# CFGpp-diffusion/CFGpp

Hardware: AMD Instinct MI355X
Metric: images/sec (higher is better)
Workload: dtype fp16; 1 GPU; SD1.5 512x512 ddim_cfg++ 50 NFE lambda=0.6 batch=8/GPU; per_gpu_batch=8, global_batch=8, nfe=50, unet_batch_rows=16, weights=seeded synthetic, exact diffusers shapes, build_id=cfgpp-build:650f45cb6498717d:nogit

## Files before the change

### cfgpp_amd/_lib.py

```python
from __future__ import annotations

import ctypes as C
import os

HERE = os.path.dirname(os.path.abspath(__file__))
LIB_PATH = os.environ.get("CFGPP_LIB") or os.path.join(HERE, "libcfgpp_hip.so")


class CfgppError(RuntimeError):
    pass


class UNetConfigC(C.Structure):
    _fields_ = [
        ("in_channels", C.c_int), ("out_channels", C.c_int),
        ("num_levels", C.c_int),
        ("block_out_channels", C.c_int * 4),
        ("layers_per_block", C.c_int),
        ("level_has_attn", C.c_int * 4),
        ("transformer_depth", C.c_int * 4),
        ("num_heads", C.c_int * 4),
        ("cross_attention_dim", C.c_int),
        ("addition_embed", C.c_int),
        ("addition_time_embed_dim", C.c_int),
# ... 15 lines not shown
    "cfgpp_kdiff_input": (_I, [_P, _P, _F, _I, _L, _P]),
    "cfgpp_step_kdiff": (_I, [_P, _P, _P, _P, _P, C.POINTER(C.c_float), _I, _I, _I, _I, _L, _P]),
    "cfgpp_kdiff_denoise": (_I, [_P, _P, _P, _F, _F, _P, _P, _L, _P]),
    "cfgpp_lincomb": (_I, [_P, _P, _P, _P, _F, _F, _I, _L, _P]),
    "cfgpp_unet_create": (_P, [C.POINTER(UNetConfigC), _I]),
    "cfgpp_unet_destroy": (None, [_P]),
    "cfgpp_unet_load_tensor": (_I, [_P, C.c_char_p, _P, _I, C.POINTER(C.c_long), _I]),
    "cfgpp_unet_missing": (_I, [_P]),
    "cfgpp_unet_finalize": (_I, [_P]),
    "cfgpp_unet_set_context": (_I, [_P, _P, _I, _I, _P, _P, _I, _P]),
    "cfgpp_unet_image_condition": (_I, [_P, _P, _I, _P]),
    "cfgpp_unet_forward": (_I, [_P, _P, _I, _I, _F, _P, _I, _P]),
    "cfgpp_sample_graph_ddim": (_I, [_P, _P, _P, _I, _I, _P, _P, _P, _I, C.POINTER(C.c_float), _I, _F, _I, _I, _P]),
    "cfgpp_unet_profile": (_I, [_P, _P, _I, _I, _F, _P, _I, _P, C.POINTER(C.c_double), C.POINTER(C.c_double), C.POINTER(C.c_int), C.c_char_p, _L]),
    "cfgpp_unet_tuning": (_I, [_P, _I, C.POINTER(C.c_int), _I, _I]),
    "cfgpp_unet_attach_control": (_I, [_P, _P, _F]),
    "cfgpp_unet_lora": (_I, [_P, C.c_char_p, _P, _P, _I, _P]),
    "cfgpp_unet_flops": (C.c_double, [_P, _I]),
    "cfgpp_unet_device_bytes": (C.c_double, [_P]),
    "cfgpp_vae_create": (_P, [_I, _I, _I, _F, _I]),
    "cfgpp_vae_destroy": (None, [_P]),
    "cfgpp_vae_load_tensor": (_I, [_P, C.c_char_p, _P, _I, C.POINTER(C.c_long), _I]),
    "cfgpp_vae_finalize": (_I, [_P]),
    "cfgpp_vae_decode": (_I, [_P, _P, _P, _I, _P]),
    "cfgpp_vae_decode_image": (_I, [_P, _P, _P, _I, _P]),
    "cfgpp_vae_encode": (_I, [_P, _P, _P, _P, _P, _I, _P]),
    "cfgpp_vae_flops": (C.c_double, [_P, _I]),
    "cfgpp_text_create": (_P, [_I, _I, _I, _I, _I, _I, _I, _I, _I]),
    "cfgpp_text_destroy": (None, [_P]),
    "cfgpp_text_load_tensor": (_I, [_P, C.c_char_p, _P, _I, C.POINTER(C.c_long), _I]),
    "cfgpp_text_finalize": (_I, [_P]),
    "cfgpp_text_encode": (_I, [_P, C.POINTER(C.c_int), C.POINTER(C.c_int), _I, _I, _P, _P, _P]),
    "cfgpp_text_device_bytes": (C.c_double, [_P]),
    "cfgpp_vae_encode_flops": (C.c_double, [_P, _I]),
    "cfgpp_vae_device_bytes": (C.c_double, [_P]),
}

IP_ADAPTER_PROTOTYPES = {
    "cfgpp_unet_ip_load": (_I, [_P, C.c_char_p, _P, _I, C.POINTER(C.c_long), _I]),
    "cfgpp_unet_image_context": (_I, [_P, _P, _I, _I, _F, _P]),
}

LONG_PROMPT_PROTOTYPES = {
    "cfgpp_unet_set_max_tokens": (_I, [_P, _I]),
}

DEBUG_PROTOTYPES = {
    "cfgpp_op_softmax_rows": (_I, [_P, _L, _I, _P]),
    "cfgpp_op_conv_in_ex": (_I, [_P, _I, _P, _P, _P, _I, _I, _I, _I, _I, _I, _P, _P, _F, _P]),
    "cfgpp_op_groupnorm": (_I, [_P, _P, _P, _P, _P, _P, _I, _I, _I, _I, _I, _I, _F, _I, _I, _P]),
    "cfgpp_op_groupnorm_pre": (_I, [_P, _P, _P, _P, _P, _P, _P, _P, _I, _I, _I, _I, _I, _I, _F, _I, _I, _P]),
    "cfgpp_op_igemm_set_gstat": (None, [_P]),
    "cfgpp_op_igemm_gstat_written": (_I, []),
    "cfgpp_groupnorm_set_prestats": (None, [_I]),
    "cfgpp_groupnorm_prestats_enabled": (_I, []),
    "cfgpp_unet_set_share_prefix": (None, [_I]),
    "cfgpp_unet_share_prefix_enabled": (_I, []),
    "cfgpp_unet_shared_prefix_ops": (_I, [_P, _I, _I]),
    "cfgpp_op_layernorm": (_I, [_P, _P, _P, _P, _L, _I, _F, _P]),
    "cfgpp_op_attention_prepare_vt": (_I, [_P, _I, _I, _I, _P]),
    "cfgpp_op_attention": (_I, [_P, _P, _P, _P, _I, _I, _I, _I, _I, _I, _I, _P]),
    "cfgpp_op_attention_cross": (_I, [_P, _P, _P, _P, _I, _I, _I, _I, _I, _I, _I, _P]),
    "cfgpp_attention_set_cross_long": (None, [_I]),
    "cfgpp_op_attention_clear_slots": (_I, [_P, _P, _I, _I, _I, _I, _I, _P]),
    "cfgpp_op_attention_ip": (_I, [_P, _P, _P, _P, _I, _I, _I, _I, _I, _I, _F, _I, _I, _P]),
    "cfgpp_op_conv_in": (_I, [_P, _I, _P, _P, _P, _I, _I, _I, _I, _I, _I, _P]),
    "cfgpp_op_conv_in_cond": (_I, [_P, _I, _P, _I, _I, _P, _P, _P, _I, _I, _I, _I, _I, _I, _P]),
    "cfgpp_op_conv_in_add": (_I, [_P, _I, _P, _I, _I, _P, _I, _P, _P, _P, _I, _I, _I, _I, _I, _I, _P]),
    "cfgpp_op_cn_conv3x3": (_I, [_P, _I, _P, _I, _P, _P, _I, _I, _I, _I, _I, _I, _I, _P]),
    "cfgpp_op_residual_add": (_I, [C.POINTER(C.c_void_p), C.POINTER(C.c_void_p), C.POINTER(C.c_int), _I, _I, _F, _P]),
    "cfgpp_op_residual_nchw": (_I, [_P, _P, _I, _I, _I, _I, _F, _P]),
    "cfgpp_controlnet_residual": (_I, [_P, _I, _F, _P, _I, C.POINTER(C.c_int), _P]),
    "cfgpp_vae_profile": (_I, [_P, _P, _P, _I, _P, C.c_char_p, C.c_long]),
    "cfgpp_unet_read_weight": (_I, [_P, C.c_char_p, _P]),
    "cfgpp_op_vae_posterior": (_I, [_P, _P, _P, _P, _P, _P, _I, _I, _F, _P]),
    "cfgpp_op_conv_out": (_I, [_P, _P, _I, _P, _P, _I, _I, _I, _I, _I, _P]),
    "cfgpp_op_conv_out_ex": (_I, [_P, _P, _I, _P, _P, _I, _I, _I, _I, _I, _F, _F, _I, _P]),
    "cfgpp_conv_out_set_tiled": (None, [_I]),
    "cfgpp_op_sinusoid": (_I, [_P, _F, _P, _I, _I, _I, _I, _P]),
    "cfgpp_op_skinny_gemm": (_I, [_P, _I, _P, _P, _P, _I, _P, _I, _I, _I, _I, _I, _I, _P]),
    "cfgpp_op_f16_to_f32_rows": (_I, [_P, _P, _I, _I, _I, _I, _P]),
    "cfgpp_op_igemm": (_I, [_P, _P, _I, _I, _I, _I, _I, _I, _P, _I, _I, _P, _P, _I, _P, _I, _I, _P, _I, _I, _I, _P]),
    "cfgpp_op_igemm_heads": (_I, [_P, _I, _P, _I, _I, _P, _I, _P, _P, _P, _I, _I, _I, _I, _I, _I, _P]),
    "cfgpp_igemm_force_config": (None, [_I]),
    "cfgpp_igemm_set_staging": (None, [_I]),
    "cfgpp_igemm_set_staged_epilogue": (None, [_I]),
    "cfgpp_igemm_set_big_tiles": (None, [_I]),
    "cfgpp_igemm_set_tail_split": (None, [_I]),
    "cfgpp_igemm_set_autotune": (None, [_I]),
    "cfgpp_igemm_set_blocked_walk": (None, [_I]),
    "cfgpp_igemm_walk_plan_probe": (None, [_I, _I, _I, _I, _I, _I, _I, C.POINTER(C.c_int)]),
    "cfgpp_igemm_set_n_major": (None, [_I]),
    "cfgpp_igemm_force_split": (None, [_I]),
    "cfgpp_igemm_set_split_tile": (None, [_I]),
    "cfgpp_igemm_set_mf16": (None, [_I]),
    "cfgpp_igemm_set_mf16_rounds": (None, [_I]),
    "cfgpp_igemm_set_mf16_heads": (None, [_I]),
    "cfgpp_igemm_set_mf16_linear": (None, [_I]),
    "cfgpp_igemm_set_big_split": (None, [_I]),
    "cfgpp_igemm_set_tune_mask": (None, [C.c_uint]),
    "cfgpp_igemm_tuner_state": (C.c_uint, []),
    "cfgpp_igemm_timeline": (None, [_P, _L, _I]),
    "cfgpp_igemm_timeline_info": (None, [C.POINTER(C.c_int)]),
    "cfgpp_groupnorm_set_mode": (None, [_I]),
    "cfgpp_layernorm_set_rows_per_wave": (None, [_I]),
    "cfgpp_attention_set_dma": (None, [_I]),
    "cfgpp_attention_set_stagger": (None, [_I]),
    "cfgpp_attention_set_cross": (None, [_I]),
    "cfgpp_attention_last_launch": (None, [C.POINTER(C.c_int)]),
    "cfgpp_groupnorm_last_launch": (None, [C.POINTER(C.c_int)]),
    "cfgpp_layernorm_last_launch": (None, [C.POINTER(C.c_int)]),
    "cfgpp_softmax_last_launch": (None, [C.POINTER(C.c_int)]),
}

_lib = None


def load():
    global _lib
    if _lib is not None:
        return _lib
    if not os.path.exists(LIB_PATH):
        raise CfgppError(
            f"{LIB_PATH} not found: build it with `python -m cfgpp_amd.build` "
            "(__graft_entry__.build()).  The HIP path has no CPU fallback.")
    import torch
    try:
        lib = C.CDLL(LIB_PATH)
    except OSError as e:
        raise CfgppError(f"cannot load {LIB_PATH}: {e}") from e
    for name, (res, args) in list(PROTOTYPES.items()) + list(IP_ADAPTER_PROTOTYPES.items()) + list(LONG_PROMPT_PROTOTYPES.items()) + list(DEBUG_PROTOTYPES.items()):
        try:
            fn = getattr(lib, name)
        except AttributeError as e:
            raise CfgppError(f"{LIB_PATH} does not export {name}") from e
        fn.restype = res
        fn.argtypes = args
    if os.environ.get("CFGPP_AUTOTUNE", "1") == "0":
        lib.cfgpp_igemm_set_autotune(0)
    _lib = lib
    return lib


def build_id() -> str:
    return load().cfgpp_build_id().decode("utf-8", "replace")


def last_error() -> str:
    return load().cfgpp_last_error().decode("utf-8", "replace")


def check(rc: int, what: str):
    if rc != 0:
        raise CfgppError(f"{what} failed (rc={rc}): {last_error()}")
```

### cfgpp_amd/csrc/big4.h

```cpp
#pragma once
#include "igemm.h"

inline void big4_tile(int cfg, int* BM, int* BN) {
    *BM = cfg == 24 ? 256 : 128;
    *BN = cfg == 25 ? 320 : 256;
}
inline bool big4_supports(int cfg, const IGemmArgs& a, bool staged_epi) {
    if (cfg < 24 || cfg > 26 || !staged_epi || a.K < 64) return false;
    const long rows = a.amode == 0 ? (long)a.M : a.amode == 2 ? (long)(a.M / a.rows_per_batch) * (2 * a.H + 2) * (2 * a.W + 2)
                                                : (long)(a.M / a.rows_per_batch) * (a.H + 2) * (a.W + 2);
    const long cmax = a.C0 > a.C1 ? a.C0 : a.C1;
    if (rows >= (1L << 24) || rows * cmax * 2 >= (1L << 32) || (long)a.N * a.K * 2 >= (1L << 32) || a.N >= (1 << 24)) return false;
    if (a.epi == EPI_STORE) return (a.N & 7) == 0;
    if (a.epi == EPI_GEGLU) return cfg != 25 && (a.N & 127) == 0 && a.omode == 0;
    return a.epi == EPI_HEADS && (a.rows_per_batch & 31) == 0 && (a.part_width & 31) == 0 && (a.head_dim & 7) == 0 && (a.N & 31) == 0 &&
           (a.M & 31) == 0;
}
int big4_par_bytes(int BN, int nb);
int big4_run(int cfg, const IGemmArgs& a, int grid, int smem, hipStream_t stream);

inline bool big4p_supports(const IGemmArgs& a, bool staged_epi) {
    return a.amode == 0 && a.C1 == 0 && a.taps == 1 && a.temb == nullptr && big4_supports(24, a, staged_epi) && (long)a.K * 2 < (1L << 24);
}
int big4p_smem(int par_bytes_one);
int big4p_run(const IGemmArgs& a, int grid, int smem, int par_bytes_one, hipStream_t stream);
```

### cfgpp_amd/csrc/cfgpp_debug.h

```cpp
#ifndef CFGPP_DEBUG_H
#define CFGPP_DEBUG_H
#ifdef __cplusplus
extern "C" {
#endif

int cfgpp_op_softmax_rows(void* s, long rows, int ncols, void* stream);
int cfgpp_op_conv_in_ex(const void* z, int z_is_half, void* out, const float* w, const float* bias,
                        int R, int zB, int Cin, int H, int W, int Cout, const float* pre_w, const float* pre_b,
                        float in_scale, void* stream);
int cfgpp_op_groupnorm(const void* src0, const void* src1, void* dst, const float* gamma, const float* beta,
                       float* stats, int N, int H, int W, int C0, int C1, int G, float eps, int silu,
                       int dst_padded, void* stream);
int cfgpp_op_groupnorm_pre(const void* src0, const void* src1, void* dst, const float* gamma, const float* beta,
                           const float* gst0, const float* gst1, float* stats, int N, int H, int W, int C0, int C1, int G,
                           float eps, int silu, int dst_padded, void* stream);
void cfgpp_op_igemm_set_gstat(void* buf);
int cfgpp_op_igemm_gstat_written(void);
void cfgpp_groupnorm_set_prestats(int on);
int cfgpp_groupnorm_prestats_enabled(void);
void cfgpp_unet_set_share_prefix(int on);
int cfgpp_unet_share_prefix_enabled(void);
int cfgpp_unet_shared_prefix_ops(cfgpp_unet* u, int rows, int z_rows);
void cfgpp_groupnorm_set_mode(int mode);
int cfgpp_op_layernorm(const void* x, void* y, const float* gamma, const float* beta, long rows, int C,
                       float eps, void* stream);
void cfgpp_layernorm_set_rows_per_wave(int rpw);
void cfgpp_groupnorm_last_launch(int* out8);
void cfgpp_layernorm_last_launch(int* out2);
void cfgpp_softmax_last_launch(int* out1);
int cfgpp_op_attention_prepare_vt(void* vt, int BH, int d, int tok_pad, void* stream);
int cfgpp_op_attention(const void* q, const void* k, const void* vt, void* o, int B, int heads, int d,
                       int nq, int nk, int q_tok_pad, int k_tok_pad, void* stream);
void cfgpp_attention_set_dma(int mode);
void cfgpp_attention_set_stagger(int sleeps);
void cfgpp_attention_set_cross(int on);
int cfgpp_op_attention_cross(const void* q, const void* k, const void* vt, void* o, int B, int heads, int d,
                             int nq, int nk, int q_tok_pad, int k_tok_pad, void* stream);
void cfgpp_attention_set_cross_long(int mode);
void cfgpp_attention_last_launch(int* out4);
int cfgpp_op_attention_clear_slots(void* k, void* vt, int BH, int d, int tok_pad, int slot0, int n, void* stream);
int cfgpp_op_attention_ip(const void* q, const void* k, const void* vt, void* o, int B, int heads, int d, int nq, int nk_text,
                          int n_img, float ip_scale, int q_tok_pad, int k_tok_pad, void* stream);
int cfgpp_op_conv_in(const void* z, int z_is_half, void* out, const float* w, const float* bias,
                     int R, int zB, int Cin, int H, int W, int Cout, void* stream);
int cfgpp_op_conv_in_cond(const void* z, int z_is_half, const void* cond, int cond_rows, int Cc, void* out, const float* w,
                          const float* bias, int R, int zB, int Cz, int H, int W, int Cout, void* stream);
int cfgpp_op_conv_in_add(const void* z, int z_is_half, const void* cond, int cond_rows, int Cc, const void* addend, int add_rows,
                         void* out, const float* w, const float* bias, int R, int zB, int Cz, int H, int W, int Cout, void* stream);
int cfgpp_op_cn_conv3x3(const void* in, int in_kind, void* out, int out_pad, const float* w, const float* bias, int R, int Ci, int Co,
                        int Hi, int Wi, int stride, int silu, void* stream);
int cfgpp_op_residual_add(void* const* dst, const void* const* src, const int* hwc, int n, int rows, float scale, void* stream);
int cfgpp_op_residual_nchw(const void* src, float* out, int rows, int H, int W, int C, float scale, void* stream);
int cfgpp_controlnet_residual(cfgpp_unet* cn, int i, float scale, float* out, int rows, int* hwc_out, void* stream);

int cfgpp_unet_read_weight(cfgpp_unet* u, const char* key, void* host_fp16_out);

int cfgpp_vae_profile(cfgpp_vae* v, const void* z, void* img, int B, void* stream, char* detail, long detail_cap);

int cfgpp_op_vae_posterior(const float* conv_out, const float* qw, const float* qb, const float* noise, float* z,
                           float* moments, int B, int HW, float scale, void* stream);
int cfgpp_op_conv_out(const void* x, void* out, int out_is_half, const void* w, const float* bias,
                      int R, int H, int W, int C, int Cout, void* stream);
int cfgpp_op_conv_out_ex(const void* x, void* out, int out_is_half, const void* w, const float* bias,
                         int R, int H, int W, int C, int Cout, float post_scale, float post_shift, int clamp01, void* stream);
void cfgpp_conv_out_set_tiled(int on);
int cfgpp_op_sinusoid(const float* vals, float scalar, float* out, int count, int dim, int out_ld, int out_off,
                      void* stream);
int cfgpp_op_skinny_gemm(const float* x, int ldx, const void* w, const float* bias, const float* addend, int add_ld,
                         float* out, int ldo, int M, int N, int K, int silu_in, int silu_out, void* stream);
int cfgpp_op_f16_to_f32_rows(const void* in, float* out, int rows, int cols, int out_ld, int out_off, void* stream);

int cfgpp_op_igemm(const void* a0, const void* a1, int C0, int C1, int taps, int amode, int H, int W,
                   const void* w, int M, int N, const float* bias, const float* temb, int temb_ld,
                   const void* resid, int rmode, int rld, void* out, int omode, int old_, int epi,
                   void* stream);
int cfgpp_op_igemm_heads(const void* a, int K, const void* w, int M, int N, const float* bias, int rows_per_batch,
                         void* hq, void* hk, void* hvt, int part0, int part_width, int head_dim, int heads,
                         int q_tok_pad, int tok_pad, void* stream);
void cfgpp_igemm_force_config(int cfg);
void cfgpp_igemm_set_tail_split(int on);
void cfgpp_igemm_set_mf16(int mode);
void cfgpp_igemm_set_mf16_linear(int on);
void cfgpp_igemm_set_mf16_heads(int on);
void cfgpp_igemm_set_mf16_rounds(int n);
void cfgpp_igemm_set_split_tile(int cfg);
void cfgpp_igemm_force_split(int s);
void cfgpp_igemm_set_big_split(int min_kt);
void cfgpp_igemm_set_n_major(int mode);
void cfgpp_igemm_set_blocked_walk(int on);
void cfgpp_igemm_walk_plan_probe(int M, int N, int K, int BM, int BN, int smem, int n_major, int* out5);
void cfgpp_igemm_set_tune_mask(unsigned mask);
unsigned cfgpp_igemm_tuner_state(void);
void cfgpp_igemm_set_autotune(int on);
void cfgpp_igemm_set_big_tiles(int on);
void cfgpp_igemm_set_staged_epilogue(int on);
void cfgpp_igemm_set_staging(int glds);
void cfgpp_igemm_timeline(void* buf, long cap_blocks, int target);
void cfgpp_igemm_timeline_info(int* out12);

#ifdef __cplusplus
}
#endif
#endif
```

### cfgpp_amd/csrc/engine_base.h

```cpp
#pragma once
#include <algorithm>
#include <cmath>
#include <cstring>
#include <deque>
#include <functional>
#include <map>
#include <string>
#include <utility>
#include <vector>

#include "../../include/cfgpp.h"
#include "../../include/cfgpp_ip_adapter.h"
#include "../../include/cfgpp_long_prompt.h"
#include "cfgpp_debug.h"
#include "igemm.h"

namespace {


struct HostParam {
    std::vector<long> shape;
    std::vector<half_t> h;
    std::vector<float> f;
    bool is_matrix = false;
// ... 69 lines not shown
        static const int cands[] = {0, 1, 4, 5, 6, 7, 8, 9, 10, 11, 12, 13, 14, 15, 16, 17, 20, 24, 25, 26, 27, 28};
        const size_t n = plan.size();
        plan_hint.resize(n, nullptr);
        hipStreamCaptureStatus cap = hipStreamCaptureStatusNone;
        if (hipStreamIsCapturing(s, &cap) != hipSuccess || cap != hipStreamCaptureStatusNone) return 0;
        std::vector<hipEvent_t> ev(n + 1, nullptr);
        for (auto& e : ev) if (hipEventCreate(&e) != hipSuccess) return -1;
        std::vector<float> base(n, 1e30f), best(n, 1e30f), t(n);
        std::vector<char> applied(n, 1);
        std::vector<int> bestc(n, 0);
        int rc = 0;
        auto timed_passes = [&]() {
            std::fill(t.begin(), t.end(), 1e30f);
            for (int rep = 0; rep < 2 && rc == 0; ++rep) {
                if (hipEventRecord(ev[0], s) != hipSuccess) rc = -1;
                for (size_t i = 0; i < n && rc == 0; ++i) {
                    rc = plan[i](s, rows_for(i, rows, shared));
                    if (plan_hint[i]) applied[i] = (char)igemm_last_hint_applied();
                    if (rc == 0 && hipEventRecord(ev[i + 1], s) != hipSuccess) rc = -1;
                }
                if (rc == 0 && hipEventSynchronize(ev[n]) != hipSuccess) rc = -1;
                for (size_t i = 0; i < n && rc == 0; ++i) {
                    if (!plan_hint[i]) continue;
                    float ms = 0.f;
                    if (hipEventElapsedTime(&ms, ev[i], ev[i + 1]) == hipSuccess && ms < t[i]) t[i] = ms;
                }
            }
        };
        const unsigned mask = igemm_tune_mask();
        for (int c : cands) {
            if (c != 0 && !((mask >> c) & 1u)) continue;
            for (int& h : cfg_hints) h = c;
            timed_passes();
            for (size_t i = 0; i < n; ++i) {
                if (c == 0) base[i] = t[i];
                if (t[i] < best[i] && (c == 0 || applied[i])) { best[i] = t[i]; bestc[i] = c; }
            }
        }
        for (size_t i = 0; i < n; ++i)
            if (plan_hint[i] && !(bestc[i] != 0 && best[i] < 0.97f * base[i])) { bestc[i] = 0; best[i] = base[i]; }
        for (int walk = 1; walk <= 2 && rc == 0 && (mask >> 31); ++walk) {
            for (size_t i = 0; i < n; ++i) if (plan_hint[i]) *plan_hint[i] = (bestc[i] & 63) | (walk << 6);
            timed_passes();
            for (size_t i = 0; i < n; ++i)
                if (plan_hint[i] && t[i] < 0.97f * best[i]) { best[i] = t[i]; bestc[i] = (bestc[i] & 63) | (walk << 6); }
        }
        for (int& h : cfg_hints) h = 0;
        for (size_t i = 0; i < n; ++i) if (plan_hint[i]) *plan_hint[i] = bestc[i];
        for (auto& e : ev) hipEventDestroy(e);
        if (rc == 0) tuned_by_rows[key] = std::vector<int>(cfg_hints.begin(), cfg_hints.end());
        tuned_rows = rows; tuned_shared = shared;
        return rc;
    }
    std::map<std::tuple<int, int, int>, std::vector<std::pair<half_t*, float*>>> pool;
    std::deque<int> gst_flags;
    float* d_gn_stats = nullptr;
    static constexpr long KSPLIT_WS_BYTES = 128L << 20;
    float* d_ksplit_ws = nullptr;
    float* ksplit_ws() {
        if (!d_ksplit_ws) d_ksplit_ws = (float*)dmalloc((size_t)KSPLIT_WS_BYTES, false);
        return d_ksplit_ws;
    }

    void* dmalloc(size_t bytes, bool zero = true) {
        void* p = nullptr;
        if (hipMalloc(&p, bytes) != hipSuccess) return nullptr;
        if (zero) hipMemset(p, 0, bytes);
        allocs.push_back(p);
        dev_bytes += (double)bytes;
        return p;
    }
    Tensor acq(int H, int W, int C) {
        auto key = std::make_tuple(H, W, C);
        auto& fl = pool[key];
        Tensor t; t.H = H; t.W = W; t.C = C;
        gst_flags.push_back(0);
        t.gst_ok = &gst_flags.back();
        if (!fl.empty()) { t.p = fl.back().first; t.gst = fl.back().second; fl.pop_back(); return t; }
        t.p = (half_t*)dmalloc((size_t)max_rows * (H + 2) * (W + 2) * C * sizeof(half_t));
        if (H * W >= 1024 && (H * W) % 32 == 0 && C % 8 == 0)
            t.gst = (float*)dmalloc((size_t)max_rows * (H * W / 32) * C * 2 * sizeof(float), false);
        return t;
    }
    void rel(const Tensor& t) { if (t.p) pool[std::make_tuple(t.H, t.W, t.C)].push_back(std::make_pair(t.p, t.gst)); }
    ~EngineBase() { for (void* p : allocs) hipFree(p); }
};

void expect(EngineBase* u, const std::string& key, std::vector<long> shape, bool matrix) {
    HostParam hp; hp.shape = std::move(shape); hp.is_matrix = matrix;
    u->params[key] = std::move(hp);
}
void expect_linear(EngineBase* u, const std::string& p, long out, long in, bool bias = true) {
    expect(u, p + ".weight", {out, in}, true);
    if (bias) expect(u, p + ".bias", {out}, false);
}
void expect_conv(EngineBase* u, const std::string& p, long out, long in, int k) {
    expect(u, p + ".weight", {out, in, k, k}, true);
    expect(u, p + ".bias", {out}, false);
}
void expect_norm(EngineBase* u, const std::string& p, long c) {
    expect(u, p + ".weight", {c}, false);
    expect(u, p + ".bias", {c}, false);
}
void expect_resnet(EngineBase* u, const std::string& p, long cin, long cout, long temb) {
    expect_norm(u, p + ".norm1", cin);
    expect_conv(u, p + ".conv1", cout, cin, 3);
    expect_linear(u, p + ".time_emb_proj", cout, temb);
    expect_norm(u, p + ".norm2", cout);
    expect_conv(u, p + ".conv2", cout, cout, 3);
    if (cin != cout) expect_conv(u, p + ".conv_shortcut", cout, cin, 1);
}
void expect_transformer(EngineBase* u, const std::string& p, long c, int depth, long cross) {
    expect_norm(u, p + ".norm", c);
    expect(u, p + ".proj_in.weight", {c, c}, true);  expect(u, p + ".proj_in.bias", {c}, false);
    expect(u, p + ".proj_out.weight", {c, c}, true); expect(u, p + ".proj_out.bias", {c}, false);
    for (int k = 0; k < depth; ++k) {
        const std::string b = p + ".transformer_blocks." + std::to_string(k);
        expect_norm(u, b + ".norm1", c); expect_norm(u, b + ".norm2", c); expect_norm(u, b + ".norm3", c);
        expect_linear(u, b + ".attn1.to_q", c, c, false); expect_linear(u, b + ".attn1.to_k", c, c, false);
        expect_linear(u, b + ".attn1.to_v", c, c, false); expect_linear(u, b + ".attn1.to_out.0", c, c, true);
        expect_linear(u, b + ".attn2.to_q", c, c, false); expect_linear(u, b + ".attn2.to_k", c, cross, false);
        expect_linear(u, b + ".attn2.to_v", c, cross, false); expect_linear(u, b + ".attn2.to_out.0", c, c, true);
        expect_linear(u, b + ".ff.net.0.proj", 8 * c, c, true);
        expect_linear(u, b + ".ff.net.2", c, 4 * c, true);
    }
}

struct Builder {
    EngineBase* u;
    bool ok = true;
    std::string err;

    HostParam* get(const std::string& key) {
        auto it = u->params.find(key);
        if (it == u->params.end() || !it->second.loaded) { ok = false; err = "missing parameter " + key; return nullptr; }
        return &it->second;
    }
    template <typename T>
    T* upload(const std::vector<T>& v) {
        T* d = (T*)u->dmalloc(v.size() * sizeof(T), false);
        if (!d) { ok = false; err = "hipMalloc failed"; return nullptr; }
        if (hipMemcpy(d, v.data(), v.size() * sizeof(T), hipMemcpyHostToDevice) != hipSuccess) { ok = false; err = "hipMemcpy failed"; }
        return d;
    }
    void slot(const std::string& key, half_t* d, int kind, long row_off = 0) {
        const HostParam& p = u->params[key];
        WeightSlot w; w.ptr = d; w.kind = kind; w.row_off = row_off; w.O = p.shape[0];
        w.taps = kind == SLOT_CONV3 ? 9 : 1; w.I = p.numel() / (w.O * w.taps);
        u->slots[key] = w;
    }
    void drop(const std::string& key) { auto& p = u->params[key]; std::vector<half_t>().swap(p.h); std::vector<float>().swap(p.f); }

    float* f32(const std::string& key) {
        HostParam* p = get(key); if (!p) return nullptr;
        float* d = upload(p->f); drop(key); return d;
    }
    half_t* linear(const std::string& key) {
        HostParam* p = get(key); if (!p) return nullptr;
        half_t* d = upload(p->h); drop(key); slot(key, d, SLOT_PLAIN); return d;
    }
    half_t* conv3(const std::string& key) {
        HostParam* p = get(key); if (!p) return nullptr;
        const long O = p->shape[0], I = p->shape[1];
        std::vector<half_t> r((size_t)O * 9 * I);
        for (long o = 0; o < O; ++o)
            for (long i = 0; i < I; ++i)
                for (int t = 0; t < 9; ++t) r[(size_t)o * 9 * I + ((i >> 6) * 9 + t) * 64 + (i & 63)] = p->h[((size_t)o * I + i) * 9 + t];
        half_t* d = upload(r); drop(key); slot(key, d, SLOT_CONV3); return d;
    }
    std::vector<half_t> concat_host(const std::vector<std::string>& keys) {
        std::vector<half_t> r;
        for (auto& k : keys) { HostParam* p = get(k); if (!p) return {}; r.insert(r.end(), p->h.begin(), p->h.end()); }
        for (auto& k : keys) drop(k);
        return r;
    }
    half_t* concat(const std::vector<std::string>& keys) {
        std::vector<half_t> r = concat_host(keys);
        if (!ok) return nullptr;
        half_t* d = upload(r);
        long row = 0;
        for (auto& k : keys) { slot(k, d, SLOT_MEMBER, row); row += u->params[k].shape[0]; }
        return d;
    }
    bool geglu_host(const std::string& pfx, long C, std::vector<half_t>& rw, std::vector<float>& rb) {
        HostParam* pw = get(pfx + ".weight"); HostParam* pb = get(pfx + ".bias");
        if (!pw || !pb) return false;
        const long F = 4 * C;
        rw.resize((size_t)2 * F * C); rb.resize((size_t)2 * F);
        for (long f = 0; f < F; ++f) {
            const long pv = (f / 32) * 64 + (f % 32), pg = pv + 32;
            std::memcpy(&rw[(size_t)pv * C], &pw->h[(size_t)f * C], C * sizeof(half_t));
            std::memcpy(&rw[(size_t)pg * C], &pw->h[(size_t)(F + f) * C], C * sizeof(half_t));
            rb[pv] = pb->f[f]; rb[pg] = pb->f[F + f];
        }
        drop(pfx + ".weight"); drop(pfx + ".bias");
        return true;
    }
    void geglu(const std::string& pfx, long C, half_t** w, float** b) {
        std::vector<half_t> rw; std::vector<float> rb;
        if (!geglu_host(pfx, C, rw, rb)) return;
        *w = upload(rw); *b = upload(rb);
        slot(pfx + ".weight", *w, SLOT_GEGLU);
    }
};

inline int round_up(int a, int b) { return (a + b - 1) / b * b; }

IGemmArgs base_args(EngineBase* u = nullptr) {
    IGemmArgs a; std::memset(&a, 0, sizeof(a)); a.out_scale = 1.0f; a.taps = 1;
    if (u) { a.ws_buf = u->ksplit_ws(); a.ws_bytes = a.ws_buf ? EngineBase::KSPLIT_WS_BYTES : 0; }
    return a;
}

struct Plan {
    EngineBase* u;
    Builder* B;
    std::vector<Op>* ops;

    void conv3x3(const Tensor& src, const Tensor& dst, const half_t* w, const float* bias, int amode,
                 const float* temb, int temb_ld, const Tensor* resid, int ashift = 0) {
        IGemmArgs a = base_args(u);
        a.a0 = src.p; a.C0 = src.C; a.taps = 9; a.amode = amode; a.ashift = ashift; a.H = dst.H; a.W = dst.W;
        a.w = w; a.N = dst.C; a.K = 9 * src.C; a.bias = bias; a.temb = temb; a.temb_ld = temb_ld;
        a.rows_per_batch = dst.H * dst.W;
        if (resid) { a.resid = resid->p; a.rmode = 1; a.rld = resid->C; }
        a.out = dst.p; a.omode = 1; a.old = dst.C; a.epi = EPI_STORE;
        a.gstat = dst.gst; a.stat_flag = dst.gst ? dst.gst_ok : nullptr;
        const int HW = dst.H * dst.W;
        u->macs_per_row += (double)HW * dst.C * 9.0 * src.C;
        int* hint = u->new_hint(ops == &u->plan);
        ops->push_back([a, HW, hint](hipStream_t s, int rows) mutable { IGemmArgs b = a; b.M = rows * HW; b.cfg_hint = *hint; return igemm_launch(b, s); });
        if (ops == &u->plan) u->tag(0, (double)HW * dst.C * 9.0 * src.C, "conv3x3 amode=" + std::to_string(amode) + " HW=" + std::to_string(HW) + " N=" + std::to_string(dst.C) + " K=" + std::to_string(9 * src.C) + (resid ? " +res" : "") + (temb ? " +temb" : ""));
    }
    void conv1x1(const Tensor& s0, const Tensor* s1, const Tensor& dst, const half_t* w, const float* bias) {
        IGemmArgs a = base_args(u);
        a.a0 = s0.p; a.C0 = s0.C; if (s1) { a.a1 = s1->p; a.C1 = s1->C; }
        a.amode = 1; a.H = dst.H; a.W = dst.W; a.w = w; a.N = dst.C; a.K = a.C0 + a.C1; a.bias = bias;
        a.rows_per_batch = dst.H * dst.W; a.out = dst.p; a.omode = 1; a.old = dst.C; a.epi = EPI_STORE;
        const int HW = dst.H * dst.W;
        u->macs_per_row += (double)HW * dst.C * a.K;
        int* hint = u->new_hint(ops == &u->plan);
        ops->push_back([a, HW, hint](hipStream_t s, int rows) mutable { IGemmArgs b = a; b.M = rows * HW; b.cfg_hint = *hint; return igemm_launch(b, s); });
        if (ops == &u->plan) u->tag(0, (double)HW * dst.C * a.K, "conv1x1 HW=" + std::to_string(HW) + " N=" + std::to_string(dst.C) + " K=" + std::to_string(a.K));
    }
    void linear(const half_t* A, int K, half_t* out, int N, const half_t* w, const float* bias, const half_t* resid,
                int tokens, int epi = EPI_STORE) {
        IGemmArgs a = base_args(u);
        a.a0 = A; a.C0 = K; a.amode = 0; a.w = w; a.N = N; a.K = K; a.bias = bias;
        a.resid = resid; a.rmode = 0; a.rld = N; a.out = out; a.omode = 0;
        a.old = (epi == EPI_GEGLU) ? N / 2 : N; a.epi = epi; a.rows_per_batch = tokens;
        u->macs_per_row += (double)tokens * N * K;
        int* hint = u->new_hint(ops == &u->plan);
        ops->push_back([a, tokens, hint](hipStream_t s, int rows) mutable { IGemmArgs b = a; b.M = rows * tokens; b.cfg_hint = *hint; return igemm_launch(b, s); });
        if (ops == &u->plan) u->tag(0, (double)tokens * N * K, std::string(epi == EPI_GEGLU ? "geglu" : "linear") + " HW=" + std::to_string(tokens) + " N=" + std::to_string(N) + " K=" + std::to_string(K) + (resid ? " +res" : ""));
    }
    void linear_to_padded(const half_t* A, int K, const Tensor& dst, const half_t* w, const float* bias, const Tensor& resid) {
        IGemmArgs a = base_args(u);
        a.a0 = A; a.C0 = K; a.amode = 0; a.H = dst.H; a.W = dst.W; a.w = w; a.N = dst.C; a.K = K; a.bias = bias;
        a.resid = resid.p; a.rmode = 1; a.rld = resid.C; a.out = dst.p; a.omode = 1; a.old = dst.C;
        a.epi = EPI_STORE; a.rows_per_batch = dst.H * dst.W;
        a.gstat = dst.gst; a.stat_flag = dst.gst ? dst.gst_ok : nullptr;
        const int HW = dst.H * dst.W;
        u->macs_per_row += (double)HW * dst.C * K;
        int* hint = u->new_hint(ops == &u->plan);
        ops->push_back([a, HW, hint](hipStream_t s, int rows) mutable { IGemmArgs b = a; b.M = rows * HW; b.cfg_hint = *hint; return igemm_launch(b, s); });
        if (ops == &u->plan) u->tag(0, (double)HW * dst.C * K, "proj_out HW=" + std::to_string(HW) + " N=" + std::to_string(dst.C) + " K=" + std::to_string(K));
    }
    void heads(const half_t* A, int K, const half_t* w, int N, int tokens, int part0, int C, int nheads,
               half_t* q, half_t* k, half_t* vt, int q_tok_pad, int tok_pad, bool count = true,
               const float* bias = nullptr) {
        IGemmArgs a = base_args(u);
        const int d = C / nheads;
        a.a0 = A; a.C0 = K; a.amode = 0; a.w = w; a.N = N; a.K = K; a.epi = EPI_HEADS;
        a.bias = bias;
        a.rows_per_batch = tokens; a.hq = q; a.hk = k; a.hvt = vt; a.part0 = part0; a.part_width = C;
        a.head_dim = d; a.head_dim_pad = round_up(d, 32); a.heads = nheads; a.tok_pad = tok_pad; a.q_tok_pad = q_tok_pad;
        if (count) u->macs_per_row += (double)tokens * N * K;
        int* hint = u->new_hint(ops == &u->plan);
        ops->push_back([a, tokens, hint](hipStream_t s, int rows) mutable { IGemmArgs b = a; b.M = rows * tokens; b.cfg_hint = *hint; return igemm_launch(b, s); });
        if (ops == &u->plan) u->tag(0, count ? (double)tokens * N * K : 0.0, "heads HW=" + std::to_string(tokens) + " N=" + std::to_string(N) + " K=" + std::to_string(K));
    }
    void groupnorm(const Tensor& s0, const Tensor* s1, half_t* dst, bool dst_padded, const float* g, const float* b,
                   float eps, bool silu) {
        EngineBase* uu = u;
        const half_t* p0 = s0.p; const half_t* p1 = s1 ? s1->p : nullptr;
        const int H = s0.H, W = s0.W, C0 = s0.C, C1 = s1 ? s1->C : 0, G = u->norm_groups;
        const float* gst0 = s0.gst; const float* gst1 = s1 ? s1->gst : nullptr;
        const int* ok0 = s0.gst_ok; const int* ok1 = s1 ? s1->gst_ok : nullptr;
        ops->push_back([=](hipStream_t s, int rows) {
            if (cfgpp_groupnorm_prestats_enabled() && gst0 && ok0 && *ok0 && (!p1 || (gst1 && ok1 && *ok1)))
                return cfgpp_op_groupnorm_pre(p0, p1, dst, g, b, gst0, gst1, uu->d_gn_stats, rows, H, W, C0, C1, G, eps, silu ? 1 : 0,
                                              dst_padded ? 1 : 0, s);
            return cfgpp_op_groupnorm(p0, p1, dst, g, b, uu->d_gn_stats, rows, H, W, C0, C1, G, eps, silu ? 1 : 0,
                                      dst_padded ? 1 : 0, s);
        });
        if (ops == &u->plan) u->tag(2, 0.0, "groupnorm HW=" + std::to_string(H * W) + " C=" + std::to_string(C0 + C1));
    }
    void layernorm(const half_t* x, half_t* y, const float* g, const float* b, int tokens, int C) {
        ops->push_back([=](hipStream_t s, int rows) { return cfgpp_op_layernorm(x, y, g, b, (long)rows * tokens, C, 1e-5f, s); });
        if (ops == &u->plan) u->tag(2, 0.0, "layernorm HW=" + std::to_string(tokens) + " C=" + std::to_string(C));
    }
    void attention(const half_t* q, const half_t* k, const half_t* vt, half_t* o, int nheads, int d, int nq, int nk,
                   int q_tok_pad, int k_tok_pad) {
        u->attn_macs_per_row += 2.0 * (double)nheads * nq * nk * d;
        ops->push_back([=](hipStream_t s, int rows) {
            return cfgpp_op_attention(q, k, vt, o, rows, nheads, d, nq, nk, q_tok_pad, k_tok_pad, s);
        });
        if (ops == &u->plan) u->tag(1, 2.0 * (double)nheads * nq * nk * d, "self_attn heads=" + std::to_string(nheads) + " N=" + std::to_string(nq) + " d=" + std::to_string(d));
    }
};

}
```

### cfgpp_amd/csrc/igemm.h

```cpp
#pragma once
#include "common.h"

enum IGemmEpi : int {
    EPI_STORE = 0,
    EPI_GEGLU = 1,
    EPI_HEADS = 2,
};

struct IGemmArgs {
    const half_t* a0;
    const half_t* a1;
    int C0, C1;
    int taps;
    int amode;
    int H, W;
    int ashift;
    const half_t* w;
    int M, N, K;
    int epi;
    const float* bias;
    const float* temb;
    int temb_ld;
    int rows_per_batch;
    const half_t* resid;
    int rmode, rld;
    half_t* out;
    int omode, old;
    float out_scale;
    float* gstat;
    int* stat_flag;
    half_t* hq; half_t* hk; half_t* hvt;
    int part0;
    int part_width;
    int head_dim, head_dim_pad, heads;
    int vt_linear;
    int tok_pad;
    int q_tok_pad;
    int n_main;
    int ksplit;
    float* ws;
    float* ws_buf;
    long ws_bytes;
    int cfg_hint;
    int allow_split;
    int staged_epi;
    int n_major;
    int walk_div;
    int walk_hint;
    int walk_bn, walk_per, walk_tmb, walk_tnb;
    int split;
    int par_nb;
    unsigned long long* tl;
};

int igemm_launch(const IGemmArgs& a, hipStream_t stream);
int igemm_autotune_enabled();
int igemm_last_hint_applied();
unsigned igemm_tune_mask();
```

### cfgpp_amd/csrc/igemm_device.h

```cpp
#pragma once
#include "igemm.h"

namespace {


__device__ __forceinline__ void tl_stamp(unsigned long long* tl, int slot) {
    if (tl != nullptr && threadIdx.x == 0) tl[(long)blockIdx.x * 16 + slot] = __builtin_amdgcn_s_memtime();
}
__device__ __forceinline__ void tl_begin(unsigned long long* tl) {
    if (tl != nullptr && threadIdx.x == 0) {
        unsigned long long* r = tl + (long)blockIdx.x * 16;
        r[0] = __builtin_amdgcn_s_memtime();
        r[4] = __builtin_amdgcn_s_memrealtime();
        const unsigned hw = __builtin_amdgcn_s_getreg((31 << 11) | 4), xcc = __builtin_amdgcn_s_getreg((31 << 11) | 20);
        r[6] = (unsigned long long)hw | ((unsigned long long)xcc << 32);
    }
}
__device__ __forceinline__ void tl_end(unsigned long long* tl) {
    if (tl != nullptr) {
        asm volatile("s_waitcnt vmcnt(0)" ::: "memory");
        if (threadIdx.x == 0) {
            unsigned long long* r = tl + (long)blockIdx.x * 16;
            r[3] = __builtin_amdgcn_s_memtime();
            r[5] = __builtin_amdgcn_s_memrealtime();
        }
    }
}

__device__ __forceinline__ int qdiv(int m, int d) {
    int dv = d;
    asm volatile("" : "+v"(dv));
    const float inv = __builtin_amdgcn_rcpf((float)dv);
    int q = (int)((float)m * inv);
    const int r = m - q * d;
    q += (r >= d ? 1 : 0) - (r < 0 ? 1 : 0);
    return q;
}

__device__ __forceinline__ int padded_pix(int m, int HW, int W, int H) {
    const int b = qdiv(m, HW), p = m - b * HW;
    const int y = qdiv(p, W), x = p - y * W;
    return (b * (H + 2) + y + 1) * (W + 2) + x + 1;
}


__device__ __forceinline__ int qdiv_u(int a, int d) { return __builtin_amdgcn_readfirstlane(qdiv(a, d)); }
__device__ __forceinline__ void tile_of(const IGemmArgs& p, int wg, int& tile_m, int& tile_n) {
    if (p.walk_bn > 0) {
        const int x = qdiv_u(wg, p.walk_per), i = wg - x * p.walk_per;
        const int bmi = qdiv_u(x, p.walk_bn), bni = x - bmi * p.walk_bn;
        int im, in;
        if (p.n_major) { in = qdiv_u(i, p.walk_tmb); im = i - in * p.walk_tmb; }
        else { im = qdiv_u(i, p.walk_tnb); in = i - im * p.walk_tnb; }
        tile_m = bmi * p.walk_tmb + im; tile_n = bni * p.walk_tnb + in;
    } else {
        const int wq = qdiv(wg, p.walk_div), wr = wg - wq * p.walk_div;
        tile_m = p.n_major ? wr : wq; tile_n = p.n_major ? wq : wr;
    }
}

constexpr int PAR_NB = 5;
__host__ __device__ constexpr int par_bnp(int BN) { return (BN + 63) / 64 * 64; }
__host__ __device__ constexpr int par_bytes(int BN, int nb = PAR_NB) { return par_bnp(BN) * 4 * (1 + nb); }
struct Par {
    const char* lds;
    int n0, b0, bnp;
};
template <int BN, int NW>
__device__ __forceinline__ void par_stage(const IGemmArgs& p, char* par, int n0, int m0, int wid, int lane) {
    constexpr int BNP = par_bnp(BN), NPC = BNP / 64;
    int nn = n0 + lane;
    const int HW = p.rows_per_batch;
    const int b0 = HW > 0 ? qdiv(m0, HW) : 0;
    const int nb = HW > 0 ? (p.M + HW - 1) / HW : 1;
    int pi = 0;
    auto arr = [&](const float* src, int slot) {
#pragma unroll
        for (int q = 0; q < NPC; ++q, ++pi) {
            if (wid == pi % NW) {
                int n = nn + 64 * q;
                n = n < p.N ? n : p.N - 1;
                __builtin_amdgcn_global_load_lds((const __attribute__((address_space(1))) void*)(src + n),
                                                 (__attribute__((address_space(3))) void*)(par + (slot * BNP + q * 64) * 4), 4, 0, 0);
            }
        }
    };
    if (p.bias) arr(p.bias, 0);
    if (p.temb) {
        for (int k = 0; k < p.par_nb; ++k) {
            int b = b0 + k;
            b = b < nb ? b : nb - 1;
            arr(p.temb + (long)b * p.temb_ld, 1 + k);
        }
    }
}
template <bool L>
__device__ __forceinline__ float4 par_bias4(const IGemmArgs& p, const Par& q, int n) {
    if constexpr (L) return *reinterpret_cast<const float4*>(q.lds + (n - q.n0) * 4);
    else return *reinterpret_cast<const float4*>(p.bias + n);
}
template <bool L>
__device__ __forceinline__ float4 par_temb4(const IGemmArgs& p, const Par& q, int b, int n) {
    if constexpr (L) {
        int k = b - q.b0;
        k = k < p.par_nb ? k : p.par_nb - 1;
        k = k < 0 ? 0 : k;
        return *reinterpret_cast<const float4*>(q.lds + ((1 + k) * q.bnp + n - q.n0) * 4);
    } else {
        return *reinterpret_cast<const float4*>(p.temb + (long)b * p.temb_ld + n);
    }
}
template <bool PIN, int NT>
__device__ __forceinline__ void acc_row_pin(f32x16 (&row)[NT]) {
    if constexpr (PIN) {
#pragma unroll
        for (int j = 0; j < NT; ++j) asm volatile("" : "+a"(row[j]));
    }
}
template <int MT, int NT, bool L>
__device__ __forceinline__ void igemm_epilogue(const IGemmArgs& p, f32x16 (&acc)[MT][NT], int mw0, int nw0, int lane, const Par& par) {
    const int frow = lane & 31, fhi = lane >> 5;
    const int HW = p.rows_per_batch;
#pragma unroll
    for (int i = 0; i < MT; ++i) {
        const int m = mw0 + i * 32 + frow;
        if (m >= p.M) continue;
        const int b = (HW > 0) ? qdiv(m, HW) : 0;
        const int tok = m - b * HW;
        long orow = m, rrow = m;
        if (p.omode == 1 || p.rmode == 1) {
            const long pp = padded_pix(m, HW, p.W, p.H);
            if (p.omode == 1) orow = pp;
            if (p.rmode == 1) rrow = pp;
        }
        if (p.epi == EPI_STORE) {
#pragma unroll
            for (int j = 0; j < NT; ++j)
#pragma unroll
                for (int g = 0; g < 4; ++g) {
                    int n = nw0 + j * 32 + 8 * g + 4 * fhi;
                    asm volatile("" : "+v"(n));
                    if (n >= p.N) continue;
                    float v[4];
#pragma unroll
                    for (int k = 0; k < 4; ++k) v[k] = acc[i][j][4 * g + k] * p.out_scale;
                    if (p.bias) {
                        const float4 bb = par_bias4<L>(p, par, n);
                        v[0] += bb.x; v[1] += bb.y; v[2] += bb.z; v[3] += bb.w;
                    }
                    if (p.temb) {
                        const float4 tt = par_temb4<L>(p, par, b, n);
                        v[0] += tt.x; v[1] += tt.y; v[2] += tt.z; v[3] += tt.w;
                    }
                    if (p.resid) {
                        const half4_t rr = *reinterpret_cast<const half4_t*>(p.resid + rrow * p.rld + n);
#pragma unroll
                        for (int k = 0; k < 4; ++k) v[k] += (float)rr[k];
                    }
                    half4_t o;
#pragma unroll
                    for (int k = 0; k < 4; ++k) o[k] = (half_t)v[k];
                    *reinterpret_cast<half4_t*>(p.out + orow * p.old + n) = o;
                }
        } else if (p.epi == EPI_GEGLU) {
            if constexpr (NT % 2 == 0) {
#pragma unroll
                for (int j = 0; j < NT; j += 2)
#pragma unroll
                    for (int g = 0; g < 4; ++g) {
                        const int pc = nw0 + j * 32 + 8 * g + 4 * fhi;
                        if (pc >= p.N) continue;
                        const int f = (pc >> 6) * 32 + (pc & 31);
                        float v[4], gt[4];
#pragma unroll
                        for (int k = 0; k < 4; ++k) { v[k] = acc[i][j][4 * g + k]; gt[k] = acc[i][j + 1][4 * g + k]; }
                        if (p.bias) {
                            const float4 bv = par_bias4<L>(p, par, pc);
                            const float4 bg = par_bias4<L>(p, par, pc + 32);
                            v[0] += bv.x; v[1] += bv.y; v[2] += bv.z; v[3] += bv.w;
                            gt[0] += bg.x; gt[1] += bg.y; gt[2] += bg.z; gt[3] += bg.w;
                        }
                        half4_t o;
                        const f32x2 g01 = gelu_erf_pk((f32x2){gt[0], gt[1]}), g23 = gelu_erf_pk((f32x2){gt[2], gt[3]});
                        o[0] = (half_t)(v[0] * g01.x); o[1] = (half_t)(v[1] * g01.y);
                        o[2] = (half_t)(v[2] * g23.x); o[3] = (half_t)(v[3] * g23.y);
                        *reinterpret_cast<half4_t*>(p.out + orow * p.old + f) = o;
                    }
            }
        } else {
#pragma unroll
            for (int j = 0; j < NT; ++j)
#pragma unroll
                for (int g = 0; g < 4; ++g) {
                    int n = nw0 + j * 32 + 8 * g + 4 * fhi;
                    asm volatile("" : "+v"(n));
                    if (n >= p.N) continue;
                    const int part = n / p.part_width + p.part0;
                    const int cn = n % p.part_width;
                    const int head = cn / p.head_dim, dd = cn - head * p.head_dim;
                    float v[4];
#pragma unroll
                    for (int k = 0; k < 4; ++k) v[k] = acc[i][j][4 * g + k];
                    if (p.bias) {
                        const float4 bb = par_bias4<L>(p, par, n);
                        v[0] += bb.x; v[1] += bb.y; v[2] += bb.z; v[3] += bb.w;
                    }
                    const long bh = (long)b * p.heads + head;
                    if (part == 2) {
                        half_t* dst = p.hvt + (bh * p.head_dim_pad + dd) * p.tok_pad + (p.vt_linear ? tok : cfgpp_vt_pos(tok));
#pragma unroll
                        for (int k = 0; k < 4; ++k) dst[(long)k * p.tok_pad] = (half_t)v[k];
                    } else {
                        half4_t o;
#pragma unroll
                        for (int k = 0; k < 4; ++k) o[k] = (half_t)v[k];
                        half_t* base = part == 0 ? p.hq : p.hk;
                        const int tp = part == 0 ? p.q_tok_pad : p.tok_pad;
                        *reinterpret_cast<half4_t*>(base + (bh * tp + tok) * p.head_dim_pad + dd) = o;
                    }
                }
        }
    }
}

template <int WTN, int PITCH>
__device__ __forceinline__ void gstat_block(const IGemmArgs& p, const char* stg, int m_blk0, int nw0, int lane) {
    if (m_blk0 >= p.M) return;
    float* dst = p.gstat + ((long)(m_blk0 >> 5) * p.N + nw0) * 2;
#pragma unroll 1
    for (int cp = lane; cp < WTN / 2; cp += 64) {
        const half2_t x0 = *reinterpret_cast<const half2_t*>(stg + cp * 4);
        const float pv0 = (float)x0[0], pv1 = (float)x0[1];
        float s0 = 0.f, s1 = 0.f, q0 = 0.f, q1 = 0.f;
#pragma unroll 4
        for (int r = 1; r < 32; ++r) {
            const half2_t x = *reinterpret_cast<const half2_t*>(stg + r * PITCH + cp * 4);
            const float d0 = (float)x[0] - pv0, d1 = (float)x[1] - pv1;
            s0 += d0; q0 += d0 * d0; s1 += d1; q1 += d1 * d1;
        }
        if (nw0 + 2 * cp < p.N)
            *reinterpret_cast<float4*>(dst + 4 * cp) = make_float4(pv0 + s0 * (1.0f / 32.0f), q0 - s0 * s0 * (1.0f / 32.0f),
                                                                   pv1 + s1 * (1.0f / 32.0f), q1 - s1 * s1 * (1.0f / 32.0f));
    }
}

template <int MT, int NT, bool L, bool PIN = false>
__device__ __forceinline__ void igemm_epilogue_staged(const IGemmArgs& p, f32x16 (&acc)[MT][NT], int mw0, int nw0, int lane,
                                                      char* stg , const Par& par) {
    constexpr int WTN = NT * 32;
    constexpr int PITCH = WTN * 2 + 16;
    constexpr int CPR = WTN / 8;
    constexpr int NQ = (32 * CPR + 63) / 64;
    constexpr bool EARLY = false;
    const int frow = lane & 31, fhi = lane >> 5;
    const int HW = p.rows_per_batch;
#pragma unroll
    for (int i = 0; i < MT; ++i) {
        acc_row_pin<PIN, NT>(acc[i]);
        const int m = mw0 + i * 32 + frow;
        const int mc = m < p.M ? m : p.M - 1;
        const int b = (HW > 0) ? qdiv(mc, HW) : 0;
        int opix = mc, rpix = mc;
        if (p.omode == 1 || p.rmode == 1) {
            const int pp = padded_pix(mc, HW, p.W, p.H);
            if (p.omode == 1) opix = pp;
            if (p.rmode == 1) rpix = pp;
        }
        half8_t rres[NQ];
        auto request_residual = [&]() {
#pragma unroll
            for (int q = 0; q < NQ; ++q) {
                const int c = lane + 64 * q;
                const int r = c / CPR, cc = c - r * CPR;
                const int rp = __shfl(rpix, r);
                int n = nw0 + cc * 8;
                n = n < p.N ? n : p.N - 8;
                rres[q] = *reinterpret_cast<const half8_t*>(p.resid + (long)rp * p.rld + n);
            }
        };
        if constexpr (EARLY) { if (p.resid) request_residual(); }
#pragma unroll
        for (int j = 0; j < NT; ++j)
#pragma unroll
            for (int g = 0; g < 4; ++g) {
                const int nl = j * 32 + 8 * g + 4 * fhi;
                int n = nw0 + nl;
                n = n < p.N ? n : p.N - 4;
                float v[4];
#pragma unroll
                for (int k = 0; k < 4; ++k) v[k] = acc[i][j][4 * g + k] * p.out_scale;
                if (p.bias) {
                    const float4 bb = par_bias4<L>(p, par, n);
                    v[0] += bb.x; v[1] += bb.y; v[2] += bb.z; v[3] += bb.w;
                }
                if (p.temb) {
                    const float4 tt = par_temb4<L>(p, par, b, n);
                    v[0] += tt.x; v[1] += tt.y; v[2] += tt.z; v[3] += tt.w;
                }
                half4_t o;
#pragma unroll
                for (int k = 0; k < 4; ++k) o[k] = (half_t)v[k];
                *reinterpret_cast<half4_t*>(stg + frow * PITCH + nl * 2) = o;
            }
        if constexpr (!EARLY) { if (p.resid) request_residual(); }
#pragma unroll
        for (int q = 0; q < NQ; ++q) {
            const int c = lane + 64 * q;
            const int r = c / CPR, cc = c - r * CPR;
            const int op = __shfl(opix, r);
            const int mm = mw0 + i * 32 + r, n = nw0 + cc * 8;
            half8_t v = *reinterpret_cast<const half8_t*>(stg + (r & 31) * PITCH + cc * 16);
            if (p.resid) {
#pragma unroll
                for (int k = 0; k < 8; ++k) v[k] = (half_t)((float)v[k] + (float)rres[q][k]);
                if (p.gstat && c < 32 * CPR) *reinterpret_cast<half8_t*>(stg + (r & 31) * PITCH + cc * 16) = v;
            }
            if (c < 32 * CPR && mm < p.M && n < p.N) *reinterpret_cast<half8_t*>(p.out + (long)op * p.old + n) = v;
        }
        if (p.gstat) gstat_block<WTN, PITCH>(p, stg, mw0 + i * 32, nw0, lane);
    }
}

template <int MT, int NT, bool L, bool PIN = false>
__device__ __forceinline__ void igemm_epilogue_geglu_staged(const IGemmArgs& p, f32x16 (&acc)[MT][NT], int mw0, int nw0, int lane,
                                                            char* stg, const Par& par) {
    constexpr int WTF = (NT / 2) * 32;
    constexpr int PITCH = WTF * 2 + 16;
    constexpr int CPR = WTF / 8;
    constexpr int NQ = (32 * CPR + 63) / 64;
    const int frow = lane & 31, fhi = lane >> 5;
    const int f0 = (nw0 >> 6) * 32;
    const int NF = p.N >> 1;
#pragma unroll
    for (int i = 0; i < MT; ++i) {
        acc_row_pin<PIN, NT>(acc[i]);
#pragma unroll
        for (int j = 0; j < NT; j += 2)
#pragma unroll
            for (int g = 0; g < 4; ++g) {
                int pc = nw0 + j * 32 + 8 * g + 4 * fhi;
                pc = pc < p.N ? pc : p.N - 64;
                float v[4], gt[4];
#pragma unroll
                for (int k = 0; k < 4; ++k) { v[k] = acc[i][j][4 * g + k]; gt[k] = acc[i][j + 1][4 * g + k]; }
                if (p.bias) {
                    const float4 bv = par_bias4<L>(p, par, pc);
                    const float4 bg = par_bias4<L>(p, par, pc + 32);
                    v[0] += bv.x; v[1] += bv.y; v[2] += bv.z; v[3] += bv.w;
                    gt[0] += bg.x; gt[1] += bg.y; gt[2] += bg.z; gt[3] += bg.w;
                }
                half4_t o;
                const f32x2 g01 = gelu_erf_pk((f32x2){gt[0], gt[1]}), g23 = gelu_erf_pk((f32x2){gt[2], gt[3]});
                o[0] = (half_t)(v[0] * g01.x); o[1] = (half_t)(v[1] * g01.y);
                o[2] = (half_t)(v[2] * g23.x); o[3] = (half_t)(v[3] * g23.y);
                *reinterpret_cast<half4_t*>(stg + frow * PITCH + ((j >> 1) * 32 + 8 * g + 4 * fhi) * 2) = o;
            }
#pragma unroll
        for (int q = 0; q < NQ; ++q) {
            const int c = lane + 64 * q;
            const int r = c / CPR, cc = c - r * CPR;
            const int mm = mw0 + i * 32 + r, f = f0 + cc * 8;
            if (c < 32 * CPR && mm < p.M && f < NF)
                *reinterpret_cast<half8_t*>(p.out + (long)mm * p.old + f) = *reinterpret_cast<const half8_t*>(stg + r * PITCH + cc * 16);
        }
    }
}

struct HeadCol { int part, head, dd; };
__device__ __forceinline__ HeadCol head_col(const IGemmArgs& p, int ng_uniform) {
    const int ng = __builtin_amdgcn_readfirstlane(ng_uniform);
    const int pr = ng / p.part_width, cn0 = ng - pr * p.part_width;
    const int h = cn0 / p.head_dim;
    HeadCol c; c.part = pr + p.part0; c.head = h; c.dd = cn0 - h * p.head_dim;
    return c;
}
__device__ __forceinline__ void head_step(const IGemmArgs& p, const HeadCol& c, int off, int& head, int& dd) {
    dd = c.dd + off; head = c.head;
    if (p.head_dim >= 32) {
        if (dd >= p.head_dim) { dd -= p.head_dim; ++head; }
    } else {
        const int q = dd / p.head_dim;
        head += q; dd -= q * p.head_dim;
    }
}

template <int MT, int NT, bool L, bool PIN = false>
__device__ __forceinline__ void igemm_epilogue_heads_staged(const IGemmArgs& p, f32x16 (&acc)[MT][NT], int mw0, int nw0, int lane,
                                                            char* stg , const Par& par) {
    constexpr int PITCH = 80, BLK = 32 * PITCH;
    const int frow = lane & 31, fhi = lane >> 5;
    const int HW = p.rows_per_batch;
    const int ppos = cfgpp_vt_pos(frow);
    HeadCol hc[NT];
#pragma unroll
    for (int j = 0; j < NT; ++j) { const int ng = nw0 + j * 32; hc[j] = head_col(p, ng < p.N ? ng : p.N - 32); }
#pragma unroll
    for (int i = 0; i < MT; ++i) {
        acc_row_pin<PIN, NT>(acc[i]);
        const int m0s = __builtin_amdgcn_readfirstlane(mw0 + i * 32);
        if (m0s >= p.M) continue;
        const int b = qdiv(m0s, HW), tok0 = m0s - b * HW;
#pragma unroll
// ... 63 lines not shown
```

### cfgpp_amd/csrc/igemm_kernel.hip

```cpp
#include <cstring>
#include <map>
#include <tuple>
#include <type_traits>
#include "igemm.h"

#include "igemm_device.h"
#include "big4.h"

namespace {

template <int WM, int WN, int WTM, int WTN, bool GLDS, int AMODE, int NST = 2>
__global__ void __launch_bounds__(64 * WM * WN)
igemm_kernel(const IGemmArgs p) {
    constexpr int NTHR = 64 * WM * WN;
    constexpr int BM = WM * WTM, BN = WN * WTN;
    constexpr int MT = WTM / 32, NT = WTN / 32;
    constexpr int RSTEP = NTHR / 8;
    constexpr int A_CH = BM / RSTEP, B_CH = BN / RSTEP;
    static_assert(BM % RSTEP == 0 && BN % RSTEP == 0, "tile/loader mismatch");
    constexpr int STAGE_BYTES = (BM + BN) * 128;

    extern __shared__ __attribute__((aligned(16))) char smem[];
    tl_begin(p.tl);
    constexpr int PAR_OFF = NST * (WM * WTM + WN * WTN) * 128;

    const int ntn = (p.N + BN - 1) / BN;
    const int bid = blockIdx.x;
    int wg, ksl = 0;
    const bool is_tail = bid >= p.n_main;
    if (!is_tail) {
        const int nwg = p.n_main;
        const int q = nwg >> 3, r = nwg & 7;
        const int xcd = bid & 7, idx = bid >> 3;
        wg = (xcd < r ? xcd * (q + 1) : r * (q + 1) + (xcd - r) * q) + idx;
    } else {
        const int b1 = bid - p.n_main, nb = (int)gridDim.x - p.n_main;
        const int q = nb >> 3, r = nb & 7;
        const int xcd = b1 & 7, idx = b1 >> 3;
        const int b2 = (xcd < r ? xcd * (q + 1) : r * (q + 1) + (xcd - r) * q) + idx;
        wg = p.n_main + b2 / p.ksplit;
        ksl = b2 - (b2 / p.ksplit) * p.ksplit;
    }
    int tile_m, tile_n;
    tile_of(p, wg, tile_m, tile_n);
    const int m0 = tile_m * BM, n0 = tile_n * BN;

    const int tid = threadIdx.x, lane = tid & 63, wid = tid >> 6;
    const int wm = wid / WN, wn = wid - wm * WN;

    const int lrow = tid >> 3, lchunk = tid & 7;
    const int HW = p.rows_per_batch;
    const int Cin = p.C0 + p.C1;
    int a_pix[A_CH];
#pragma unroll
    for (int j = 0; j < A_CH; ++j) {
        int m = m0 + lrow + j * RSTEP;
        m = m < p.M ? m : p.M - 1;
        if constexpr (AMODE == 0) a_pix[j] = m;
        else if constexpr (AMODE == 1) a_pix[j] = padded_pix(m, HW, p.W, p.H);
        else if constexpr (AMODE == 2) {
            const int b = qdiv(m, HW), q = m - b * HW, y = qdiv(q, p.W), x = q - y * p.W;
            a_pix[j] = (b * (2 * p.H + 2) + 2 * y + 1 + p.ashift) * (2 * p.W + 2) + 2 * x + 1 + p.ashift;
        } else {
            const int b = qdiv(m, HW), q = m - b * HW, y = qdiv(q, p.W), x = q - y * p.W;
            a_pix[j] = (b << 22) | (y << 11) | x;
        }
    }
    const int schunk = GLDS ? (lchunk ^ ((lrow >> 1) & 7)) : lchunk;
    const half_t* b_ptr[B_CH];
#pragma unroll
    for (int j = 0; j < B_CH; ++j) {
        int n = n0 + lrow + j * RSTEP;
        n = n < p.N ? n : p.N - 1;
        b_ptr[j] = p.w + (long)n * p.K + schunk * 8;
    }
    int st_off[(A_CH > B_CH ? A_CH : B_CH)];
#pragma unroll
    for (int j = 0; j < (A_CH > B_CH ? A_CH : B_CH); ++j) {
        const int r = lrow + j * RSTEP;
        st_off[j] = r * 128 + ((lchunk ^ ((r >> 1) & 7)) << 4);
    }

    half8_t ra[A_CH], rb[B_CH];
    const int KT_all = p.K >> 6;
    const int kt_begin = is_tail ? (int)(((long)ksl * KT_all) / p.ksplit) : 0;
    const int kt_end = is_tail ? (int)(((long)(ksl + 1) * KT_all) / p.ksplit) : KT_all;

    auto load_tile = [&](int kt) {
        int tap = 0, cc = kt << 6;
        if (p.taps == 9) { const int cb = kt / 9; tap = kt - cb * 9; cc = cb << 6; }
        const bool s0 = cc < p.C0;
        const half_t* src = s0 ? p.a0 : p.a1;
        const int cs = s0 ? cc : cc - p.C0, Cs = s0 ? p.C0 : p.C1;
        int dy = 0, dx = 0;
        if (p.taps == 9) { dy = tap / 3 - 1; dx = tap - (tap / 3) * 3 - 1; }
        int dpix = 0;
        if constexpr (AMODE == 1) dpix = dy * (p.W + 2) + dx;
        else if constexpr (AMODE == 2) dpix = dy * (2 * p.W + 2) + dx;
#pragma unroll
        for (int j = 0; j < A_CH; ++j) {
            int pix;
            if constexpr (AMODE == 3) {
                const int b = a_pix[j] >> 22, y = (a_pix[j] >> 11) & 2047, x = a_pix[j] & 2047;
                const int Hs = p.H >> 1, Ws = p.W >> 1;
                pix = (b * (Hs + 2) + ((y + dy) >> 1) + 1) * (Ws + 2) + ((x + dx) >> 1) + 1;
            } else {
                pix = a_pix[j] + dpix;
            }
            ra[j] = *reinterpret_cast<const half8_t*>(src + (long)pix * Cs + cs + lchunk * 8);
        }
#pragma unroll
        for (int j = 0; j < B_CH; ++j) rb[j] = *reinterpret_cast<const half8_t*>(b_ptr[j] + ((long)kt << 6));
    };
    const int wave_row0 = __builtin_amdgcn_readfirstlane(wid) * 8;
    auto dma_tile = [&](int kt, int stage) {
        int tap = 0, cc = kt << 6;
        if (p.taps == 9) { const int cb = kt / 9; tap = kt - cb * 9; cc = cb << 6; }
        const bool s0 = cc < p.C0;
        const half_t* src = s0 ? p.a0 : p.a1;
        const int cs = s0 ? cc : cc - p.C0, Cs = s0 ? p.C0 : p.C1;
        int dy = 0, dx = 0;
        if (p.taps == 9) { dy = tap / 3 - 1; dx = tap - (tap / 3) * 3 - 1; }
        int dpix = 0;
        if constexpr (AMODE == 1) dpix = dy * (p.W + 2) + dx;
        else if constexpr (AMODE == 2) dpix = dy * (2 * p.W + 2) + dx;
        char* As = smem + stage * STAGE_BYTES;
        char* Bs = As + BM * 128;
#pragma unroll
        for (int j = 0; j < A_CH; ++j) {
            int pix;
            if constexpr (AMODE == 3) {
                const int b = a_pix[j] >> 22, y = (a_pix[j] >> 11) & 2047, x = a_pix[j] & 2047;
                const int Hs = p.H >> 1, Ws = p.W >> 1;
                pix = (b * (Hs + 2) + ((y + dy) >> 1) + 1) * (Ws + 2) + ((x + dx) >> 1) + 1;
            } else {
                pix = a_pix[j] + dpix;
            }
            const half_t* g = src + (long)pix * Cs + cs + schunk * 8;
            __builtin_amdgcn_global_load_lds((const __attribute__((address_space(1))) void*)g,
                                             (__attribute__((address_space(3))) void*)(As + (wave_row0 + j * RSTEP) * 128), 16, 0, 0);
        }
#pragma unroll
        for (int j = 0; j < B_CH; ++j) {
            const half_t* g = b_ptr[j] + ((long)kt << 6);
            __builtin_amdgcn_global_load_lds((const __attribute__((address_space(1))) void*)g,
                                             (__attribute__((address_space(3))) void*)(Bs + (wave_row0 + j * RSTEP) * 128), 16, 0, 0);
        }
    };
    auto store_tile = [&](int stage) {
        char* As = smem + stage * STAGE_BYTES;
        char* Bs = As + BM * 128;
#pragma unroll
        for (int j = 0; j < A_CH; ++j) *reinterpret_cast<half8_t*>(As + st_off[j]) = ra[j];
#pragma unroll
        for (int j = 0; j < B_CH; ++j) *reinterpret_cast<half8_t*>(Bs + st_off[j]) = rb[j];
    };

    f32x16 acc[MT][NT];
#pragma unroll
    for (int i = 0; i < MT; ++i)
#pragma unroll
        for (int j = 0; j < NT; ++j)
#pragma unroll
            for (int k = 0; k < 16; ++k) acc[i][j][k] = 0.f;

    const int frow = lane & 31, fhi = lane >> 5;
    const int fsw = (frow >> 1) & 7;
    const int a_rd = (wm * WTM + frow) * 128;
    const int b_rd = (wn * WTN + frow) * 128;

    if constexpr (GLDS) {
        constexpr int NP = A_CH + B_CH;
        constexpr int NM = 4 * MT * NT;
        constexpr bool ILV = (WM * WN >= 8);
        constexpr int SPAN = ILV ? (NM * 5) / 8 : 0;
        const int nk = kt_end - kt_begin;
        tl_stamp(p.tl, 8);
        if (!is_tail) par_stage<BN, WM * WN>(p, smem + PAR_OFF, n0, m0, __builtin_amdgcn_readfirstlane(wid), lane);
#pragma unroll
        for (int s_ = 0; s_ < NST - 1; ++s_) if (s_ < nk) dma_tile(kt_begin + s_, s_);
        tl_stamp(p.tl, 9);
        if (NST > 2 && nk >= NST - 1) asm volatile("s_waitcnt vmcnt(%0)" :: "n"((NST > 2 ? (NST - 2) * NP : 0)) : "memory");
        else asm volatile("s_waitcnt vmcnt(0)" ::: "memory");
        __syncthreads();
        tl_stamp(p.tl, 1);
        auto tile_body = [&](int kt, int cur, int ktn, int nxt, auto with_dma) {
            constexpr bool DMA = decltype(with_dma)::value;
            const char* As = smem + cur * STAGE_BYTES;
            const char* Bs = As + BM * 128;
            const half_t* src = p.a0; int cs = 0, Cs = p.C0, dpix = 0, dy = 0, dx = 0;
            char* Asn = smem + nxt * STAGE_BYTES;
            char* Bsn = Asn + BM * 128;
            if constexpr (DMA) {
                int tap = 0, cc = ktn << 6;
                if (p.taps == 9) { const int cb = ktn / 9; tap = ktn - cb * 9; cc = cb << 6; }
                const bool s0 = cc < p.C0;
                src = s0 ? p.a0 : p.a1;
                cs = s0 ? cc : cc - p.C0; Cs = s0 ? p.C0 : p.C1;
                if (p.taps == 9) { dy = tap / 3 - 1; dx = tap - (tap / 3) * 3 - 1; }
                if constexpr (AMODE == 1) dpix = dy * (p.W + 2) + dx;
                else if constexpr (AMODE == 2) dpix = dy * (2 * p.W + 2) + dx;
            }
            auto piece = [&](int q) {
                if (q < A_CH) {
                    const int j = q;
                    int pix;
                    if constexpr (AMODE == 3) {
                        const int b = a_pix[j] >> 22, y = (a_pix[j] >> 11) & 2047, x = a_pix[j] & 2047;
                        const int Hs = p.H >> 1, Ws = p.W >> 1;
                        pix = (b * (Hs + 2) + ((y + dy) >> 1) + 1) * (Ws + 2) + ((x + dx) >> 1) + 1;
                    } else {
                        pix = a_pix[j] + dpix;
                    }
                    const half_t* g = src + (long)pix * Cs + cs + schunk * 8;
                            __builtin_amdgcn_global_load_lds((const __attribute__((address_space(1))) void*)g,
                                                     (__attribute__((address_space(3))) void*)(Asn + (wave_row0 + j * RSTEP) * 128), 16, 0, 0);
                } else {
                    const int j = q - A_CH;
                    const half_t* g = b_ptr[j] + ((long)ktn << 6);
                            __builtin_amdgcn_global_load_lds((const __attribute__((address_space(1))) void*)g,
                                                     (__attribute__((address_space(3))) void*)(Bsn + (wave_row0 + j * RSTEP) * 128), 16, 0, 0);
                }
            };
            int issued = 0, done = 0;
            if constexpr (DMA && !ILV) {
#pragma unroll
                for (int q = 0; q < NP; ++q) piece(q);
                issued = NP;
            }
            auto after_mfma = [&]() {
                ++done;
                if constexpr (DMA && ILV) {
                    if (issued < NP && done * NP >= (issued + 1) * SPAN) {
                        __builtin_amdgcn_sched_barrier(0);
                        piece(issued); ++issued;
                        __builtin_amdgcn_sched_barrier(0);
                    }
                }
            };
            if constexpr (MT * NT <= 8) {
                half8_t xa[2][MT], wb[2][NT];
                {
                    const int coff = ((0 | fhi) ^ fsw) << 4;
#pragma unroll
                    for (int i = 0; i < MT; ++i) xa[0][i] = *reinterpret_cast<const half8_t*>(As + a_rd + i * 32 * 128 + coff);
#pragma unroll
                    for (int j = 0; j < NT; ++j) wb[0][j] = *reinterpret_cast<const half8_t*>(Bs + b_rd + j * 32 * 128 + coff);
                }
#pragma unroll
                for (int ks = 0; ks < 4; ++ks) {
                    if (ks < 3) {
                        const int coff = ((((ks + 1) << 1) | fhi) ^ fsw) << 4;
#pragma unroll
                        for (int i = 0; i < MT; ++i) xa[(ks + 1) & 1][i] = *reinterpret_cast<const half8_t*>(As + a_rd + i * 32 * 128 + coff);
#pragma unroll
                        for (int j = 0; j < NT; ++j) wb[(ks + 1) & 1][j] = *reinterpret_cast<const half8_t*>(Bs + b_rd + j * 32 * 128 + coff);
                    }
#pragma unroll
                    for (int i = 0; i < MT; ++i) {
#pragma unroll
                        for (int j = 0; j < NT; ++j) {
                            acc[i][j] = __builtin_amdgcn_mfma_f32_32x32x16_f16(wb[ks & 1][j], xa[ks & 1][i], acc[i][j], 0, 0, 0);
                            after_mfma();
                        }
                    }
                }
            } else {
#pragma unroll
                for (int ks = 0; ks < 4; ++ks) {
                    const int coff = (((ks << 1) | fhi) ^ fsw) << 4;
                    half8_t xa[MT], wb[NT];
#pragma unroll
                    for (int i = 0; i < MT; ++i) xa[i] = *reinterpret_cast<const half8_t*>(As + a_rd + i * 32 * 128 + coff);
#pragma unroll
                    for (int j = 0; j < NT; ++j) wb[j] = *reinterpret_cast<const half8_t*>(Bs + b_rd + j * 32 * 128 + coff);
#pragma unroll
                    for (int i = 0; i < MT; ++i) {
#pragma unroll
                        for (int j = 0; j < NT; ++j) {
                            acc[i][j] = __builtin_amdgcn_mfma_f32_32x32x16_f16(wb[j], xa[i], acc[i][j], 0, 0, 0);
                            after_mfma();
                        }
                    }
                    __builtin_amdgcn_sched_barrier(0);
// ... 12 lines not shown
                asm volatile("s_waitcnt lgkmcnt(0)" ::: "memory");
                __builtin_amdgcn_s_barrier();
                asm volatile("" ::: "memory");
            }
        };
        int kt = kt_begin;
        for (; kt + NST - 1 < kt_end; ++kt) {
            tile_body(kt, (kt - kt_begin) % NST, kt + NST - 1, (kt - kt_begin + NST - 1) % NST, std::true_type{});
            if (kt == kt_begin) tl_stamp(p.tl, 7);
        }
        for (; kt < kt_end; ++kt) tile_body(kt, (kt - kt_begin) % NST, 0, 0, std::false_type{});
        tl_stamp(p.tl, 2);
    } else {
        load_tile(kt_begin);
        store_tile(0);
    __syncthreads();
    for (int kt = kt_begin; kt < kt_end; ++kt) {
        const int cur = (kt - kt_begin) & 1;
        if (kt + 1 < kt_end) {
            load_tile(kt + 1);
        }
        const char* As = smem + cur * STAGE_BYTES;
        const char* Bs = As + BM * 128;
        if constexpr (MT * NT <= 8) {
            half8_t xa[2][MT], wb[2][NT];
            {
                const int coff = ((0 | fhi) ^ fsw) << 4;
#pragma unroll
                for (int i = 0; i < MT; ++i) xa[0][i] = *reinterpret_cast<const half8_t*>(As + a_rd + i * 32 * 128 + coff);
#pragma unroll
                for (int j = 0; j < NT; ++j) wb[0][j] = *reinterpret_cast<const half8_t*>(Bs + b_rd + j * 32 * 128 + coff);
            }
#pragma unroll
            for (int ks = 0; ks < 4; ++ks) {
                if (ks < 3) {
                    const int coff = ((((ks + 1) << 1) | fhi) ^ fsw) << 4;
#pragma unroll
                    for (int i = 0; i < MT; ++i) xa[(ks + 1) & 1][i] = *reinterpret_cast<const half8_t*>(As + a_rd + i * 32 * 128 + coff);
#pragma unroll
                    for (int j = 0; j < NT; ++j) wb[(ks + 1) & 1][j] = *reinterpret_cast<const half8_t*>(Bs + b_rd + j * 32 * 128 + coff);
                }
#pragma unroll
                for (int i = 0; i < MT; ++i)
#pragma unroll
                    for (int j = 0; j < NT; ++j)
                        acc[i][j] = __builtin_amdgcn_mfma_f32_32x32x16_f16(wb[ks & 1][j], xa[ks & 1][i], acc[i][j], 0, 0, 0);
            }
        } else {
#pragma unroll
            for (int ks = 0; ks < 4; ++ks) {
                const int coff = (((ks << 1) | fhi) ^ fsw) << 4;
                half8_t xa[MT], wb[NT];
#pragma unroll
                for (int i = 0; i < MT; ++i) xa[i] = *reinterpret_cast<const half8_t*>(As + a_rd + i * 32 * 128 + coff);
#pragma unroll
                for (int j = 0; j < NT; ++j) wb[j] = *reinterpret_cast<const half8_t*>(Bs + b_rd + j * 32 * 128 + coff);
#pragma unroll
                for (int i = 0; i < MT; ++i)
#pragma unroll
                    for (int j = 0; j < NT; ++j)
                        acc[i][j] = __builtin_amdgcn_mfma_f32_32x32x16_f16(wb[j], xa[i], acc[i][j], 0, 0, 0);
                __builtin_amdgcn_sched_barrier(0);
            }
        }
        if (kt + 1 < kt_end) store_tile(cur ^ 1);
        __syncthreads();
    }

    }

    const int mw0 = m0 + wm * WTM, nw0 = n0 + wn * WTN;
    if (is_tail) {
        float* ws = p.ws + ((long)(wg - p.n_main) * p.ksplit + ksl) * (MT * NT * 16) * NTHR + tid;
#pragma unroll
        for (int i = 0; i < MT; ++i)
#pragma unroll
            for (int j = 0; j < NT; ++j)
#pragma unroll
                for (int r = 0; r < 16; ++r) ws[(long)((i * NT + j) * 16 + r) * NTHR] = acc[i][j][r];
        tl_end(p.tl);
        return;
    }
    Par par;
    par.lds = GLDS ? smem + PAR_OFF : nullptr; par.n0 = n0; par.b0 = HW > 0 ? qdiv(m0, HW) : 0; par.bnp = par_bnp(BN);
    constexpr bool STAGED_FITS = WM * WN * 32 * (WTN * 2 + 16) <= NST * STAGE_BYTES;
    if (STAGED_FITS && p.epi == EPI_STORE && (p.N & 7) == 0 && p.staged_epi) {
        igemm_epilogue_staged<MT, NT, GLDS>(p, acc, mw0, nw0, lane, smem + wid * (32 * (WTN * 2 + 16)), par);
        tl_end(p.tl);
        return;
    }
    if constexpr (NT % 2 == 0) {
        if (p.epi == EPI_GEGLU && (p.N & 127) == 0 && p.staged_epi && p.omode == 0) {
            igemm_epilogue_geglu_staged<MT, NT, GLDS>(p, acc, mw0, nw0, lane, smem + wid * (32 * ((NT / 2) * 64 + 16)), par);
            tl_end(p.tl);
            return;
        }
    }
    constexpr bool HEADS_FITS = WM * WN * NT * 2560 <= NST * STAGE_BYTES && MT * NT <= 8;
    if constexpr (HEADS_FITS) if (p.epi == EPI_HEADS && p.staged_epi && (p.rows_per_batch & 31) == 0 && (p.part_width & 31) == 0 &&
        (p.head_dim & 7) == 0 && (p.N & 31) == 0 && (p.M & 31) == 0) {
        igemm_epilogue_heads_staged<MT, NT, GLDS>(p, acc, mw0, nw0, lane, smem + wid * (NT * 2560), par);
        tl_end(p.tl);
        return;
    }
    igemm_epilogue<MT, NT, GLDS>(p, acc, mw0, nw0, lane, par);
    tl_end(p.tl);
}

template <int WM, int WN, int WTM, int WTN>
__global__ void __launch_bounds__(64 * WM * WN)
igemm_reduce_kernel(const IGemmArgs p) {
    constexpr int NTHR = 64 * WM * WN;
    constexpr int BM = WM * WTM, BN = WN * WTN;
    constexpr int MT = WTM / 32, NT = WTN / 32;
    const int ntn = (p.N + BN - 1) / BN;
    const int wg = p.n_main + blockIdx.x;
    const int ij = blockIdx.y, i = ij / NT, j = ij - i * NT;
    const int tile_m = wg / ntn, tile_n = wg - tile_m * ntn;
    const int tid = threadIdx.x, lane = tid & 63, wid = tid >> 6;
    const int wm = wid / WN, wn = wid - wm * WN;
    const float* base = p.ws + ((long)blockIdx.x * p.ksplit * (MT * NT * 16) + (long)ij * 16) * NTHR + tid;
    const long sstride = (long)(MT * NT * 16) * NTHR;
    f32x16 acc[1][1];
#pragma unroll
    for (int r = 0; r < 16; ++r) acc[0][0][r] = 0.f;
    int sidx = 0;
    for (; sidx + 2 <= p.ksplit; sidx += 2) {
        float v0[16], v1[16];
#pragma unroll
        for (int r = 0; r < 16; ++r) { v0[r] = base[sidx * sstride + (long)r * NTHR]; v1[r] = base[(sidx + 1) * sstride + (long)r * NTHR]; }
#pragma unroll
        for (int r = 0; r < 16; ++r) acc[0][0][r] += v0[r] + v1[r];
    }
    if (sidx < p.ksplit) {
#pragma unroll
        for (int r = 0; r < 16; ++r) acc[0][0][r] += base[sidx * sstride + (long)r * NTHR];
    }
    Par par; par.lds = nullptr; par.n0 = 0; par.b0 = 0; par.bnp = 0;
    igemm_epilogue<1, 1, false>(p, acc, tile_m * BM + wm * WTM + i * 32, tile_n * BN + wn * WTN + j * 32, lane, par);
}

template <int WM, int WN, int WTM, int WTN, int NST, int WPE, int AMODE>
__global__ void __launch_bounds__(64 * WM * WN) __attribute__((amdgpu_waves_per_eu(WPE, WPE)))
tile32_kernel(const IGemmArgs p) {
    constexpr int NW = WM * WN;
    constexpr int BM = WM * WTM, BN = WN * WTN;
    constexpr int MT = WTM / 32, NT = WTN / 32;
    constexpr int A_P = BM / 16, B_P = BN / 16, TOT = A_P + B_P;
    constexpr int FULL = TOT / NW, REM = TOT % NW, PPW = FULL + (REM ? 1 : 0);
    constexpr int NM = 2 * MT * NT;
    constexpr int STAGE_BYTES = (BM + BN) * 64;
    constexpr int PAR_OFF = NST * STAGE_BYTES;
    extern __shared__ __attribute__((aligned(16))) char smem[];
    tl_begin(p.tl);

    const int bid = blockIdx.x;
    int wg;
    {
        const int nwg = gridDim.x;
        const int q = nwg >> 3, r = nwg & 7;
        const int xcd = bid & 7, idx = bid >> 3;
        wg = (xcd < r ? xcd * (q + 1) : r * (q + 1) + (xcd - r) * q) + idx;
    }
    int tile_m, tile_n;
    tile_of(p, wg, tile_m, tile_n);
    const int m0 = tile_m * BM, n0 = tile_n * BN;

    const int tid = threadIdx.x, lane = tid & 63;
    const int wid = __builtin_amdgcn_readfirstlane(tid >> 6);
    const int wm = wid / WN, wn = wid - wm * WN;
    const bool extra = REM != 0 && wid < REM;
    const int HW = p.rows_per_batch;

    const int prow = lane >> 2, pchunk = lane & 3;
    const int schunk = pchunk ^ ((prow >> 2) & 3);
    int a_pix[PPW];
    const half_t* b_ptr[PPW];
    int dst[PPW];
#pragma unroll
    for (int q = 0; q < PPW; ++q) {
        const int g = wid + NW * q;
        a_pix[q] = 0; b_ptr[q] = p.w;
        if (g < A_P) {
            int m = m0 + g * 16 + prow;
            m = m < p.M ? m : p.M - 1;
            if constexpr (AMODE == 0) a_pix[q] = m;
            else if constexpr (AMODE == 1) a_pix[q] = padded_pix(m, HW, p.W, p.H);
            else if constexpr (AMODE == 2) {
                const int b = qdiv(m, HW), r2 = m - b * HW, y = qdiv(r2, p.W), x = r2 - y * p.W;
                a_pix[q] = (b * (2 * p.H + 2) + 2 * y + 1 + p.ashift) * (2 * p.W + 2) + 2 * x + 1 + p.ashift;
            } else {
                const int b = qdiv(m, HW), r2 = m - b * HW, y = qdiv(r2, p.W), x = r2 - y * p.W;
                a_pix[q] = (b << 22) | (y << 11) | x;
            }
            dst[q] = g * 16 * 64;
        } else {
            int n = n0 + (g - A_P) * 16 + prow;
            n = n < p.N ? n : p.N - 1;
            b_ptr[q] = p.w + (long)n * p.K + schunk * 8;
            dst[q] = BM * 64 + (g - A_P) * 16 * 64;
        }
    }
    struct Gather { const half_t* src; int cs, Cs, dpix, dy, dx; };
    auto gather_of = [&](int kt) {
        Gather g;
        const int k64 = kt >> 1;
        int tap = 0, cc = k64 << 6;
        if (p.taps == 9) { const int cb = k64 / 9; tap = k64 - cb * 9; cc = cb << 6; }
        const bool s0 = cc < p.C0;
        g.src = s0 ? p.a0 : p.a1;
        g.cs = (s0 ? cc : cc - p.C0) + ((kt & 1) << 5); g.Cs = s0 ? p.C0 : p.C1;
        g.dy = 0; g.dx = 0;
        if (p.taps == 9) { g.dy = tap / 3 - 1; g.dx = tap - (tap / 3) * 3 - 1; }
        g.dpix = 0;
        if constexpr (AMODE == 1) g.dpix = g.dy * (p.W + 2) + g.dx;
        else if constexpr (AMODE == 2) g.dpix = g.dy * (2 * p.W + 2) + g.dx;
        return g;
    };
    auto piece = [&](int q, int kt, int stage, const Gather& g) {
        char* base = smem + stage * STAGE_BYTES;
        const int gi = wid + NW * q;
        if (gi < A_P) {
            int pix;
            if constexpr (AMODE == 3) {
                const int b = a_pix[q] >> 22, y = (a_pix[q] >> 11) & 2047, x = a_pix[q] & 2047;
                const int Hs = p.H >> 1, Ws = p.W >> 1;
                pix = (b * (Hs + 2) + ((y + g.dy) >> 1) + 1) * (Ws + 2) + ((x + g.dx) >> 1) + 1;
            } else {
                pix = a_pix[q] + g.dpix;
            }
            const half_t* gp = g.src + (long)pix * g.Cs + g.cs + schunk * 8;
            __builtin_amdgcn_global_load_lds((const __attribute__((address_space(1))) void*)gp,
                                             (__attribute__((address_space(3))) void*)(base + dst[q]), 16, 0, 0);
        } else {
            __builtin_amdgcn_global_load_lds((const __attribute__((address_space(1))) void*)(b_ptr[q] + ((long)kt << 5)),
                                             (__attribute__((address_space(3))) void*)(base + dst[q]), 16, 0, 0);
        }
    };
    auto dma_tile = [&](int kt, int stage) {
        const Gather g = gather_of(kt);
#pragma unroll
        for (int q = 0; q < PPW; ++q) if (q < FULL || extra) piece(q, kt, stage, g);
    };
#define CFGPP_T32_WAIT(n) do { if (REM != 0 && extra) asm volatile("s_waitcnt vmcnt(%0)" :: "n"((n) * PPW) : "memory");          \
                               else asm volatile("s_waitcnt vmcnt(%0)" :: "n"((n) * FULL) : "memory"); } while (0)

    f32x16 acc[MT][NT];
#pragma unroll
    for (int i = 0; i < MT; ++i)
#pragma unroll
        for (int j = 0; j < NT; ++j)
#pragma unroll
            for (int k = 0; k < 16; ++k) acc[i][j][k] = 0.f;

    const int frow = lane & 31, fhi = lane >> 5;
    const int fsw = (frow >> 2) & 3;
    const int a_rd = (wm * WTM + frow) * 64;
    const int b_rd = BM * 64 + (wn * WTN + frow) * 64;

    const int nk = p.K >> 5;
    tl_stamp(p.tl, 8);
    par_stage<BN, NW>(p, smem + PAR_OFF, n0, m0, wid, lane);
#pragma unroll
    for (int s_ = 0; s_ < NST - 1; ++s_) if (s_ < nk) dma_tile(s_, s_);
    tl_stamp(p.tl, 9);

    auto tile_body = [&](int stage, int ktn, int nxt, auto with_dma) {
        constexpr bool DMA = decltype(with_dma)::value;
        const char* S = smem + stage * STAGE_BYTES;
        Gather gn = {p.a0, 0, p.C0, 0, 0, 0};
        if constexpr (DMA) gn = gather_of(ktn);
        int issued = 0, done = 0;
        auto after_mfma = [&]() {
            ++done;
            if constexpr (DMA) {
                if (issued < PPW && done >= 2 * issued + 1) {
                    __builtin_amdgcn_sched_barrier(0);
                    if (issued < FULL || extra) piece(issued, ktn, nxt, gn);
                    ++issued;
                    __builtin_amdgcn_sched_barrier(0);
                }
            }
        };
        if constexpr (MT * NT <= 8) {
            half8_t xa[2][MT], wb[2][NT];
#pragma unroll
            for (int ks = 0; ks < 2; ++ks) {
                const int coff = (((ks << 1) | fhi) ^ fsw) << 4;
#pragma unroll
                for (int i = 0; i < MT; ++i) xa[ks][i] = *reinterpret_cast<const half8_t*>(S + a_rd + i * 32 * 64 + coff);
#pragma unroll
                for (int j = 0; j < NT; ++j) wb[ks][j] = *reinterpret_cast<const half8_t*>(S + b_rd + j * 32 * 64 + coff);
            }
#pragma unroll
            for (int ks = 0; ks < 2; ++ks)
#pragma unroll
                for (int i = 0; i < MT; ++i)
#pragma unroll
                    for (int j = 0; j < NT; ++j) {
                        acc[i][j] = __builtin_amdgcn_mfma_f32_32x32x16_f16(wb[ks][j], xa[ks][i], acc[i][j], 0, 0, 0);
                        after_mfma();
                    }
        } else {
#pragma unroll
            for (int ks = 0; ks < 2; ++ks) {
                const int coff = (((ks << 1) | fhi) ^ fsw) << 4;
                half8_t xa[MT], wb[NT];
#pragma unroll
                for (int i = 0; i < MT; ++i) xa[i] = *reinterpret_cast<const half8_t*>(S + a_rd + i * 32 * 64 + coff);
#pragma unroll
                for (int j = 0; j < NT; ++j) wb[j] = *reinterpret_cast<const half8_t*>(S + b_rd + j * 32 * 64 + coff);
#pragma unroll
                for (int i = 0; i < MT; ++i)
#pragma unroll
                    for (int j = 0; j < NT; ++j) {
                        acc[i][j] = __builtin_amdgcn_mfma_f32_32x32x16_f16(wb[j], xa[i], acc[i][j], 0, 0, 0);
                        after_mfma();
                    }
                __builtin_amdgcn_sched_barrier(0);
            }
        }
        if constexpr (DMA) {
#pragma unroll
            for (int q = 0; q < PPW; ++q) if (q >= issued && (q < FULL || extra)) piece(q, ktn, nxt, gn);
        }
    };
    int kt = 0, cur = 0, nxt = NST - 1;
    for (; kt + NST - 1 < nk; ++kt) {
        CFGPP_T32_WAIT(NST - 2);
        __builtin_amdgcn_s_barrier();
        asm volatile("" ::: "memory");
        if (kt == 0) tl_stamp(p.tl, 1);
        tile_body(cur, kt + NST - 1, nxt, std::true_type{});
        if (kt == 0) tl_stamp(p.tl, 7);
        cur = cur + 1 == NST ? 0 : cur + 1;
        nxt = nxt + 1 == NST ? 0 : nxt + 1;
    }
    for (; kt < nk; ++kt) {
        asm volatile("s_waitcnt vmcnt(0)" ::: "memory");
        __builtin_amdgcn_s_barrier();
        asm volatile("" ::: "memory");
        tile_body(cur, 0, 0, std::false_type{});
        cur = cur + 1 == NST ? 0 : cur + 1;
    }
#undef CFGPP_T32_WAIT
    asm volatile("s_waitcnt vmcnt(0)" ::: "memory");
    __syncthreads();
    tl_stamp(p.tl, 2);

    const int mw0 = m0 + wm * WTM, nw0 = n0 + wn * WTN;
    Par par;
    par.lds = smem + PAR_OFF; par.n0 = n0; par.b0 = HW > 0 ? qdiv(m0, HW) : 0; par.bnp = par_bnp(BN);
    constexpr bool STAGED_FITS = NW * 32 * (WTN * 2 + 16) <= NST * STAGE_BYTES;
    if (STAGED_FITS && p.epi == EPI_STORE && (p.N & 7) == 0 && p.staged_epi) {
        igemm_epilogue_staged<MT, NT, true>(p, acc, mw0, nw0, lane, smem + wid * (32 * (WTN * 2 + 16)), par);
        tl_end(p.tl);
        return;
    }
    if constexpr (NT % 2 == 0) {
        if (p.epi == EPI_GEGLU && (p.N & 127) == 0 && p.staged_epi && p.omode == 0) {
            igemm_epilogue_geglu_staged<MT, NT, true>(p, acc, mw0, nw0, lane, smem + wid * (32 * ((NT / 2) * 64 + 16)), par);
            tl_end(p.tl);
            return;
        }
    }
    constexpr bool HEADS_FITS = NW * NT * 2560 <= NST * STAGE_BYTES && MT * NT <= 8;
    if constexpr (HEADS_FITS) if (p.epi == EPI_HEADS && p.staged_epi && (p.rows_per_batch & 31) == 0 && (p.part_width & 31) == 0 &&
        (p.head_dim & 7) == 0 && (p.N & 31) == 0 && (p.M & 31) == 0) {
        igemm_epilogue_heads_staged<MT, NT, true>(p, acc, mw0, nw0, lane, smem + wid * (NT * 2560), par);
        tl_end(p.tl);
        return;
    }
    igemm_epilogue<MT, NT, true>(p, acc, mw0, nw0, lane, par);
    tl_end(p.tl);
}

template <bool L = true>
__device__ __forceinline__ void igemm_epilogue_staged16(const IGemmArgs& p, f32x4 (&acc)[2][5], int mw0, int nw0, int lane,
                                                        char* stg , const Par& par) {
    constexpr int WTN = 80, PITCH = WTN * 2 + 16, CPR = WTN / 8, NQ = (32 * CPR + 63) / 64;
    const int c16 = lane & 15, fq = lane >> 4;
    const int HW = p.rows_per_batch;
    const int frow = lane & 31;
    const int mr = mw0 + frow;
    const int mrc = mr < p.M ? mr : p.M - 1;
    int opix = mrc, rpix = mrc;
    if (p.omode == 1 || p.rmode == 1) {
        const int pp = padded_pix(mrc, HW, p.W, p.H);
        if (p.omode == 1) opix = pp;
        if (p.rmode == 1) rpix = pp;
    }
    float4 add[2][5];
#pragma unroll
    for (int i = 0; i < 2; ++i) {
        const int m = mw0 + i * 16 + c16;
        const int mc = m < p.M ? m : p.M - 1;
        const int b = (HW > 0) ? qdiv(mc, HW) : 0;
#pragma unroll
        for (int j = 0; j < 5; ++j) {
            int n = nw0 + j * 16 + 4 * fq;
            n = n < p.N ? n : p.N - 4;
            add[i][j] = make_float4(0.f, 0.f, 0.f, 0.f);
            if (p.bias) add[i][j] = par_bias4<L>(p, par, n);
            if (p.temb) {
                const float4 tt = par_temb4<L>(p, par, b, n);
                add[i][j].x += tt.x; add[i][j].y += tt.y; add[i][j].z += tt.z; add[i][j].w += tt.w;
            }
        }
    }
    half8_t rres[NQ];
    if (p.resid) {
#pragma unroll
        for (int q = 0; q < NQ; ++q) {
            const int c = lane + 64 * q;
            const int r = c / CPR, cc = c - r * CPR;
            const int rp = __shfl(rpix, r);
            int n = nw0 + cc * 8;
            n = n < p.N ? n : p.N - 8;
            rres[q] = *reinterpret_cast<const half8_t*>(p.resid + (long)rp * p.rld + n);
        }
    }
#pragma unroll
    for (int i = 0; i < 2; ++i)
#pragma unroll
        for (int j = 0; j < 5; ++j) {
            const int nl = j * 16 + 4 * fq;
            half4_t o;
            o[0] = (half_t)(acc[i][j][0] * p.out_scale + add[i][j].x);
            o[1] = (half_t)(acc[i][j][1] * p.out_scale + add[i][j].y);
            o[2] = (half_t)(acc[i][j][2] * p.out_scale + add[i][j].z);
            o[3] = (half_t)(acc[i][j][3] * p.out_scale + add[i][j].w);
            *reinterpret_cast<half4_t*>(stg + (i * 16 + c16) * PITCH + nl * 2) = o;
        }
#pragma unroll
    for (int q = 0; q < NQ; ++q) {
        const int c = lane + 64 * q;
        const int r = c / CPR, cc = c - r * CPR;
        const int op = __shfl(opix, r);
        const int mm = mw0 + r, n = nw0 + cc * 8;
        half8_t v = *reinterpret_cast<const half8_t*>(stg + (r & 31) * PITCH + cc * 16);
        if (p.resid) {
#pragma unroll
            for (int k = 0; k < 8; ++k) v[k] = (half_t)((float)v[k] + (float)rres[q][k]);
            if (p.gstat && c < 32 * CPR) *reinterpret_cast<half8_t*>(stg + (r & 31) * PITCH + cc * 16) = v;
        }
        if (c < 32 * CPR && mm < p.M && n < p.N) *reinterpret_cast<half8_t*>(p.out + (long)op * p.old + n) = v;
    }
    if (p.gstat) gstat_block<WTN, PITCH>(p, stg, mw0, nw0, lane);
}

template <bool L = true>
__device__ __forceinline__ void igemm_epilogue_heads_staged16(const IGemmArgs& p, f32x4 (&acc)[2][5], int mw0, int nw0, int lane,
                                                              char* stg , const Par& par) {
    constexpr int BLK = 1536, QK_PITCH = 48, VT_PITCH = 80;
    if (mw0 >= p.M) return;
    const int c16 = lane & 15, fq = lane >> 4;
    const int HW = p.rows_per_batch;
    const int mw0u = __builtin_amdgcn_readfirstlane(mw0);
    const int b = qdiv(mw0u, HW), tok0 = mw0u - b * HW;
    HeadCol hc[5];
#pragma unroll
    for (int j = 0; j < 5; ++j) hc[j] = head_col(p, nw0 + j * 16);
#pragma unroll
    for (int j = 0; j < 5; ++j) {
        const int ng = nw0 + j * 16;
        const int part = hc[j].part;
        char* blk = stg + j * BLK;
        const int n = ng + 4 * fq;
#pragma unroll
        for (int i = 0; i < 2; ++i) {
            const int r = i * 16 + c16;
            float v[4];
#pragma unroll
            for (int k = 0; k < 4; ++k) v[k] = acc[i][j][k];
            if (p.bias) {
                const float4 bb = par_bias4<L>(p, par, n);
                v[0] += bb.x; v[1] += bb.y; v[2] += bb.z; v[3] += bb.w;
            }
            if (part == 2) {
                const int pos = p.vt_linear ? r : cfgpp_vt_pos(r);
#pragma unroll
                for (int k = 0; k < 4; ++k) *reinterpret_cast<half_t*>(blk + (4 * fq + k) * VT_PITCH + pos * 2) = (half_t)v[k];
            } else {
                half4_t o;
#pragma unroll
                for (int k = 0; k < 4; ++k) o[k] = (half_t)v[k];
                *reinterpret_cast<half4_t*>(blk + r * QK_PITCH + (4 * fq) * 2) = o;
            }
        }
    }
#pragma unroll
    for (int j = 0; j < 5; ++j) {
        const int part = hc[j].part;
        const char* blk = stg + j * BLK;
        if (part == 2) {
            const int r = lane >> 2, c4 = lane & 3;
            const half8_t v = *reinterpret_cast<const half8_t*>(blk + r * VT_PITCH + c4 * 16);
            int head, dd;
            head_step(p, hc[j], r, head, dd);
            const long bh = (long)b * p.heads + head;
            *reinterpret_cast<half8_t*>(p.hvt + (bh * p.head_dim_pad + dd) * p.tok_pad + tok0 + 8 * c4) = v;
        } else {
            const int r = lane >> 1, c2 = lane & 1;
            const half8_t v = *reinterpret_cast<const half8_t*>(blk + r * QK_PITCH + c2 * 16);
            int head, dd;
            head_step(p, hc[j], 8 * c2, head, dd);
            const long bh = (long)b * p.heads + head;
            half_t* base = part == 0 ? p.hq : p.hk;
            const int tp = part == 0 ? p.q_tok_pad : p.tok_pad;
            *reinterpret_cast<half8_t*>(base + (bh * tp + tok0 + r) * p.head_dim_pad + dd) = v;
        }
    }
}

template <int AMODE, int NST>
__global__ void __launch_bounds__(512)
igemm16_kernel(const IGemmArgs p) {
    constexpr int BM = 128, BN = 160, RSTEP = 64;
    constexpr int A_CH = BM / RSTEP;
    constexpr int STAGE_BYTES = (BM + BN) * 128;
    constexpr int NM = 20;
    static_assert(NST >= 3 && NST <= 4, "ring depth");
    extern __shared__ __attribute__((aligned(16))) char smem[];
    tl_begin(p.tl);

    const int bid = blockIdx.x;
    int wg;
    {
        const int nwg = gridDim.x;
        const int q = nwg >> 3, r = nwg & 7;
        const int xcd = bid & 7, idx = bid >> 3;
        wg = (xcd < r ? xcd * (q + 1) : r * (q + 1) + (xcd - r) * q) + idx;
    }
    int tile_m, tile_n;
    tile_of(p, wg, tile_m, tile_n);
    const int m0 = tile_m * BM, n0 = tile_n * BN;

    const int tid = threadIdx.x, lane = tid & 63;
    const int wid = __builtin_amdgcn_readfirstlane(tid >> 6);
    const int wm = wid >> 1, wn = wid & 1;
    const bool b3 = wid < 4;

    const int lrow = tid >> 3, lchunk = tid & 7;
    const int HW = p.rows_per_batch;
    int a_pix[A_CH];
#pragma unroll
    for (int j = 0; j < A_CH; ++j) {
        int m = m0 + lrow + j * RSTEP;
        m = m < p.M ? m : p.M - 1;
        if constexpr (AMODE == 0) a_pix[j] = m;
        else if constexpr (AMODE == 1) a_pix[j] = padded_pix(m, HW, p.W, p.H);
        else if constexpr (AMODE == 2) {
            const int b = qdiv(m, HW), q = m - b * HW, y = qdiv(q, p.W), x = q - y * p.W;
            a_pix[j] = (b * (2 * p.H + 2) + 2 * y + 1 + p.ashift) * (2 * p.W + 2) + 2 * x + 1 + p.ashift;
        } else {
            const int b = qdiv(m, HW), q = m - b * HW, y = qdiv(q, p.W), x = q - y * p.W;
            a_pix[j] = (b << 22) | (y << 11) | x;
        }
    }
    const int schunk = lchunk ^ ((lrow >> 1) & 7);
    const half_t* b_ptr[3];
#pragma unroll
    for (int j = 0; j < 3; ++j) {
        int n = n0 + lrow + j * RSTEP;
        n = n < p.N ? n : p.N - 1;
        b_ptr[j] = p.w + (long)n * p.K + schunk * 8;
    }
    const int wave_row0 = wid * 8;

    struct Gather { const half_t* src; int cs, Cs, dpix, dy, dx; };
    auto gather_of = [&](int kt) {
        Gather g;
        int tap = 0, cc = kt << 6;
        if (p.taps == 9) { const int cb = kt / 9; tap = kt - cb * 9; cc = cb << 6; }
        const bool s0 = cc < p.C0;
        g.src = s0 ? p.a0 : p.a1;
        g.cs = s0 ? cc : cc - p.C0; g.Cs = s0 ? p.C0 : p.C1;
        g.dy = 0; g.dx = 0;
        if (p.taps == 9) { g.dy = tap / 3 - 1; g.dx = tap - (tap / 3) * 3 - 1; }
        g.dpix = 0;
        if constexpr (AMODE == 1) g.dpix = g.dy * (p.W + 2) + g.dx;
        else if constexpr (AMODE == 2) g.dpix = g.dy * (2 * p.W + 2) + g.dx;
        return g;
    };
    auto piece = [&](int q, int kt, int stage, const Gather& g) {
        char* As = smem + stage * STAGE_BYTES;
        char* Bs = As + BM * 128;
        if (q < A_CH) {
            const int j = q;
            int pix;
            if constexpr (AMODE == 3) {
                const int b = a_pix[j] >> 22, y = (a_pix[j] >> 11) & 2047, x = a_pix[j] & 2047;
                const int Hs = p.H >> 1, Ws = p.W >> 1;
                pix = (b * (Hs + 2) + ((y + g.dy) >> 1) + 1) * (Ws + 2) + ((x + g.dx) >> 1) + 1;
            } else {
                pix = a_pix[j] + g.dpix;
            }
            const half_t* gp = g.src + (long)pix * g.Cs + g.cs + schunk * 8;
            __builtin_amdgcn_global_load_lds((const __attribute__((address_space(1))) void*)gp,
                                             (__attribute__((address_space(3))) void*)(As + (wave_row0 + j * RSTEP) * 128), 16, 0, 0);
        } else {
            const int j = q - A_CH;
            const half_t* gp = b_ptr[j] + ((long)kt << 6);
            __builtin_amdgcn_global_load_lds((const __attribute__((address_space(1))) void*)gp,
                                             (__attribute__((address_space(3))) void*)(Bs + (wave_row0 + j * RSTEP) * 128), 16, 0, 0);
        }
    };
#define CFGPP_WAIT_TILES(n) do { if (b3) asm volatile("s_waitcnt vmcnt(%0)" :: "n"((n) * 5) : "memory");          \
                                 else asm volatile("s_waitcnt vmcnt(%0)" :: "n"((n) * 4) : "memory"); } while (0)

    f32x4 acc[2][5];
#pragma unroll
    for (int i = 0; i < 2; ++i)
#pragma unroll
        for (int j = 0; j < 5; ++j)
#pragma unroll
            for (int k = 0; k < 4; ++k) acc[i][j][k] = 0.f;

    const int c16 = lane & 15, fq = lane >> 4;
    const int fsw = c16 >> 1;
    const int a_rd = (wm * 32 + c16) * 128;
    const int b_rd = (wn * 80 + c16) * 128;

    const int nk = p.K >> 6;
    tl_stamp(p.tl, 8);
    constexpr int PAR_OFF = NST * STAGE_BYTES;
    par_stage<BN, 8>(p, smem + PAR_OFF, n0, m0, wid, lane);
#pragma unroll
    for (int s_ = 0; s_ < NST - 1; ++s_)
        if (s_ < nk) {
            const Gather g = gather_of(s_);
#pragma unroll
            for (int q = 0; q < 4; ++q) piece(q, s_, s_, g);
            if (b3) piece(4, s_, s_, g);
        }
    tl_stamp(p.tl, 9);
    if (nk >= NST - 1) CFGPP_WAIT_TILES(NST - 2);
    else asm volatile("s_waitcnt vmcnt(0)" ::: "memory");
    __builtin_amdgcn_s_barrier();
    asm volatile("" ::: "memory");
    tl_stamp(p.tl, 1);

    half8_t xa[2][2], wb[2][5];
    auto rd_frags = [&](int s, int stage) {
        const char* As = smem + stage * STAGE_BYTES;
        const char* Bs = As + BM * 128;
        const int coff = (((s << 2) | fq) ^ fsw) << 4;
#pragma unroll
        for (int i = 0; i < 2; ++i) xa[s][i] = *reinterpret_cast<const half8_t*>(As + a_rd + i * 16 * 128 + coff);
#pragma unroll
        for (int j = 0; j < 5; ++j) wb[s][j] = *reinterpret_cast<const half8_t*>(Bs + b_rd + j * 16 * 128 + coff);
    };
    rd_frags(0, 0);

    auto tile_body = [&](int kt, int cur, int ktn, int nxt, auto with_dma) {
        constexpr bool DMA = decltype(with_dma)::value;
        Gather gn = {p.a0, 0, p.C0, 0, 0, 0};
        if constexpr (DMA) gn = gather_of(ktn);
        auto phase = [&](auto s_tag) {
            constexpr int s = decltype(s_tag)::value;
            const bool mine = (s == 0) == b3;
#pragma unroll
            for (int m = 0; m < 10; ++m) {
                const int i = m / 5, j = m - 5 * (m / 5);
                acc[i][j] = __builtin_amdgcn_mfma_f32_16x16x32_f16(wb[s][j], xa[s][i], acc[i][j], 0, 0, 0);
                if (m == 0) {
                    __builtin_amdgcn_sched_barrier(0);
                    if (s == 0) rd_frags(1, cur);
                    else if (kt + 1 < nk) rd_frags(0, (kt + 1) % NST);
                    __builtin_amdgcn_sched_barrier(0);
                }
                if constexpr (DMA) {
                    if ((m & 1) == 1) {
                        const int q = m >> 1;
                        __builtin_amdgcn_sched_barrier(0);
                        if (mine && (q < 4 || b3)) piece(q, ktn, nxt, gn);
                        __builtin_amdgcn_sched_barrier(0);
                    }
                }
            }
        };
        phase(std::integral_constant<int, 0>{});
        if constexpr (DMA) {
            if (b3) asm volatile("s_waitcnt vmcnt(%0)" :: "n"((NST - 2) * 5) : "memory");
            else asm volatile("s_waitcnt vmcnt(%0)" :: "n"((NST - 3) * 4) : "memory");
        } else {
            asm volatile("s_waitcnt vmcnt(0)" ::: "memory");
        }
        asm volatile("s_waitcnt lgkmcnt(0)" ::: "memory");
        __builtin_amdgcn_s_barrier();
        asm volatile("" ::: "memory");
        phase(std::integral_constant<int, 1>{});
    };
    int kt = 0;
    for (; kt + NST - 1 < nk; ++kt) {
        tile_body(kt, kt % NST, kt + NST - 1, (kt + NST - 1) % NST, std::true_type{});
        if (kt == 0) tl_stamp(p.tl, 7);
    }
    for (; kt < nk; ++kt) tile_body(kt, kt % NST, 0, 0, std::false_type{});
    tl_stamp(p.tl, 2);
#undef CFGPP_WAIT_TILES

    Par par;
    par.lds = smem + PAR_OFF; par.n0 = n0; par.b0 = HW > 0 ? qdiv(m0, HW) : 0; par.bnp = par_bnp(BN);
    if (p.epi == EPI_HEADS) igemm_epilogue_heads_staged16(p, acc, m0 + wm * 32, n0 + wn * 80, lane, smem + wid * (5 * 1536), par);
    else igemm_epilogue_staged16(p, acc, m0 + wm * 32, n0 + wn * 80, lane, smem + wid * (32 * 176), par);
    tl_end(p.tl);
}

static unsigned long long* g_tl = nullptr; static long g_tl_cap = 0; static int g_tl_target = -1, g_tl_count = 0;
static int g_tl_info[12] = {0};
static unsigned long long* tl_take(int cfg, int grid, int threads, int BM, int BN, int NST, const IGemmArgs& a) {
    if (!a.tl || grid > g_tl_cap) return nullptr;
    const int info[12] = {cfg, grid, threads, BM, BN, NST, a.ksplit, a.n_major, a.M, a.N, a.K, a.epi};
    for (int i = 0; i < 12; ++i) g_tl_info[i] = info[i];
    return g_tl;
}
constexpr long WS_BYTES = 128L << 20;
static std::map<hipStream_t, float*> g_ws_by_stream;
static float* ws_for(hipStream_t stream) {
    auto it = g_ws_by_stream.find(stream);
    if (it != g_ws_by_stream.end()) return it->second;
    float* p = nullptr;
    if (hipMalloc((void**)&p, (size_t)WS_BYTES) != hipSuccess) p = nullptr;
    if (p) g_ws_by_stream[stream] = p;
    return p;
}
static int g_staged_epi = 1;
static int g_last_hint_applied = 1;
extern "C" void cfgpp_igemm_set_staged_epilogue(int on) { g_staged_epi = on ? 1 : 0; }
static int g_big_tiles = 1;
extern "C" void cfgpp_igemm_set_big_tiles(int on) { g_big_tiles = on ? 1 : 0; }
static int g_tail_split = 1;
static int g_n_major = -1;
extern "C" void cfgpp_igemm_set_n_major(int mode) { g_n_major = mode; }

static int par_slots(const IGemmArgs& a, int BM) {
    if (a.temb == nullptr || a.rows_per_batch <= 0) return 0;
    const int HW = a.rows_per_batch, nbatch = cdiv(a.M, HW);
    const int span = (BM + HW - 1) / HW + 1;
    return span < nbatch ? span : nbatch;
}

static int g_walk_blocked = 1;
extern "C" void cfgpp_igemm_set_blocked_walk(int on) { g_walk_blocked = on ? 1 : 0; }
static void walk_plan(IGemmArgs& a, int BM, int BN, int ntm, int ntn, int smem) {
    a.walk_bn = 0; a.walk_per = 0; a.walk_tmb = 0; a.walk_tnb = 0;
    const int T = ntm * ntn;
    if (!g_walk_blocked || a.walk_hint || (T & 7) || T < 64 || a.ksplit > 1 || a.n_main != T) return;
    const int per = T >> 3;
    int wpc = smem > 0 ? (160 * 1024) / smem : 1;
    wpc = wpc < 1 ? 1 : wpc > 4 ? 4 : wpc;
    const int R = 32 * wpc;
    const double a_row = 2.0 * BM * (a.C0 + a.C1) * (a.amode == 2 ? 4.0 : a.amode == 3 ? 0.25 : 1.0);
    const double w_col = 2.0 * BN * a.K;
    auto cost = [&](auto tile_at) {
        double tot = 0.0;
        for (int r0 = 0; r0 < per; r0 += R) {
            unsigned long long seen_m[8] = {0}, seen_n[8] = {0};
            int nm = 0, nn = 0;
            for (int i = r0; i < per && i < r0 + R; ++i) {
                int tm, tn; tile_at(i, tm, tn);
                if (tm < 512 && !((seen_m[tm >> 6] >> (tm & 63)) & 1ull)) { seen_m[tm >> 6] |= 1ull << (tm & 63); ++nm; }
                if (tn < 512 && !((seen_n[tn >> 6] >> (tn & 63)) & 1ull)) { seen_n[tn >> 6] |= 1ull << (tn & 63); ++nn; }
            }
            tot += nm * a_row + nn * w_col;
        }
        return tot;
    };
    if (ntm > 512 || ntn > 512) return;
    const int div1 = a.n_major ? ntm : ntn;
    const double now = cost([&](int i, int& tm, int& tn) { const int q = i / div1, r = i - q * div1; tm = a.n_major ? r : q; tn = a.n_major ? q : r; });
    double best = now; int best_bn = 0, best_inner = 0, best_tmb = 0, best_tnb = 0;
    for (int bn : {4, 2}) {
        const int bm = 8 / bn;
        if (ntm % bm || ntn % bn) continue;
        const int tmb = ntm / bm, tnb = ntn / bn;
        for (int inner = 0; inner < 2; ++inner) {
            const double c = cost([&](int i, int& tm, int& tn) {
                if (inner) { tn = i / tmb; tm = i - tn * tmb; } else { tm = i / tnb; tn = i - tm * tnb; } });
            if (c < best) { best = c; best_bn = bn; best_inner = inner; best_tmb = tmb; best_tnb = tnb; }
        }
    }
    if (best_bn && best <= 0.85 * now) {
        a.walk_bn = best_bn; a.walk_per = per; a.walk_tmb = best_tmb; a.walk_tnb = best_tnb; a.n_major = best_inner;
    }
}

extern "C" void cfgpp_igemm_walk_plan_probe(int M, int N, int K, int BM, int BN, int smem, int n_major, int* out5) {
    IGemmArgs a; std::memset(&a, 0, sizeof(a));
    a.M = M; a.N = N; a.K = K; a.C0 = K; a.amode = 0; a.ksplit = 1; a.n_major = n_major;
    const int ntm = cdiv(M, BM), ntn = cdiv(N, BN);
    a.n_main = ntm * ntn;
    walk_plan(a, BM, BN, ntm, ntn, smem);
    out5[0] = a.walk_bn ? 8 / a.walk_bn : 0; out5[1] = a.walk_bn; out5[2] = a.walk_tmb; out5[3] = a.walk_tnb; out5[4] = a.n_major;
}

static void stats_decide(IGemmArgs& a, bool staged_store) {
    const bool on = a.gstat != nullptr && staged_store && a.epi == EPI_STORE && (a.N & 7) == 0 && (a.M & 31) == 0 && a.ksplit <= 1 && a.n_main > 0;
    if (!on) a.gstat = nullptr;
    if (a.stat_flag) *a.stat_flag = on ? 1 : 0;
}

template <int WM, int WN, int WTM, int WTN, bool GLDS, int AMODE, int NST = 2>
int launch_cfg_amode(const IGemmArgs& a_in, hipStream_t stream) {
    constexpr int BM = WM * WTM, BN = WN * WTN, NTHR = 64 * WM * WN;
    constexpr int smem_std = NST * (BM + BN) * 128 + (GLDS ? par_bytes(BN) : 0);
    static_assert(smem_std <= 160 * 1024, "tile does not fit the LDS");
    constexpr int blocks_per_cu = (160 * 1024) / smem_std < 8 ? (160 * 1024) / smem_std : 8;
    constexpr int slots = 256 * blocks_per_cu;
    IGemmArgs a = a_in;
    a.par_nb = par_slots(a, BM);
    const int smem = NST * (BM + BN) * 128 + (GLDS ? par_bytes(BN, a.par_nb > PAR_NB ? a.par_nb : PAR_NB) : 0);
    if (smem > 160 * 1024) {
        if constexpr (WM * WTM > 64 || WN * WTN > 64 || NST != 2) { g_last_hint_applied = 0; return launch_cfg_amode<2, 2, 32, 32, GLDS, AMODE, 2>(a_in, stream); }
        else { cfgpp_set_error("igemm: %d time-embedding rows per tile do not fit the LDS", a.par_nb); return -2; }
    }
    static int attr_smem = 0;
    auto kern = igemm_kernel<WM, WN, WTM, WTN, GLDS, AMODE, NST>;
    if (smem > attr_smem) {
        CFGPP_HIP_CHECK(hipFuncSetAttribute(reinterpret_cast<const void*>(kern),
                                            hipFuncAttributeMaxDynamicSharedMemorySize, smem));
        attr_smem = smem;
    }
    const int T = cdiv(a.M, BM) * cdiv(a.N, BN);
    const int KT = a.K >> 6;
    a.n_main = T; a.ksplit = 1; a.ws = nullptr; a.staged_epi = g_staged_epi;
    {
        const double w_bytes = 2.0 * a.N * a.K, a_bytes = 2.0 * a.M * (a.C0 + a.C1) * (a.amode == 2 ? 4.0 : a.amode == 3 ? 0.25 : 1.0);
        a.n_major = (g_n_major == 1 || (g_n_major < 0 && w_bytes > 1.5 * a_bytes && cdiv(a.N, BN) >= 8)) ? 1 : 0;
        if (g_n_major < 0 && a.walk_hint) a.n_major = a.walk_hint == 2 ? 1 : 0;
    }
    {
        int S = 0;
        if (a_in.split >= 2 && a.epi == EPI_STORE) S = a_in.split < KT ? a_in.split : KT;
        else if (g_tail_split && a_in.allow_split && (WTM == 64 && WTN == 64) && a.epi == EPI_STORE && T * 2 <= slots && KT >= 32) {
            S = g_tail_split == 2 ? (slots + T - 1) / T : slots / T;
            if (KT / S < 12) S = KT / 12;
            if (S > 16) S = 16;
        }
        if (S >= 2 && (long)T * S * BM * BN * 4 <= (a_in.ws_buf ? a_in.ws_bytes : WS_BYTES)) {
            float* const ws = a_in.ws_buf ? a_in.ws_buf : ws_for(stream);
            if (ws) { a.n_main = 0; a.ksplit = S; a.ws = ws; }
        }
    }
    const int n_tail = T - a.n_main;
    stats_decide(a, WM * WN * 32 * (WTN * 2 + 16) <= NST * (BM + BN) * 128 && a.staged_epi && n_tail == 0);
    if (n_tail > 0) a.n_major = 0;
    a.walk_div = a.n_major ? cdiv(a.M, BM) : cdiv(a.N, BN);
    walk_plan(a, BM, BN, cdiv(a.M, BM), cdiv(a.N, BN), smem);
    a.tl = tl_take(WM * 100 + WN * 10 + (GLDS ? 1 : 0), a.n_main + n_tail * a.ksplit, NTHR, BM, BN, NST, a);
    hipLaunchKernelGGL(kern, dim3(a.n_main + n_tail * a.ksplit), dim3(NTHR), smem, stream, a);
    if (n_tail > 0)
        hipLaunchKernelGGL((igemm_reduce_kernel<WM, WN, WTM, WTN>), dim3(n_tail, (WTM / 32) * (WTN / 32)), dim3(NTHR), 0, stream, a);
    CFGPP_HIP_CHECK(hipGetLastError());
    return 0;
}

template <int WM, int WN, int WTM, int WTN, bool GLDS, int NST = 2>
int launch_cfg(const IGemmArgs& a, hipStream_t stream) {
    switch (a.amode) {
        case 0: return launch_cfg_amode<WM, WN, WTM, WTN, GLDS, 0, NST>(a, stream);
        case 1: return launch_cfg_amode<WM, WN, WTM, WTN, GLDS, 1, NST>(a, stream);
        case 2: return launch_cfg_amode<WM, WN, WTM, WTN, GLDS, 2, NST>(a, stream);
        case 3: return launch_cfg_amode<WM, WN, WTM, WTN, GLDS, 3, NST>(a, stream);
        default: cfgpp_set_error("igemm: bad amode %d", a.amode); return -2;
    }
}

template <int WM, int WN, int WTM, int WTN, int NST, int WPE, int AMODE>
int launch_tile32_amode(const IGemmArgs& a_in, hipStream_t stream) {
    constexpr int BM = WM * WTM, BN = WN * WTN, NTHR = 64 * WM * WN;
    constexpr int WGS = WPE * 4 / (WM * WN);
    static_assert((NST * (BM + BN) * 64 + par_bytes(BN)) * WGS <= 160 * 1024, "the workgroups that are meant to share a CU do not fit its LDS");
    IGemmArgs a = a_in;
    a.par_nb = par_slots(a, BM);
    const int nb = a.temb ? (a.par_nb > PAR_NB ? a.par_nb : PAR_NB) : 0;
    const int smem = NST * (BM + BN) * 64 + par_bytes(BN, nb);
    if (smem > 160 * 1024) { g_last_hint_applied = 0; return launch_cfg_amode<2, 2, 32, 32, true, AMODE, 2>(a_in, stream); }
    if (WGS > 1 && smem * WGS > 160 * 1024) {
        g_last_hint_applied = 0;
        return launch_cfg_amode<2, 2, 64, 64, true, AMODE, 2>(a_in, stream);
    }
    static int attr_smem = 0;
    auto kern = tile32_kernel<WM, WN, WTM, WTN, NST, WPE, AMODE>;
    if (smem > attr_smem) {
        CFGPP_HIP_CHECK(hipFuncSetAttribute(reinterpret_cast<const void*>(kern), hipFuncAttributeMaxDynamicSharedMemorySize, smem));
        attr_smem = smem;
    }
    const int ntm = cdiv(a.M, BM), ntn = cdiv(a.N, BN);
    a.n_main = ntm * ntn; a.ksplit = 1; a.ws = nullptr; a.staged_epi = g_staged_epi;
    const double w_bytes = 2.0 * a.N * a.K, a_bytes = 2.0 * a.M * (a.C0 + a.C1) * (a.amode == 2 ? 4.0 : a.amode == 3 ? 0.25 : 1.0);
    a.n_major = (g_n_major == 1 || (g_n_major < 0 && w_bytes > 1.5 * a_bytes && ntn >= 8)) ? 1 : 0;
    if (g_n_major < 0 && a.walk_hint) a.n_major = a.walk_hint == 2 ? 1 : 0;
    a.walk_div = a.n_major ? ntm : ntn;
    walk_plan(a, BM, BN, ntm, ntn, smem);
    stats_decide(a, NTHR / 64 * 32 * (WTN * 2 + 16) <= NST * (BM + BN) * 64 && a.staged_epi);
    a.tl = tl_take(3200 + WM * 100 + WN * 10, a.n_main, NTHR, BM, BN, NST, a);
    hipLaunchKernelGGL(kern, dim3(a.n_main), dim3(NTHR), smem, stream, a);
    CFGPP_HIP_CHECK(hipGetLastError());
    return 0;
}
template <int WM, int WN, int WTM, int WTN, int NST, int WPE>
int launch_tile32(const IGemmArgs& a, hipStream_t stream) {
    switch (a.amode) {
        case 0: return launch_tile32_amode<WM, WN, WTM, WTN, NST, WPE, 0>(a, stream);
        case 1: return launch_tile32_amode<WM, WN, WTM, WTN, NST, WPE, 1>(a, stream);
        case 2: return launch_tile32_amode<WM, WN, WTM, WTN, NST, WPE, 2>(a, stream);
        case 3: return launch_tile32_amode<WM, WN, WTM, WTN, NST, WPE, 3>(a, stream);
        default: cfgpp_set_error("igemm: bad amode %d", a.amode); return -2;
    }
}

}

static int g_mf16_heads = 1;
extern "C" void cfgpp_igemm_set_mf16_heads(int on) { g_mf16_heads = on ? 1 : 0; }
static bool mf16_supports(const IGemmArgs& a) {
    if (a.N % 160 != 0 || !g_staged_epi || a.K < 64) return false;
    if (a.epi == EPI_STORE) return true;
    return a.epi == EPI_HEADS && g_mf16_heads && a.rows_per_batch % 32 == 0 && a.M % 32 == 0 && a.part_width % 16 == 0 &&
           a.head_dim % 8 == 0;
}
template <int AMODE, int NST>
int launch_mf16_amode(const IGemmArgs& a_in, hipStream_t stream) {
    IGemmArgs a = a_in;
    a.par_nb = par_slots(a, 128);
    const int smem = NST * (128 + 160) * 128 + par_bytes(160, a.par_nb > PAR_NB ? a.par_nb : PAR_NB);
    if (smem > 160 * 1024) { g_last_hint_applied = 0; return launch_cfg_amode<4, 1, 32, 160, true, AMODE, 2>(a_in, stream); }
    static int attr_smem = 0;
    auto kern = igemm16_kernel<AMODE, NST>;
    if (smem > attr_smem) {
        CFGPP_HIP_CHECK(hipFuncSetAttribute(reinterpret_cast<const void*>(kern), hipFuncAttributeMaxDynamicSharedMemorySize, smem));
        attr_smem = smem;
    }
    const int ntm = cdiv(a.M, 128), ntn = a.N / 160;
    a.n_main = ntm * ntn; a.ksplit = 1; a.ws = nullptr; a.staged_epi = 1;
    const double w_bytes = 2.0 * a.N * a.K, a_bytes = 2.0 * a.M * (a.C0 + a.C1) * (a.amode == 2 ? 4.0 : a.amode == 3 ? 0.25 : 1.0);
    a.n_major = (g_n_major == 1 || (g_n_major < 0 && w_bytes > 1.5 * a_bytes && ntn >= 8)) ? 1 : 0;
    if (g_n_major < 0 && a.walk_hint) a.n_major = a.walk_hint == 2 ? 1 : 0;
    a.walk_div = a.n_major ? ntm : ntn;
    walk_plan(a, 128, 160, ntm, ntn, smem);
    stats_decide(a, true);
    a.tl = tl_take(16, a.n_main, 512, 128, 160, NST, a);
    hipLaunchKernelGGL(kern, dim3(a.n_main), dim3(512), smem, stream, a);
    CFGPP_HIP_CHECK(hipGetLastError());
    return 0;
}
template <int NST>
int launch_mf16(const IGemmArgs& a, hipStream_t stream) {
    switch (a.amode) {
        case 0: return launch_mf16_amode<0, NST>(a, stream);
        case 1: return launch_mf16_amode<1, NST>(a, stream);
        case 2: return launch_mf16_amode<2, NST>(a, stream);
        case 3: return launch_mf16_amode<3, NST>(a, stream);
        default: cfgpp_set_error("igemm: bad amode %d", a.amode); return -2;
    }
}

static int big4_smem(int cfg, const IGemmArgs& a) {
    int BM, BN; big4_tile(cfg, &BM, &BN);
    const int nb = a.temb ? par_slots(a, BM) : 0;
    return 2 * (BM + BN) * 128 + big4_par_bytes(BN, nb);
}
static bool big4_ok(int cfg, const IGemmArgs& a) { return big4_supports(cfg, a, g_staged_epi != 0) && big4_smem(cfg, a) <= 160 * 1024; }
static int launch_big4(int cfg, const IGemmArgs& a_in, hipStream_t stream) {
    int BM, BN; big4_tile(cfg, &BM, &BN);
    IGemmArgs a = a_in;
    a.par_nb = par_slots(a, BM);
    const int smem = big4_smem(cfg, a);
    const int ntm = cdiv(a.M, BM), ntn = cdiv(a.N, BN);
    a.n_main = ntm * ntn; a.ksplit = 1; a.ws = nullptr; a.staged_epi = 1;
    const double w_bytes = 2.0 * a.N * a.K, a_bytes = 2.0 * a.M * (a.C0 + a.C1) * (a.amode == 2 ? 4.0 : a.amode == 3 ? 0.25 : 1.0);
    a.n_major = (g_n_major == 1 || (g_n_major < 0 && w_bytes > 1.5 * a_bytes && ntn >= 8)) ? 1 : 0;
    if (g_n_major < 0 && a.walk_hint) a.n_major = a.walk_hint == 2 ? 1 : 0;
    a.walk_div = a.n_major ? ntm : ntn;
    walk_plan(a, BM, BN, ntm, ntn, smem);
    stats_decide(a, true);
    a.tl = tl_take(4000 + cfg, a.n_main, 256, BM, BN, 2, a);
    return big4_run(cfg, a, a.n_main, smem, stream);
}

static bool big4p_ok(const IGemmArgs& a) { return big4p_supports(a, g_staged_epi != 0) && big4p_smem(big4_par_bytes(256, 0)) <= 160 * 1024; }
static int launch_big4p(const IGemmArgs& a_in, hipStream_t stream) {
    IGemmArgs a = a_in;
    a.par_nb = 0;
    const int pb = big4_par_bytes(256, 0), smem = big4p_smem(pb);
    const int ntm = cdiv(a.M, 256), ntn = cdiv(a.N, 256);
    a.n_main = ntm * ntn; a.ksplit = 1; a.ws = nullptr; a.staged_epi = 1; a.tl = nullptr;
    const double w_bytes = 2.0 * a.N * a.K, a_bytes = 2.0 * a.M * a.C0;
    a.n_major = (g_n_major == 1 || (g_n_major < 0 && w_bytes > 1.5 * a_bytes && ntn >= 8)) ? 1 : 0;
    if (g_n_major < 0 && a.walk_hint) a.n_major = a.walk_hint == 2 ? 1 : 0;
    a.walk_div = a.n_major ? ntm : ntn;
    walk_plan(a, 256, 256, ntm, ntn, smem);
    stats_decide(a, true);
    return big4p_run(a, a.n_main < 256 ? a.n_main : 256, smem, pb, stream);
}

static int g_force_cfg = 0;
static int g_staging = 1;
extern "C" void cfgpp_igemm_force_config(int cfg) { g_force_cfg = cfg; }
extern "C" void cfgpp_igemm_set_staging(int glds) { g_staging = glds ? 1 : 0; }
extern "C" void cfgpp_igemm_set_tail_split(int on) { g_tail_split = on == 2 ? 2 : on ? 1 : 0; }

static int launch_config(int cfg, const IGemmArgs& a, hipStream_t stream) {
    bool glds = g_staging != 0;
    if (cfg > 20 && cfg < 24) { cfg -= 20; glds = false; }
    switch (cfg) {
        case 1: return glds ? launch_cfg<2, 2, 64, 64, true>(a, stream) : launch_cfg<2, 2, 64, 64, false>(a, stream);
        case 2: return glds ? launch_cfg<4, 1, 64, 64, true>(a, stream) : launch_cfg<4, 1, 64, 64, false>(a, stream);
        case 3: return glds ? launch_cfg<2, 2, 32, 32, true>(a, stream) : launch_cfg<2, 2, 32, 32, false>(a, stream);
        case 4: return launch_cfg<2, 4, 128, 64, true>(a, stream);
        case 5: return launch_cfg<4, 2, 64, 160, true>(a, stream);
        case 6: return launch_cfg<4, 2, 64, 64, true>(a, stream);
        case 7: return launch_cfg<4, 1, 32, 160, true>(a, stream);
        case 8: return launch_cfg<4, 2, 32, 160, true>(a, stream);
        case 9: return launch_cfg<4, 1, 32, 160, true, 3>(a, stream);
        case 11: return launch_cfg<4, 1, 32, 160, true, 4>(a, stream);
        case 12: return launch_cfg<2, 2, 64, 64, true, 3>(a, stream);
        case 14: return launch_cfg<4, 2, 64, 64, true, 3>(a, stream);
        case 10: return launch_cfg<8, 1, 32, 320, true>(a, stream);
        case 15: return launch_tile32<4, 2, 64, 64, 3, 4>(a, stream);
        case 16: return launch_tile32<2, 2, 64, 64, 3, 3>(a, stream);
        case 17: return launch_tile32<4, 1, 64, 64, 3, 2>(a, stream);
        case 13: return launch_tile32<2, 4, 128, 64, 4, 2>(a, stream);
        case 27: if (a.epi != EPI_STORE) return launch_tile32<2, 2, 64, 64, 3, 3>(a, stream);
                 return launch_tile32<2, 2, 64, 160, 2, 2>(a, stream);
        case 20: if (a.epi == EPI_GEGLU) return launch_tile32<2, 4, 128, 64, 4, 2>(a, stream);
                 return launch_tile32<4, 2, 64, 160, 4, 2>(a, stream);
        case 18: return mf16_supports(a) ? launch_mf16<3>(a, stream) : launch_cfg<4, 1, 32, 160, true>(a, stream);
        case 19: return mf16_supports(a) ? launch_mf16<4>(a, stream) : launch_cfg<4, 1, 32, 160, true>(a, stream);
        case 24: case 25: case 26: return big4_ok(cfg, a) ? launch_big4(cfg, a, stream) : launch_cfg<2, 2, 64, 64, true>(a, stream);
        case 28: return big4p_ok(a) ? launch_big4p(a, stream) : launch_cfg<2, 2, 64, 64, true>(a, stream);
        default: cfgpp_set_error("igemm: bad config %d", cfg); return -2;
    }
}

static int g_autotune = 1;
extern "C" void cfgpp_igemm_set_autotune(int on) { g_autotune = on ? 1 : 0; }
static int g_split_cfg = 14;
extern "C" void cfgpp_igemm_set_split_tile(int cfg) { g_split_cfg = (cfg == 1 || cfg == 12) ? cfg : 14; }
static int g_mf16 = 4;
extern "C" void cfgpp_igemm_set_mf16(int mode) { g_mf16 = (mode == 3 || mode == 4) ? mode : 0; }
static int g_mf16_linear = 1;
extern "C" void cfgpp_igemm_set_mf16_linear(int on) { g_mf16_linear = on ? 1 : 0; }
static int g_mf16_rounds = 2;
extern "C" void cfgpp_igemm_set_mf16_rounds(int n) { g_mf16_rounds = n >= 1 ? n : 1; }
static int g_force_split = 0;
extern "C" void cfgpp_igemm_force_split(int s) { g_force_split = s >= 2 ? s : 0; }
static int g_big_split_min_kt = 0;
extern "C" void cfgpp_igemm_set_big_split(int min_kt) { g_big_split_min_kt = min_kt > 0 ? min_kt : 0; }
int igemm_autotune_enabled() { return g_autotune && g_force_cfg == 0 && g_staging != 0; }
static unsigned g_tune_mask = 0xf1ffffffu;
extern "C" void cfgpp_igemm_set_tune_mask(unsigned mask) { g_tune_mask = mask; }
unsigned igemm_tune_mask() { return g_tune_mask; }
extern "C" unsigned cfgpp_igemm_tuner_state(void) {
    return g_tune_mask ^ ((unsigned)g_big_tiles << 1) ^ ((unsigned)g_tail_split << 3) ^ ((unsigned)(g_n_major + 1) << 6) ^ ((unsigned)g_walk_blocked << 9) ^
           ((unsigned)g_staged_epi << 10) ^ ((unsigned)g_force_cfg << 12) ^ ((unsigned)g_staging << 20);
}

extern "C" void cfgpp_igemm_timeline(void* buf, long cap_blocks, int target) {
    g_tl = (unsigned long long*)buf; g_tl_cap = buf ? cap_blocks : 0; g_tl_target = buf ? target : -1; g_tl_count = 0;
}
extern "C" void cfgpp_igemm_timeline_info(int* out12) { for (int i = 0; i < 12; ++i) out12[i] = g_tl_info[i]; }

int igemm_last_hint_applied() { return g_last_hint_applied; }

int igemm_launch(const IGemmArgs& a_in, hipStream_t stream) {
    IGemmArgs a = a_in;
    g_last_hint_applied = (a_in.cfg_hint & 63) == 0 ? 1 : 0;
    a.allow_split = 1;
    a.tl = nullptr;
    if (g_tl) { if (g_tl_count == g_tl_target) a.tl = g_tl; ++g_tl_count; }
    const int Cin = a.C0 + a.C1;
    CFGPP_REQUIRE(a.C0 > 0 && a.C0 % 64 == 0 && a.C1 % 64 == 0, "igemm: C0=%d C1=%d must be multiples of 64", a.C0, a.C1);
    CFGPP_REQUIRE(a.taps == 1 || a.taps == 9, "igemm: taps=%d", a.taps);
    CFGPP_REQUIRE(a.K == a.taps * Cin, "igemm: K=%d != taps*Cin=%d", a.K, a.taps * Cin);
    CFGPP_REQUIRE(a.N % 4 == 0 && a.M > 0 && a.N > 0, "igemm: M=%d N=%d (N must be a multiple of 4)", a.M, a.N);
    CFGPP_REQUIRE(a.amode == 0 || (a.H > 0 && a.W > 0 && a.rows_per_batch == a.H * a.W), "igemm: spatial args");
    CFGPP_REQUIRE(a.amode != 3 || (a.H < 2048 && a.W < 2048 && (a.M / a.rows_per_batch) < 512), "igemm: upsample range");
    CFGPP_REQUIRE(a.epi != EPI_GEGLU || a.N % 64 == 0, "igemm: GEGLU needs N %% 64 == 0");
    CFGPP_REQUIRE(a.epi != EPI_HEADS || (a.head_dim % 4 == 0 && a.part_width % 4 == 0), "igemm: heads args");
    CFGPP_REQUIRE(a.rows_per_batch <= 0 || a.M / a.rows_per_batch < (1 << 20), "igemm: %d rows in batches of %d (batch index must stay below 2^20)", a.M, a.rows_per_batch);
    int cfg = g_force_cfg;
    if (cfg == 0) {
        const long t128 = (long)cdiv(a.M, 128) * cdiv(a.N, 128);
        const long t256x64 = (long)cdiv(a.M, 256) * cdiv(a.N, 64);
        const bool n_odd64 = (a.N % 128) != 0;
        const int KT = a.K >> 6;
        const long t5 = (a.N % 320 == 0) ? (long)cdiv(a.M, 256) * (a.N / 320) : 0;
        const long t4 = (a.N % 256 == 0) ? (long)cdiv(a.M, 256) * (a.N / 256) : 0;
        auto fills = [](long t) { return t >= 224 && (t % 256 == 0 || t % 256 >= 160 || t >= 1024); };
        if (g_big_tiles && a.epi != EPI_GEGLU && a.K >= 1280 && fills(t5)) cfg = 5;
        else if (g_big_tiles && t4 >= 192 && (t4 % 256 == 0 || t4 % 256 >= 128 || t4 >= 512)) cfg = 4;
        else
        if (t128 >= 256 && !n_odd64) cfg = 1;
        else if (t256x64 >= 256 && (n_odd64 || a.N <= 64)) cfg = 2;
        else if (t128 >= 200) cfg = 1;
        else if (g_tail_split && KT >= 32 && t128 >= 8 && a.epi == EPI_STORE) cfg = g_split_cfg;
        else cfg = 3;
        if (a.epi == EPI_GEGLU && cfg == 3) cfg = 1;
    }
    bool big_split = false;
    a.split = 0;
    if (g_force_cfg != 0) a.split = g_force_split;
    else if (g_big_split_min_kt > 0 && g_big_tiles && g_staging != 0 && g_tail_split && a.epi == EPI_STORE && a.N % 320 == 0) {
        const long t8 = (long)cdiv(a.M, 128) * (a.N / 320);
        const int KT = a.K >> 6;
        if (t8 >= 64 && t8 <= 128) {
            int S = (int)(256 / t8);
            while (S >= 2 && KT / S < g_big_split_min_kt) --S;
            if (S >= 2 && t8 * S >= 192) { cfg = 8; a.split = S; big_split = true; }
        }
    }
    if (g_force_cfg == 0 && g_mf16 != 0 && g_staging != 0 && !big_split && mf16_supports(a) && (g_mf16_linear || a.amode != 0)) {
        const long t7 = (long)cdiv(a.M, 128) * (a.N / 160);
        const bool full_rounds = t7 > 256 && t7 % 256 == 0 && t7 / 256 <= g_mf16_rounds;
        if ((t7 >= 200 && t7 <= 256) || full_rounds) return launch_config(g_mf16 == 4 ? 19 : 18, a, stream);
    }
    if (g_force_cfg == 0 && a.cfg_hint > 0 && g_staging != 0 && !big_split) {
        const int KT = a.K >> 6;
        const long t128 = (long)cdiv(a.M, 128) * cdiv(a.N, 128);
        const long t_rule = cfg == 14 ? (long)cdiv(a.M, 256) * cdiv(a.N, 128) : t128;
        const bool rule_splits = (cfg == 1 || cfg == 12 || cfg == 14) && g_tail_split && a.epi == EPI_STORE && KT >= 32 && t_rule * 2 <= (cfg == 1 ? 512 : 256);
        const int h = a.cfg_hint & 63;
        const bool valid = (h == 1 || h == 4 || h == 6 || h == 12 || h == 14 || (h == 10 && a.epi == EPI_GEGLU) ||
                            ((h == 5 || h == 7 || h == 8 || h == 9 || h == 11) && a.epi != EPI_GEGLU) ||
                            h == 13 || h == 15 || h == 16 || h == 17 || (h == 20 && a.epi != EPI_GEGLU) || (h == 27 && a.epi == EPI_STORE) || ((h >= 24 && h <= 26) && big4_ok(h, a)) || (h == 28 && big4p_ok(a))) && (g_big_tiles || h == 1);
        if (!rule_splits && valid) { cfg = h; a.allow_split = 0; g_last_hint_applied = 1; }
    }
    a.walk_hint = (g_force_cfg == 0 && g_staging != 0) ? (a.cfg_hint >> 6) & 3 : 0;
    return launch_config(cfg, a, stream);
}
```

### cfgpp_amd/csrc/lora_kernels.hip

```cpp
#include "common.h"

namespace {

constexpr int LORA_BO = 32, LORA_BK = 128, LORA_RC = 32, LORA_UP_LD = 36;

template <int KIND>
__global__ __launch_bounds__(256) void lora_merge_kernel(const half_t* __restrict__ base, half_t* __restrict__ dst,
                                                         const float* __restrict__ up, const float* __restrict__ down, int rank,
                                                         int O, int Kc, int taps, int vec2) {
    __shared__ __attribute__((aligned(16))) float up_s[LORA_RC][LORA_UP_LD];
    __shared__ __attribute__((aligned(16))) float down_s[LORA_RC][LORA_BK];
    const int tid = threadIdx.x, lane = tid & 63, wave = tid >> 6;
    const int p0 = blockIdx.y * LORA_BO, k0 = blockIdx.x * LORA_BK;

    const int u_r = tid & 31, u_row = tid >> 5;
    const int d_col = tid & 127, d_r = tid >> 7;
    long u_src[4];
#pragma unroll
    for (int i = 0; i < 4; ++i) {
        const int p = p0 + u_row + 8 * i;
        long o = p;
        if (KIND == 2) { const int w = p & 63; o = (long)(p >> 6) * 32 + (w & 31) + (w >= 32 ? O / 2 : 0); }
        u_src[i] = p < O ? o * rank : -1;
    }
    long d_src = -1;
    {
        const int k = k0 + d_col;
        if (k < Kc) {
            d_src = k;
            if (KIND == 1) { const int q = k >> 6; d_src = ((long)(q / taps) * 64 + (k & 63)) * taps + q % taps; }
        }
    }

    float acc[8][2];
#pragma unroll
    for (int i = 0; i < 8; ++i) { acc[i][0] = 0.f; acc[i][1] = 0.f; }

    for (int r0 = 0; r0 < rank; r0 += LORA_RC) {
        const bool u_live = r0 + u_r < rank;
#pragma unroll
        for (int i = 0; i < 4; ++i) up_s[u_r][u_row + 8 * i] = (u_live && u_src[i] >= 0) ? up[u_src[i] + r0 + u_r] : 0.f;
#pragma unroll
        for (int i = 0; i < LORA_RC / 2; ++i) {
            const int r = r0 + d_r + 2 * i;
            down_s[d_r + 2 * i][d_col] = (d_src >= 0 && r < rank) ? down[(long)r * Kc + d_src] : 0.f;
        }
        __syncthreads();
        const int rn = min(LORA_RC, rank - r0);
#pragma unroll 4
        for (int r = 0; r < rn; ++r) {
            const float2 d = *reinterpret_cast<const float2*>(&down_s[r][2 * lane]);
            const float4 a = *reinterpret_cast<const float4*>(&up_s[r][8 * wave]);
            const float4 b = *reinterpret_cast<const float4*>(&up_s[r][8 * wave + 4]);
            const float uu[8] = {a.x, a.y, a.z, a.w, b.x, b.y, b.z, b.w};
#pragma unroll
            for (int i = 0; i < 8; ++i) { acc[i][0] = fmaf(uu[i], d.x, acc[i][0]); acc[i][1] = fmaf(uu[i], d.y, acc[i][1]); }
        }
        __syncthreads();
    }

    const int k = k0 + 2 * lane;
    if (k >= Kc) return;
#pragma unroll
    for (int i = 0; i < 8; ++i) {
        const int p = p0 + 8 * wave + i;
        if (p >= O) break;
        const long off = (long)p * Kc + k;
        if (vec2) {
            const half2_t w = *reinterpret_cast<const half2_t*>(base + off);
            half2_t o;
            o.x = (half_t)((float)w.x + acc[i][0]); o.y = (half_t)((float)w.y + acc[i][1]);
            *reinterpret_cast<half2_t*>(dst + off) = o;
        } else {
            dst[off] = (half_t)((float)base[off] + acc[i][0]);
            if (k + 1 < Kc) dst[off + 1] = (half_t)((float)base[off + 1] + acc[i][1]);
        }
    }
}

}

int lora_merge_launch(const half_t* base, half_t* dst, const float* up, const float* down, int rank, int kind, long O, long I,
                      int taps, hipStream_t s) {
    const long Kc = I * taps;
    CFGPP_REQUIRE(base && dst && up && down && rank > 0 && O > 0 && Kc > 0 && O < (1L << 30) && Kc < (1L << 30), "lora_merge: bad args");
    CFGPP_REQUIRE(kind != 1 || I % 64 == 0, "lora_merge: conv3x3 repack with %ld input channels (a multiple of 64)", I);
    CFGPP_REQUIRE(kind != 2 || O % 64 == 0, "lora_merge: GEGLU interleave with %ld rows (a multiple of 64)", O);
    const dim3 grid((unsigned)cdiv(Kc, LORA_BK), (unsigned)cdiv(O, LORA_BO));
    CFGPP_REQUIRE(grid.y <= 65535u, "lora_merge: %ld rows", O);
    const int vec2 = Kc % 2 == 0 ? 1 : 0;
    if (kind == 1) hipLaunchKernelGGL(lora_merge_kernel<1>, grid, dim3(256), 0, s, base, dst, up, down, rank, (int)O, (int)Kc, taps, vec2);
    else if (kind == 2) hipLaunchKernelGGL(lora_merge_kernel<2>, grid, dim3(256), 0, s, base, dst, up, down, rank, (int)O, (int)Kc, taps, vec2);
    else hipLaunchKernelGGL(lora_merge_kernel<0>, grid, dim3(256), 0, s, base, dst, up, down, rank, (int)O, (int)Kc, taps, vec2);
    CFGPP_HIP_CHECK(hipGetLastError());
    return 0;
}
```

### cfgpp_amd/csrc/unet.hip

```cpp
#include "engine_base.h"

struct cfgpp_unet : EngineBase {
    cfgpp_unet_config cfg;
    int device = 0;
    bool finalized = false;

    std::vector<Op> ctx_plan;
    const void* in_z = nullptr; int in_z_half = 0; int in_z_rows = 0; float in_t = 0.f; void* out_eps = nullptr;
    const float* in_t_dev = nullptr;
    half_t* d_cond = nullptr; int cond_rows = 0;
    float* d_step_tab = nullptr; int step_tab_cap = 0; float* d_step_cur = nullptr; int* d_step_idx = nullptr;
    hipStream_t cap_stream = nullptr;
    struct GraphKey { const void* z; void* z0t; void* eps; const void* euc; const void* ec; int z_half, z_rows, rows, tw, rn; float lam; long n; int tuned_serial; int cond_rows;
                      int ip_active = 0, ip_n_img = 0; unsigned ip_scale_bits = 0;
                      int ctx_tokens = 77; };
    struct Graph { GraphKey key; hipGraph_t graph; hipGraphExec_t exec; };
    std::vector<Graph> graphs;
    int tuned_serial = 0;
    int prefix_ops = 0;
    double prefix_macs_per_row = 0;
    int ran_shared = -1;
    bool shares(int rows, int z_rows) const;
    bool enter_call(int rows, int z_rows) {
        const bool sh = shares(rows, z_rows);
// ... 1053 lines not shown
    for (int k = 0; k < 4; ++k) { out_ms[k] = 0; out_flops[k] = 0; out_launches[k] = 0; }
    if (rc == 0) {
        for (size_t i = 0; i < n; ++i) {
            if (op_rows[i] == 0) continue;
            float ms = 0.f; hipEventElapsedTime(&ms, ev[i], ev[i + 1]);
            const int k = u->plan_kind[i];
            out_ms[k] += ms; out_flops[k] += 2.0 * u->plan_macs[i] * op_rows[i]; out_launches[k] += 1;
        }
        if (detail && detail_cap > 0) {
            std::string txt;
            for (size_t i = 0; i < n; ++i) {
                if (op_rows[i] == 0) continue;
                float ms = 0.f; hipEventElapsedTime(&ms, ev[i], ev[i + 1]);
                char line[256];
                const std::string desc = u->plan_desc[i] + (op_rows[i] != rows ? " rows=" + std::to_string(op_rows[i]) : std::string());
                snprintf(line, sizeof(line), "%zu\t%d\t%s\t%.1f\t%.3f\n", i, u->plan_kind[i], desc.c_str(), ms * 1e3,
                         2.0 * u->plan_macs[i] * op_rows[i] * 1e-9);
                txt += line;
            }
            const long ncopy = std::min<long>((long)txt.size(), detail_cap - 1);
            std::memcpy(detail, txt.data(), ncopy); detail[ncopy] = 0;
        }
    }
    for (auto& e : ev) hipEventDestroy(e);
    return rc;
}

int cfgpp_unet_tuning(cfgpp_unet* u, int rows, int* hints, int cap, int set) {
    CFGPP_REQUIRE(u && u->finalized && hints && rows > 0, "unet_tuning: bad args");
    const int n = (int)u->cfg_hints.size();
    CFGPP_REQUIRE(cap >= n, "unet_tuning: buffer of %d for %d launches", cap, n);
    if (set) {
        for (int sh = 0; sh < 2; ++sh) u->tuned_by_rows[std::make_pair(rows, sh != 0)] = std::vector<int>(hints, hints + n);
        if (u->tuned_rows == rows) u->tuned_rows = 0;
        ++u->tuned_serial;
        return n;
    }
    auto it = u->tuned_by_rows.find(std::make_pair(rows, u->ran_shared == 1));
    if (it == u->tuned_by_rows.end()) { cfgpp_set_error("unet_tuning: batch %d has not been tuned", rows); return -3; }
    std::copy(it->second.begin(), it->second.end(), hints);
    return n;
}

double cfgpp_unet_flops(cfgpp_unet* u, int rows) {
    if (!u || !u->finalized) return 0.0;
    const double once = u->ran_shared == 1 ? u->prefix_macs_per_row * (rows / 2) : 0.0;
    const double ip = u->ip_active ? u->ip_macs_per_key * u->ip_n_img : 0.0;
    const double text = u->ip_macs_per_key * (u->ctx_tokens - 77);
    return 2.0 * ((u->macs_per_row + u->attn_macs_per_row + text + ip) * rows - once);
}

void cfgpp_unet_set_share_prefix(int on) { g_share_prefix = on ? 1 : 0; }
int cfgpp_unet_share_prefix_enabled(void) { return g_share_prefix; }
int cfgpp_unet_shared_prefix_ops(cfgpp_unet* u, int rows, int z_rows) {
    if (!u || !u->finalized) return 0;
    return u->shares(rows, z_rows) ? u->prefix_ops : 0;
}
double cfgpp_unet_device_bytes(cfgpp_unet* u) { return u ? u->dev_bytes : 0.0; }

static WeightSlot* lora_slot(cfgpp_unet* u, const char* key, const char* who) {
    if (!u || !key) { cfgpp_set_error("%s: null argument", who); return nullptr; }
    if (!u->finalized) { cfgpp_set_error("%s: %s: the engine is not finalized (weights are merged into the uploaded, repacked matrices)", who, key); return nullptr; }
    const std::string k = key;
    if (k == "conv_in.weight" || k == "conv_out.weight") {
        cfgpp_set_error("%s: %s runs on the fp32 small-kernel path and takes no adapter", who, key); return nullptr;
    }
    auto it = u->params.find(k);
    if (it == u->params.end()) { cfgpp_set_error("%s: unknown key %s", who, key); return nullptr; }
    if (!it->second.is_matrix) { cfgpp_set_error("%s: %s is a 1-D parameter (bias / norm): adapters apply to matrices", who, key); return nullptr; }
    auto sl = u->slots.find(k);
    if (sl == u->slots.end()) { cfgpp_set_error("%s: %s is not held as an fp16 matrix (fp32 direct-convolution path)", who, key); return nullptr; }
    return &sl->second;
}

int cfgpp_unet_lora(cfgpp_unet* u, const char* key, const float* up, const float* down, int rank, void* stream) {
    WeightSlot* w = lora_slot(u, key, "lora");
    if (!w) return -2;
    CFGPP_REQUIRE(rank >= 0, "lora: %s: rank %d", key, rank);
    CFGPP_REQUIRE(rank == 0 || (up && down), "lora: %s: rank %d with a null up / down matrix", key, rank);
    CFGPP_HIP_CHECK(hipSetDevice(u->device));
    hipStream_t s = (hipStream_t)stream;
    const size_t bytes = (size_t)w->O * w->K() * sizeof(half_t);
    if (rank == 0) {
        if (w->base) CFGPP_HIP_CHECK(hipMemcpyAsync(w->rows(), w->base, bytes, hipMemcpyDeviceToDevice, s));
        return 0;
    }
    if (!w->base) {
        half_t* b = (half_t*)u->dmalloc(bytes, false);
        CFGPP_REQUIRE(b, "lora: %s: out of device memory for the saved base (%zu bytes)", key, bytes);
        CFGPP_HIP_CHECK(hipMemcpyAsync(b, w->rows(), bytes, hipMemcpyDeviceToDevice, s));
        w->base = b;
    }
    const int kind = w->kind == SLOT_MEMBER ? SLOT_PLAIN : w->kind;
    int e = lora_merge_launch(w->base, w->rows(), up, down, rank, kind, w->O, w->I, w->taps, s);
    if (e) { const std::string m = cfgpp_last_error(); cfgpp_set_error("lora: %s: %s", key, m.c_str()); }
    return e;
}

int cfgpp_unet_read_weight(cfgpp_unet* u, const char* key, void* host_fp16_out) {
    WeightSlot* w = lora_slot(u, key, "read_weight");
    if (!w) return -2;
    CFGPP_REQUIRE(host_fp16_out, "read_weight: %s: null output", key);
    const long O = w->O, Kc = w->K(), I = w->I; const int taps = w->taps;
    std::vector<half_t> r((size_t)O * Kc);
    CFGPP_HIP_CHECK(hipSetDevice(u->device));
    CFGPP_HIP_CHECK(hipDeviceSynchronize());
    CFGPP_HIP_CHECK(hipMemcpy(r.data(), w->rows(), r.size() * sizeof(half_t), hipMemcpyDeviceToHost));
    half_t* out = (half_t*)host_fp16_out;
    for (long p = 0; p < O; ++p) {
        long o = p;
        if (w->kind == SLOT_GEGLU) { const long q = p & 63; o = (p >> 6) * 32 + (q & 31) + (q >= 32 ? O / 2 : 0); }
        const half_t* src = &r[(size_t)p * Kc];
        half_t* dst = out + (size_t)o * Kc;
        if (w->kind == SLOT_CONV3) {
            for (long i = 0; i < I; ++i) for (int t = 0; t < taps; ++t) dst[i * taps + t] = src[((i >> 6) * taps + t) * 64 + (i & 63)];
        } else {
            std::memcpy(dst, src, Kc * sizeof(half_t));
        }
    }
    return 0;
}

static float* g_op_gstat = nullptr;
static int g_op_gstat_flag = 0;
void cfgpp_op_igemm_set_gstat(void* buf) { g_op_gstat = (float*)buf; }
int cfgpp_op_igemm_gstat_written() { return g_op_gstat_flag; }

int cfgpp_op_igemm(const void* a0, const void* a1, int C0, int C1, int taps, int amode, int H, int W,
                   const void* w, int M, int N, const float* bias, const float* temb, int temb_ld,
                   const void* resid, int rmode, int rld, void* out, int omode, int old_, int epi, void* stream) {
    IGemmArgs a = base_args();
    a.a0 = (const half_t*)a0; a.a1 = (const half_t*)a1; a.C0 = C0; a.C1 = C1; a.taps = taps; a.amode = amode; a.H = H; a.W = W;
    a.w = (const half_t*)w; a.M = M; a.N = N; a.K = taps * (C0 + C1); a.bias = bias; a.temb = temb; a.temb_ld = temb_ld;
    a.rows_per_batch = H * W; a.resid = (const half_t*)resid; a.rmode = rmode; a.rld = rld;
    a.out = (half_t*)out; a.omode = omode; a.old = old_; a.epi = epi;
    a.gstat = g_op_gstat; a.stat_flag = &g_op_gstat_flag; g_op_gstat_flag = 0;
    return igemm_launch(a, (hipStream_t)stream);
}

int cfgpp_op_igemm_heads(const void* a_, int K, const void* w, int M, int N, const float* bias, int rows_per_batch,
                         void* hq, void* hk, void* hvt, int part0, int part_width, int head_dim, int heads,
                         int q_tok_pad, int tok_pad, void* stream) {
    IGemmArgs a = base_args();
    a.a0 = (const half_t*)a_; a.C0 = K; a.amode = 0; a.w = (const half_t*)w; a.M = M; a.N = N; a.K = K; a.bias = bias;
    a.epi = EPI_HEADS; a.rows_per_batch = rows_per_batch; a.hq = (half_t*)hq; a.hk = (half_t*)hk; a.hvt = (half_t*)hvt;
    a.part0 = part0; a.part_width = part_width; a.head_dim = head_dim; a.head_dim_pad = round_up(head_dim, 32);
    a.heads = heads; a.q_tok_pad = q_tok_pad; a.tok_pad = tok_pad;
    return igemm_launch(a, (hipStream_t)stream);
}

}
```

Baseline: 8.595 images/sec.

## Fold nearest-upsample 3x3 convs into four 2x2 phase convolutions

Nearest-neighbour 2x upsample followed by a 3x3 conv is rewritten as four sub-pixel phase convolutions with 2x2 folded weights (K=4C instead of 9C). The phase weights are precomputed by a new fold kernel, and the implicit-GEMM kernel gains an amode 4 that selects phase from the tile index and writes interleaved output rows. This targets the redundant MACs in the SD1.5 UNet upsampler convs. It costs extra weight memory, refolding on LoRA updates, fp16 rounding from the summed weights, and excludes big4 tiles and split paths for these layers.

```diff
diff --git a/cfgpp_amd/_lib.py b/cfgpp_amd/_lib.py
--- a/cfgpp_amd/_lib.py
+++ b/cfgpp_amd/_lib.py
@@ -121,6 +121,11 @@
     "cfgpp_op_f16_to_f32_rows": (_I, [_P, _P, _I, _I, _I, _I, _P]),
     "cfgpp_op_igemm": (_I, [_P, _P, _I, _I, _I, _I, _I, _I, _P, _I, _I, _P, _P, _I, _P, _I, _I, _P, _I, _I, _I, _P]),
     "cfgpp_op_igemm_heads": (_I, [_P, _I, _P, _I, _I, _P, _I, _P, _P, _P, _I, _I, _I, _I, _I, _I, _P]),
+    "cfgpp_op_fold_upsample": (_I, [_P, _P, _I, _I, _P]),
+    "cfgpp_op_upsample_conv3x3": (_I, [_P, _I, _I, _I, _P, _P, _I, _I, _P, _P, _P]),
+    "cfgpp_igemm_set_upsample_phase": (None, [_I]),
+    "cfgpp_igemm_last_amode": (_I, []),
+    "cfgpp_igemm_last_config_ran": (_I, []),
     "cfgpp_igemm_force_config": (None, [_I]),
     "cfgpp_igemm_set_staging": (None, [_I]),
     "cfgpp_igemm_set_staged_epilogue": (None, [_I]),
diff --git a/cfgpp_amd/csrc/big4.h b/cfgpp_amd/csrc/big4.h
--- a/cfgpp_amd/csrc/big4.h
+++ b/cfgpp_amd/csrc/big4.h
@@ -7,6 +7,7 @@
 }
 inline bool big4_supports(int cfg, const IGemmArgs& a, bool staged_epi) {
     if (cfg < 24 || cfg > 26 || !staged_epi || a.K < 64) return false;
+    if (a.amode == 4) return false;
     const long rows = a.amode == 0 ? (long)a.M : a.amode == 2 ? (long)(a.M / a.rows_per_batch) * (2 * a.H + 2) * (2 * a.W + 2)
                                                 : (long)(a.M / a.rows_per_batch) * (a.H + 2) * (a.W + 2);
     const long cmax = a.C0 > a.C1 ? a.C0 : a.C1;
diff --git a/cfgpp_amd/csrc/cfgpp_debug.h b/cfgpp_amd/csrc/cfgpp_debug.h
--- a/cfgpp_amd/csrc/cfgpp_debug.h
+++ b/cfgpp_amd/csrc/cfgpp_debug.h
@@ -74,6 +74,12 @@
                    const void* w, int M, int N, const float* bias, const float* temb, int temb_ld,
                    const void* resid, int rmode, int rld, void* out, int omode, int old_, int epi,
                    void* stream);
+int cfgpp_op_fold_upsample(const void* w9, void* w4, int O, int I, void* stream);
+int cfgpp_op_upsample_conv3x3(const void* src, int C, int Hs, int Ws, const void* w9, const void* w4, int rows, int N,
+                              const float* bias, void* out, void* stream);
+void cfgpp_igemm_set_upsample_phase(int on);
+int cfgpp_igemm_last_amode(void);
+int cfgpp_igemm_last_config_ran(void);
 int cfgpp_op_igemm_heads(const void* a, int K, const void* w, int M, int N, const float* bias, int rows_per_batch,
                          void* hq, void* hk, void* hvt, int part0, int part_width, int head_dim, int heads,
                          int q_tok_pad, int tok_pad, void* stream);
diff --git a/cfgpp_amd/csrc/engine_base.h b/cfgpp_amd/csrc/engine_base.h
--- a/cfgpp_amd/csrc/engine_base.h
+++ b/cfgpp_amd/csrc/engine_base.h
@@ -175,6 +175,20 @@
             t.gst = (float*)dmalloc((size_t)max_rows * (H * W / 32) * C * 2 * sizeof(float), false);
         return t;
     }
+    struct FoldSite { const half_t* w9; half_t* w4; long O, I; };
+    std::vector<FoldSite> folds;
+    half_t* fold_site(const half_t* w9, long O, long I) {
+        half_t* w4 = (half_t*)dmalloc((size_t)16 * O * I * sizeof(half_t), false);
+        if (!w4) return nullptr;
+        if (igemm_fold_upsample_launch(w9, w4, O, I, nullptr) != 0 || hipStreamSynchronize(nullptr) != hipSuccess) return nullptr;
+        folds.push_back({w9, w4, O, I});
+        return w4;
+    }
+    int refold(const half_t* w9, hipStream_t s) {
+        for (const FoldSite& f : folds)
+            if (f.w9 == w9) { const int e = igemm_fold_upsample_launch(f.w9, f.w4, f.O, f.I, s); if (e) return e; }
+        return 0;
+    }
     void rel(const Tensor& t) { if (t.p) pool[std::make_tuple(t.H, t.W, t.C)].push_back(std::make_pair(t.p, t.gst)); }
     ~EngineBase() { for (void* p : allocs) hipFree(p); }
 };
@@ -305,6 +319,8 @@
     return a;
 }
 
+inline bool upsample_phase_form(int Hs, int Ws, int N) { return igemm_upsample_phase_enabled() && Hs >= 8 && Ws >= 8 && N % 8 == 0; }
+
 struct Plan {
     EngineBase* u;
     Builder* B;
@@ -320,10 +336,19 @@
         a.out = dst.p; a.omode = 1; a.old = dst.C; a.epi = EPI_STORE;
         a.gstat = dst.gst; a.stat_flag = dst.gst ? dst.gst_ok : nullptr;
         const int HW = dst.H * dst.W;
+        std::string issued;
+        if (amode == 3 && !resid && !temb && upsample_phase_form(src.H, src.W, dst.C)) {
+            half_t* w4 = u->fold_site(w, dst.C, src.C);
+            if (!w4) { B->ok = false; B->err = "folded upsampler weight: out of device memory"; }
+            else {
+                a.amode = amode = 4; a.taps = 4; a.w = w4; a.K = 4 * src.C;
+                issued = " as 4x2x2 K=" + std::to_string(a.K);
+            }
+        }
         u->macs_per_row += (double)HW * dst.C * 9.0 * src.C;
         int* hint = u->new_hint(ops == &u->plan);
         ops->push_back([a, HW, hint](hipStream_t s, int rows) mutable { IGemmArgs b = a; b.M = rows * HW; b.cfg_hint = *hint; return igemm_launch(b, s); });
-        if (ops == &u->plan) u->tag(0, (double)HW * dst.C * 9.0 * src.C, "conv3x3 amode=" + std::to_string(amode) + " HW=" + std::to_string(HW) + " N=" + std::to_string(dst.C) + " K=" + std::to_string(9 * src.C) + (resid ? " +res" : "") + (temb ? " +temb" : ""));
+        if (ops == &u->plan) u->tag(0, (double)HW * dst.C * 9.0 * src.C, "conv3x3 amode=" + std::to_string(amode) + " HW=" + std::to_string(HW) + " N=" + std::to_string(dst.C) + " K=" + std::to_string(9 * src.C) + issued + (resid ? " +res" : "") + (temb ? " +temb" : ""));
     }
     void conv1x1(const Tensor& s0, const Tensor* s1, const Tensor& dst, const half_t* w, const float* bias) {
         IGemmArgs a = base_args(u);
diff --git a/cfgpp_amd/csrc/igemm.h b/cfgpp_amd/csrc/igemm.h
--- a/cfgpp_amd/csrc/igemm.h
+++ b/cfgpp_amd/csrc/igemm.h
@@ -48,6 +48,7 @@
     int walk_div;
     int walk_hint;
     int walk_bn, walk_per, walk_tmb, walk_tnb;
+    int ph_tiles;
     int split;
     int par_nb;
     unsigned long long* tl;
@@ -56,4 +57,6 @@
 int igemm_launch(const IGemmArgs& a, hipStream_t stream);
 int igemm_autotune_enabled();
 int igemm_last_hint_applied();
+int igemm_upsample_phase_enabled();
+int igemm_fold_upsample_launch(const half_t* w9, half_t* w4, long O, long I, hipStream_t stream);
 unsigned igemm_tune_mask();
diff --git a/cfgpp_amd/csrc/igemm_device.h b/cfgpp_amd/csrc/igemm_device.h
--- a/cfgpp_amd/csrc/igemm_device.h
+++ b/cfgpp_amd/csrc/igemm_device.h
@@ -41,6 +41,14 @@
     const int b = qdiv(m, HW), p = m - b * HW;
     const int y = qdiv(p, W), x = p - y * W;
     return (b * (H + 2) + y + 1) * (W + 2) + x + 1;
+}
+__device__ __forceinline__ int phase_pix(int m, int HW, int W, int H, int phase) {
+    const int b = qdiv(m, HW), p = m - b * HW;
+    const int i = qdiv(p, W), j = p - i * W;
+    return (b * (2 * H + 2) + 2 * i + (phase >> 1) + 1) * (2 * W + 2) + 2 * j + (phase & 1) + 1;
+}
+__device__ __forceinline__ int phase_src_pix(int m, int HW, int W, int H, int phase) {
+    return padded_pix(m, HW, W, H) + ((phase >> 1) - 1) * (W + 2) + (phase & 1) - 1;
 }
 
 
@@ -58,6 +66,16 @@
         tile_m = p.n_major ? wr : wq; tile_n = p.n_major ? wq : wr;
     }
 }
+template <int AMODE>
+__device__ __forceinline__ int phase_of(const IGemmArgs& p, int& tile_m) {
+    if constexpr (AMODE == 4) {
+        const int ph = qdiv_u(tile_m, p.ph_tiles);
+        tile_m = __builtin_amdgcn_readfirstlane(tile_m - ph * p.ph_tiles);
+        return ph;
+    } else {
+        return 0;
+    }
+}
 
 constexpr int PAR_NB = 5;
 __host__ __device__ constexpr int par_bnp(int BN) { return (BN + 63) / 64 * 64; }
@@ -65,6 +83,7 @@
 struct Par {
     const char* lds;
     int n0, b0, bnp;
+    int phase = 0;
 };
 template <int BN, int NW>
 __device__ __forceinline__ void par_stage(const IGemmArgs& p, char* par, int n0, int m0, int wid, int lane) {
@@ -117,7 +136,7 @@
         for (int j = 0; j < NT; ++j) asm volatile("" : "+a"(row[j]));
     }
 }
-template <int MT, int NT, bool L>
+template <int MT, int NT, bool L, int AMODE = 0>
 __device__ __forceinline__ void igemm_epilogue(const IGemmArgs& p, f32x16 (&acc)[MT][NT], int mw0, int nw0, int lane, const Par& par) {
     const int frow = lane & 31, fhi = lane >> 5;
     const int HW = p.rows_per_batch;
@@ -128,7 +147,9 @@
         const int b = (HW > 0) ? qdiv(m, HW) : 0;
         const int tok = m - b * HW;
         long orow = m, rrow = m;
-        if (p.omode == 1 || p.rmode == 1) {
+        if constexpr (AMODE == 4) {
+            orow = phase_pix(m, HW, p.W, p.H, par.phase);
+        } else if (p.omode == 1 || p.rmode == 1) {
             const long pp = padded_pix(m, HW, p.W, p.H);
             if (p.omode == 1) orow = pp;
             if (p.rmode == 1) rrow = pp;
@@ -224,9 +245,15 @@
 }
 
 template <int WTN, int PITCH>
-__device__ __forceinline__ void gstat_block(const IGemmArgs& p, const char* stg, int m_blk0, int nw0, int lane) {
+__device__ __forceinline__ void gstat_block(const IGemmArgs& p, const char* stg, int m_blk0, int nw0, int lane, int phase = -1) {
     if (m_blk0 >= p.M) return;
-    float* dst = p.gstat + ((long)(m_blk0 >> 5) * p.N + nw0) * 2;
+    int slot = m_blk0 >> 5;
+    if (phase >= 0) {
+        const int bps = p.rows_per_batch >> 5;
+        slot = __builtin_amdgcn_readfirstlane(slot);
+        slot += (3 * qdiv_u(slot, bps) + phase) * bps;
+    }
+    float* dst = p.gstat + ((long)slot * p.N + nw0) * 2;
 #pragma unroll 1
     for (int cp = lane; cp < WTN / 2; cp += 64) {
         const half2_t x0 = *reinterpret_cast<const half2_t*>(stg + cp * 4);
@@ -244,7 +271,7 @@
     }
 }
 
-template <int MT, int NT, bool L, bool PIN = false>
+template <int MT, int NT, bool L, bool PIN = false, int AMODE = 0>
 __device__ __forceinline__ void igemm_epilogue_staged(const IGemmArgs& p, f32x16 (&acc)[MT][NT], int mw0, int nw0, int lane,
                                                       char* stg , const Par& par) {
     constexpr int WTN = NT * 32;
@@ -261,7 +288,9 @@
         const int mc = m < p.M ? m : p.M - 1;
         const int b = (HW > 0) ? qdiv(mc, HW) : 0;
         int opix = mc, rpix = mc;
-        if (p.omode == 1 || p.rmode == 1) {
+        if constexpr (AMODE == 4) {
+            opix = phase_pix(mc, HW, p.W, p.H, par.phase);
+        } else if (p.omode == 1 || p.rmode == 1) {
             const int pp = padded_pix(mc, HW, p.W, p.H);
             if (p.omode == 1) opix = pp;
             if (p.rmode == 1) rpix = pp;
@@ -317,7 +346,7 @@
             }
             if (c < 32 * CPR && mm < p.M && n < p.N) *reinterpret_cast<half8_t*>(p.out + (long)op * p.old + n) = v;
         }
-        if (p.gstat) gstat_block<WTN, PITCH>(p, stg, mw0 + i * 32, nw0, lane);
+        if (p.gstat) gstat_block<WTN, PITCH>(p, stg, mw0 + i * 32, nw0, lane, AMODE == 4 ? par.phase : -1);
     }
 }
 
diff --git a/cfgpp_amd/csrc/igemm_kernel.hip b/cfgpp_amd/csrc/igemm_kernel.hip
--- a/cfgpp_amd/csrc/igemm_kernel.hip
+++ b/cfgpp_amd/csrc/igemm_kernel.hip
@@ -43,6 +43,7 @@
     }
     int tile_m, tile_n;
     tile_of(p, wg, tile_m, tile_n);
+    const int phase = phase_of<AMODE>(p, tile_m);
     const int m0 = tile_m * BM, n0 = tile_n * BN;
 
     const int tid = threadIdx.x, lane = tid & 63, wid = tid >> 6;
@@ -61,6 +62,8 @@
         else if constexpr (AMODE == 2) {
             const int b = qdiv(m, HW), q = m - b * HW, y = qdiv(q, p.W), x = q - y * p.W;
             a_pix[j] = (b * (2 * p.H + 2) + 2 * y + 1 + p.ashift) * (2 * p.W + 2) + 2 * x + 1 + p.ashift;
+        } else if constexpr (AMODE == 4) {
+            a_pix[j] = phase_src_pix(m, HW, p.W, p.H, phase);
         } else {
             const int b = qdiv(m, HW), q = m - b * HW, y = qdiv(q, p.W), x = q - y * p.W;
             a_pix[j] = (b << 22) | (y << 11) | x;
@@ -72,7 +75,7 @@
     for (int j = 0; j < B_CH; ++j) {
         int n = n0 + lrow + j * RSTEP;
         n = n < p.N ? n : p.N - 1;
-        b_ptr[j] = p.w + (long)n * p.K + schunk * 8;
+        b_ptr[j] = p.w + ((long)phase * p.N + n) * p.K + schunk * 8;
     }
     int st_off[(A_CH > B_CH ? A_CH : B_CH)];
 #pragma unroll
@@ -88,7 +91,8 @@
 
     auto load_tile = [&](int kt) {
         int tap = 0, cc = kt << 6;
-        if (p.taps == 9) { const int cb = kt / 9; tap = kt - cb * 9; cc = cb << 6; }
+        if constexpr (AMODE == 4) { tap = kt & 3; cc = (kt >> 2) << 6; }
+        else if (p.taps == 9) { const int cb = kt / 9; tap = kt - cb * 9; cc = cb << 6; }
         const bool s0 = cc < p.C0;
         const half_t* src = s0 ? p.a0 : p.a1;
         const int cs = s0 ? cc : cc - p.C0, Cs = s0 ? p.C0 : p.C1;
@@ -97,6 +101,7 @@
         int dpix = 0;
         if constexpr (AMODE == 1) dpix = dy * (p.W + 2) + dx;
         else if constexpr (AMODE == 2) dpix = dy * (2 * p.W + 2) + dx;
+        else if constexpr (AMODE == 4) dpix = (tap >> 1) * (p.W + 2) + (tap & 1);
 #pragma unroll
         for (int j = 0; j < A_CH; ++j) {
             int pix;
@@ -115,7 +120,8 @@
     const int wave_row0 = __builtin_amdgcn_readfirstlane(wid) * 8;
     auto dma_tile = [&](int kt, int stage) {
         int tap = 0, cc = kt << 6;
-        if (p.taps == 9) { const int cb = kt / 9; tap = kt - cb * 9; cc = cb << 6; }
+        if constexpr (AMODE == 4) { tap = kt & 3; cc = (kt >> 2) << 6; }
+        else if (p.taps == 9) { const int cb = kt / 9; tap = kt - cb * 9; cc = cb << 6; }
         const bool s0 = cc < p.C0;
         const half_t* src = s0 ? p.a0 : p.a1;
         const int cs = s0 ? cc : cc - p.C0, Cs = s0 ? p.C0 : p.C1;
@@ -124,6 +130,7 @@
         int dpix = 0;
         if constexpr (AMODE == 1) dpix = dy * (p.W + 2) + dx;
         else if constexpr (AMODE == 2) dpix = dy * (2 * p.W + 2) + dx;
+        else if constexpr (AMODE == 4) dpix = (tap >> 1) * (p.W + 2) + (tap & 1);
         char* As = smem + stage * STAGE_BYTES;
         char* Bs = As + BM * 128;
 #pragma unroll
@@ -193,13 +200,15 @@
             char* Bsn = Asn + BM * 128;
             if constexpr (DMA) {
                 int tap = 0, cc = ktn << 6;
-                if (p.taps == 9) { const int cb = ktn / 9; tap = ktn - cb * 9; cc = cb << 6; }
+                if constexpr (AMODE == 4) { tap = ktn & 3; cc = (ktn >> 2) << 6; }
+                else if (p.taps == 9) { const int cb = ktn / 9; tap = ktn - cb * 9; cc = cb << 6; }
                 const bool s0 = cc < p.C0;
                 src = s0 ? p.a0 : p.a1;
                 cs = s0 ? cc : cc - p.C0; Cs = s0 ? p.C0 : p.C1;
                 if (p.taps == 9) { dy = tap / 3 - 1; dx = tap - (tap / 3) * 3 - 1; }
                 if constexpr (AMODE == 1) dpix = dy * (p.W + 2) + dx;
                 else if constexpr (AMODE == 2) dpix = dy * (2 * p.W + 2) + dx;
+        else if constexpr (AMODE == 4) dpix = (tap >> 1) * (p.W + 2) + (tap & 1);
             }
             auto piece = [&](int q) {
                 if (q < A_CH) {
@@ -378,10 +387,10 @@
         return;
     }
     Par par;
-    par.lds = GLDS ? smem + PAR_OFF : nullptr; par.n0 = n0; par.b0 = HW > 0 ? qdiv(m0, HW) : 0; par.bnp = par_bnp(BN);
+    par.lds = GLDS ? smem + PAR_OFF : nullptr; par.n0 = n0; par.b0 = HW > 0 ? qdiv(m0, HW) : 0; par.bnp = par_bnp(BN); par.phase = phase;
     constexpr bool STAGED_FITS = WM * WN * 32 * (WTN * 2 + 16) <= NST * STAGE_BYTES;
     if (STAGED_FITS && p.epi == EPI_STORE && (p.N & 7) == 0 && p.staged_epi) {
-        igemm_epilogue_staged<MT, NT, GLDS>(p, acc, mw0, nw0, lane, smem + wid * (32 * (WTN * 2 + 16)), par);
+        igemm_epilogue_staged<MT, NT, GLDS, false, AMODE>(p, acc, mw0, nw0, lane, smem + wid * (32 * (WTN * 2 + 16)), par);
         tl_end(p.tl);
         return;
     }
@@ -399,7 +408,7 @@
         tl_end(p.tl);
         return;
     }
-    igemm_epilogue<MT, NT, GLDS>(p, acc, mw0, nw0, lane, par);
+    igemm_epilogue<MT, NT, GLDS, AMODE>(p, acc, mw0, nw0, lane, par);
     tl_end(p.tl);
 }
 
@@ -460,6 +469,7 @@
     }
     int tile_m, tile_n;
     tile_of(p, wg, tile_m, tile_n);
+    const int phase = phase_of<AMODE>(p, tile_m);
     const int m0 = tile_m * BM, n0 = tile_n * BN;
 
     const int tid = threadIdx.x, lane = tid & 63;
@@ -485,6 +495,8 @@
             else if constexpr (AMODE == 2) {
                 const int b = qdiv(m, HW), r2 = m - b * HW, y = qdiv(r2, p.W), x = r2 - y * p.W;
                 a_pix[q] = (b * (2 * p.H + 2) + 2 * y + 1 + p.ashift) * (2 * p.W + 2) + 2 * x + 1 + p.ashift;
+            } else if constexpr (AMODE == 4) {
+                a_pix[q] = phase_src_pix(m, HW, p.W, p.H, phase);
             } else {
                 const int b = qdiv(m, HW), r2 = m - b * HW, y = qdiv(r2, p.W), x = r2 - y * p.W;
                 a_pix[q] = (b << 22) | (y << 11) | x;
@@ -493,7 +505,7 @@
         } else {
             int n = n0 + (g - A_P) * 16 + prow;
             n = n < p.N ? n : p.N - 1;
-            b_ptr[q] = p.w + (long)n * p.K + schunk * 8;
+            b_ptr[q] = p.w + ((long)phase * p.N + n) * p.K + schunk * 8;
             dst[q] = BM * 64 + (g - A_P) * 16 * 64;
         }
     }
@@ -502,7 +514,8 @@
         Gather g;
         const int k64 = kt >> 1;
         int tap = 0, cc = k64 << 6;
-        if (p.taps == 9) { const int cb = k64 / 9; tap = k64 - cb * 9; cc = cb << 6; }
+        if constexpr (AMODE == 4) { tap = k64 & 3; cc = (k64 >> 2) << 6; }
+        else if (p.taps == 9) { const int cb = k64 / 9; tap = k64 - cb * 9; cc = cb << 6; }
         const bool s0 = cc < p.C0;
         g.src = s0 ? p.a0 : p.a1;
         g.cs = (s0 ? cc : cc - p.C0) + ((kt & 1) << 5); g.Cs = s0 ? p.C0 : p.C1;
@@ -511,6 +524,7 @@
         g.dpix = 0;
         if constexpr (AMODE == 1) g.dpix = g.dy * (p.W + 2) + g.dx;
         else if constexpr (AMODE == 2) g.dpix = g.dy * (2 * p.W + 2) + g.dx;
+        else if constexpr (AMODE == 4) g.dpix = (tap >> 1) * (p.W + 2) + (tap & 1);
         return g;
     };
     auto piece = [&](int q, int kt, int stage, const Gather& g) {
@@ -646,10 +660,10 @@
 
     const int mw0 = m0 + wm * WTM, nw0 = n0 + wn * WTN;
     Par par;
-    par.lds = smem + PAR_OFF; par.n0 = n0; par.b0 = HW > 0 ? qdiv(m0, HW) : 0; par.bnp = par_bnp(BN);
+    par.lds = smem + PAR_OFF; par.n0 = n0; par.b0 = HW > 0 ? qdiv(m0, HW) : 0; par.bnp = par_bnp(BN); par.phase = phase;
     constexpr bool STAGED_FITS = NW * 32 * (WTN * 2 + 16) <= NST * STAGE_BYTES;
     if (STAGED_FITS && p.epi == EPI_STORE && (p.N & 7) == 0 && p.staged_epi) {
-        igemm_epilogue_staged<MT, NT, true>(p, acc, mw0, nw0, lane, smem + wid * (32 * (WTN * 2 + 16)), par);
+        igemm_epilogue_staged<MT, NT, true, false, AMODE>(p, acc, mw0, nw0, lane, smem + wid * (32 * (WTN * 2 + 16)), par);
         tl_end(p.tl);
         return;
     }
@@ -667,11 +681,11 @@
         tl_end(p.tl);
         return;
     }
-    igemm_epilogue<MT, NT, true>(p, acc, mw0, nw0, lane, par);
+    igemm_epilogue<MT, NT, true, AMODE>(p, acc, mw0, nw0, lane, par);
     tl_end(p.tl);
 }
 
-template <bool L = true>
+template <bool L = true, int AMODE = 0>
 __device__ __forceinline__ void igemm_epilogue_staged16(const IGemmArgs& p, f32x4 (&acc)[2][5], int mw0, int nw0, int lane,
                                                         char* stg , const Par& par) {
     constexpr int WTN = 80, PITCH = WTN * 2 + 16, CPR = WTN / 8, NQ = (32 * CPR + 63) / 64;
@@ -681,7 +695,9 @@
     const int mr = mw0 + frow;
     const int mrc = mr < p.M ? mr : p.M - 1;
     int opix = mrc, rpix = mrc;
-    if (p.omode == 1 || p.rmode == 1) {
+    if constexpr (AMODE == 4) {
+        opix = phase_pix(mrc, HW, p.W, p.H, par.phase);
+    } else if (p.omode == 1 || p.rmode == 1) {
         const int pp = padded_pix(mrc, HW, p.W, p.H);
         if (p.omode == 1) opix = pp;
         if (p.rmode == 1) rpix = pp;
@@ -742,7 +758,7 @@
         }
         if (c < 32 * CPR && mm < p.M && n < p.N) *reinterpret_cast<half8_t*>(p.out + (long)op * p.old + n) = v;
     }
-    if (p.gstat) gstat_block<WTN, PITCH>(p, stg, mw0, nw0, lane);
+    if (p.gstat) gstat_block<WTN, PITCH>(p, stg, mw0, nw0, lane, AMODE == 4 ? par.phase : -1);
 }
 
 template <bool L = true>
@@ -830,6 +846,7 @@
     }
     int tile_m, tile_n;
     tile_of(p, wg, tile_m, tile_n);
+    const int phase = phase_of<AMODE>(p, tile_m);
     const int m0 = tile_m * BM, n0 = tile_n * BN;
 
     const int tid = threadIdx.x, lane = tid & 63;
@@ -849,6 +866,8 @@
         else if constexpr (AMODE == 2) {
             const int b = qdiv(m, HW), q = m - b * HW, y = qdiv(q, p.W), x = q - y * p.W;
             a_pix[j] = (b * (2 * p.H + 2) + 2 * y + 1 + p.ashift) * (2 * p.W + 2) + 2 * x + 1 + p.ashift;
+        } else if constexpr (AMODE == 4) {
+            a_pix[j] = phase_src_pix(m, HW, p.W, p.H, phase);
         } else {
             const int b = qdiv(m, HW), q = m - b * HW, y = qdiv(q, p.W), x = q - y * p.W;
             a_pix[j] = (b << 22) | (y << 11) | x;
@@ -860,7 +879,7 @@
     for (int j = 0; j < 3; ++j) {
         int n = n0 + lrow + j * RSTEP;
         n = n < p.N ? n : p.N - 1;
-        b_ptr[j] = p.w + (long)n * p.K + schunk * 8;
+        b_ptr[j] = p.w + ((long)phase * p.N + n) * p.K + schunk * 8;
     }
     const int wave_row0 = wid * 8;
 
@@ -868,7 +887,8 @@
     auto gather_of = [&](int kt) {
         Gather g;
         int tap = 0, cc = kt << 6;
-        if (p.taps == 9) { const int cb = kt / 9; tap = kt - cb * 9; cc = cb << 6; }
+        if constexpr (AMODE == 4) { tap = kt & 3; cc = (kt >> 2) << 6; }
+        else if (p.taps == 9) { const int cb = kt / 9; tap = kt - cb * 9; cc = cb << 6; }
         const bool s0 = cc < p.C0;
         g.src = s0 ? p.a0 : p.a1;
         g.cs = s0 ? cc : cc - p.C0; g.Cs = s0 ? p.C0 : p.C1;
@@ -877,6 +897,7 @@
         g.dpix = 0;
         if constexpr (AMODE == 1) g.dpix = g.dy * (p.W + 2) + g.dx;
         else if constexpr (AMODE == 2) g.dpix = g.dy * (2 * p.W + 2) + g.dx;
+        else if constexpr (AMODE == 4) g.dpix = (tap >> 1) * (p.W + 2) + (tap & 1);
         return g;
     };
     auto piece = [&](int q, int kt, int stage, const Gather& g) {
@@ -998,9 +1019,9 @@
 #undef CFGPP_WAIT_TILES
 
     Par par;
-    par.lds = smem + PAR_OFF; par.n0 = n0; par.b0 = HW > 0 ? qdiv(m0, HW) : 0; par.bnp = par_bnp(BN);
+    par.lds = smem + PAR_OFF; par.n0 = n0; par.b0 = HW > 0 ? qdiv(m0, HW) : 0; par.bnp = par_bnp(BN); par.phase = phase;
     if (p.epi == EPI_HEADS) igemm_epilogue_heads_staged16(p, acc, m0 + wm * 32, n0 + wn * 80, lane, smem + wid * (5 * 1536), par);
-    else igemm_epilogue_staged16(p, acc, m0 + wm * 32, n0 + wn * 80, lane, smem + wid * (32 * 176), par);
+    else igemm_epilogue_staged16<true, AMODE>(p, acc, m0 + wm * 32, n0 + wn * 80, lane, smem + wid * (32 * 176), par);
     tl_end(p.tl);
 }
 
@@ -1024,6 +1045,11 @@
 }
 static int g_staged_epi = 1;
 static int g_last_hint_applied = 1;
+static int g_upsample_phase = 1;
+extern "C" void cfgpp_igemm_set_upsample_phase(int on) { g_upsample_phase = on ? 1 : 0; }
+static int g_last_amode = -1;
+extern "C" int cfgpp_igemm_last_amode(void) { return g_last_amode; }
+extern "C" int cfgpp_igemm_last_config_ran(void) { return g_last_hint_applied; }
 extern "C" void cfgpp_igemm_set_staged_epilogue(int on) { g_staged_epi = on ? 1 : 0; }
 static int g_big_tiles = 1;
 extern "C" void cfgpp_igemm_set_big_tiles(int on) { g_big_tiles = on ? 1 : 0; }
@@ -1040,6 +1066,13 @@
 
 static int g_walk_blocked = 1;
 extern "C" void cfgpp_igemm_set_blocked_walk(int on) { g_walk_blocked = on ? 1 : 0; }
+static double a_traffic(const IGemmArgs& a) { return a.amode == 2 ? 4.0 : a.amode == 3 ? 0.25 : 1.0; }
+static double a_bytes_of(const IGemmArgs& a) { return 2.0 * a.M * (a.amode == 4 ? 4.0 : 1.0) * (a.C0 + a.C1) * a_traffic(a); }
+static int phase_view(IGemmArgs& a, int BM) {
+    a.H >>= 1; a.W >>= 1; a.rows_per_batch = a.H * a.W; a.M >>= 2; a.omode = 2;
+    a.ph_tiles = cdiv(a.M, BM);
+    return 4 * a.ph_tiles;
+}
 static void walk_plan(IGemmArgs& a, int BM, int BN, int ntm, int ntn, int smem) {
     a.walk_bn = 0; a.walk_per = 0; a.walk_tmb = 0; a.walk_tnb = 0;
     const int T = ntm * ntn;
@@ -1048,7 +1081,7 @@
     int wpc = smem > 0 ? (160 * 1024) / smem : 1;
     wpc = wpc < 1 ? 1 : wpc > 4 ? 4 : wpc;
     const int R = 32 * wpc;
-    const double a_row = 2.0 * BM * (a.C0 + a.C1) * (a.amode == 2 ? 4.0 : a.amode == 3 ? 0.25 : 1.0);
+    const double a_row = 2.0 * BM * (a.C0 + a.C1) * a_traffic(a);
     const double w_col = 2.0 * BN * a.K;
     auto cost = [&](auto tile_at) {
         double tot = 0.0;
@@ -1093,7 +1126,8 @@
 }
 
 static void stats_decide(IGemmArgs& a, bool staged_store) {
-    const bool on = a.gstat != nullptr && staged_store && a.epi == EPI_STORE && (a.N & 7) == 0 && (a.M & 31) == 0 && a.ksplit <= 1 && a.n_main > 0;
+    const bool on = a.gstat != nullptr && staged_store && a.epi == EPI_STORE && (a.N & 7) == 0 && (a.M & 31) == 0 && a.ksplit <= 1 && a.n_main > 0 &&
+                    (a.amode != 4 || (a.rows_per_batch & 31) == 0);
     if (!on) a.gstat = nullptr;
     if (a.stat_flag) *a.stat_flag = on ? 1 : 0;
 }
@@ -1106,6 +1140,7 @@
     constexpr int blocks_per_cu = (160 * 1024) / smem_std < 8 ? (160 * 1024) / smem_std : 8;
     constexpr int slots = 256 * blocks_per_cu;
     IGemmArgs a = a_in;
+    const int ntm = AMODE == 4 ? phase_view(a, BM) : cdiv(a.M, BM);
     a.par_nb = par_slots(a, BM);
     const int smem = NST * (BM + BN) * 128 + (GLDS ? par_bytes(BN, a.par_nb > PAR_NB ? a.par_nb : PAR_NB) : 0);
     if (smem > 160 * 1024) {
@@ -1119,17 +1154,18 @@
                                             hipFuncAttributeMaxDynamicSharedMemorySize, smem));
         attr_smem = smem;
     }
-    const int T = cdiv(a.M, BM) * cdiv(a.N, BN);
+    const int T = ntm * cdiv(a.N, BN);
     const int KT = a.K >> 6;
     a.n_main = T; a.ksplit = 1; a.ws = nullptr; a.staged_epi = g_staged_epi;
     {
-        const double w_bytes = 2.0 * a.N * a.K, a_bytes = 2.0 * a.M * (a.C0 + a.C1) * (a.amode == 2 ? 4.0 : a.amode == 3 ? 0.25 : 1.0);
+        const double w_bytes = 2.0 * a.N * a.K, a_bytes = a_bytes_of(a);
         a.n_major = (g_n_major == 1 || (g_n_major < 0 && w_bytes > 1.5 * a_bytes && cdiv(a.N, BN) >= 8)) ? 1 : 0;
         if (g_n_major < 0 && a.walk_hint) a.n_major = a.walk_hint == 2 ? 1 : 0;
     }
     {
         int S = 0;
-        if (a_in.split >= 2 && a.epi == EPI_STORE) S = a_in.split < KT ? a_in.split : KT;
+        if (AMODE == 4) S = 0;
+        else if (a_in.split >= 2 && a.epi == EPI_STORE) S = a_in.split < KT ? a_in.split : KT;
         else if (g_tail_split && a_in.allow_split && (WTM == 64 && WTN == 64) && a.epi == EPI_STORE && T * 2 <= slots && KT >= 32) {
             S = g_tail_split == 2 ? (slots + T - 1) / T : slots / T;
             if (KT / S < 12) S = KT / 12;
@@ -1143,8 +1179,8 @@
     const int n_tail = T - a.n_main;
     stats_decide(a, WM * WN * 32 * (WTN * 2 + 16) <= NST * (BM + BN) * 128 && a.staged_epi && n_tail == 0);
     if (n_tail > 0) a.n_major = 0;
-    a.walk_div = a.n_major ? cdiv(a.M, BM) : cdiv(a.N, BN);
-    walk_plan(a, BM, BN, cdiv(a.M, BM), cdiv(a.N, BN), smem);
+    a.walk_div = a.n_major ? ntm : cdiv(a.N, BN);
+    walk_plan(a, BM, BN, ntm, cdiv(a.N, BN), smem);
     a.tl = tl_take(WM * 100 + WN * 10 + (GLDS ? 1 : 0), a.n_main + n_tail * a.ksplit, NTHR, BM, BN, NST, a);
     hipLaunchKernelGGL(kern, dim3(a.n_main + n_tail * a.ksplit), dim3(NTHR), smem, stream, a);
     if (n_tail > 0)
@@ -1160,6 +1196,7 @@
         case 1: return launch_cfg_amode<WM, WN, WTM, WTN, GLDS, 1, NST>(a, stream);
         case 2: return launch_cfg_amode<WM, WN, WTM, WTN, GLDS, 2, NST>(a, stream);
         case 3: return launch_cfg_amode<WM, WN, WTM, WTN, GLDS, 3, NST>(a, stream);
+        case 4: return launch_cfg_amode<WM, WN, WTM, WTN, GLDS, 4, NST>(a, stream);
         default: cfgpp_set_error("igemm: bad amode %d", a.amode); return -2;
     }
 }
@@ -1170,6 +1207,7 @@
     constexpr int WGS = WPE * 4 / (WM * WN);
     static_assert((NST * (BM + BN) * 64 + par_bytes(BN)) * WGS <= 160 * 1024, "the workgroups that are meant to share a CU do not fit its LDS");
     IGemmArgs a = a_in;
+    const int ntm = AMODE == 4 ? phase_view(a, BM) : cdiv(a.M, BM);
     a.par_nb = par_slots(a, BM);
     const int nb = a.temb ? (a.par_nb > PAR_NB ? a.par_nb : PAR_NB) : 0;
     const int smem = NST * (BM + BN) * 64 + par_bytes(BN, nb);
@@ -1184,9 +1222,9 @@
         CFGPP_HIP_CHECK(hipFuncSetAttribute(reinterpret_cast<const void*>(kern), hipFuncAttributeMaxDynamicSharedMemorySize, smem));
         attr_smem = smem;
     }
-    const int ntm = cdiv(a.M, BM), ntn = cdiv(a.N, BN);
+    const int ntn = cdiv(a.N, BN);
     a.n_main = ntm * ntn; a.ksplit = 1; a.ws = nullptr; a.staged_epi = g_staged_epi;
-    const double w_bytes = 2.0 * a.N * a.K, a_bytes = 2.0 * a.M * (a.C0 + a.C1) * (a.amode == 2 ? 4.0 : a.amode == 3 ? 0.25 : 1.0);
+    const double w_bytes = 2.0 * a.N * a.K, a_bytes = a_bytes_of(a);
     a.n_major = (g_n_major == 1 || (g_n_major < 0 && w_bytes > 1.5 * a_bytes && ntn >= 8)) ? 1 : 0;
     if (g_n_major < 0 && a.walk_hint) a.n_major = a.walk_hint == 2 ? 1 : 0;
     a.walk_div = a.n_major ? ntm : ntn;
@@ -1204,6 +1242,8 @@
         case 1: return launch_tile32_amode<WM, WN, WTM, WTN, NST, WPE, 1>(a, stream);
         case 2: return launch_tile32_amode<WM, WN, WTM, WTN, NST, WPE, 2>(a, stream);
         case 3: return launch_tile32_amode<WM, WN, WTM, WTN, NST, WPE, 3>(a, stream);
+        case 4: if constexpr (WTN == 160) { g_last_hint_applied = 0; return launch_cfg_amode<4, 2, 64, 160, true, 4, 2>(a, stream); }
+                else return launch_tile32_amode<WM, WN, WTM, WTN, NST, WPE, 4>(a, stream);
         default: cfgpp_set_error("igemm: bad amode %d", a.amode); return -2;
     }
 }
@@ -1221,6 +1261,7 @@
 template <int AMODE, int NST>
 int launch_mf16_amode(const IGemmArgs& a_in, hipStream_t stream) {
     IGemmArgs a = a_in;
+    const int ntm = AMODE == 4 ? phase_view(a, 128) : cdiv(a.M, 128);
     a.par_nb = par_slots(a, 128);
     const int smem = NST * (128 + 160) * 128 + par_bytes(160, a.par_nb > PAR_NB ? a.par_nb : PAR_NB);
     if (smem > 160 * 1024) { g_last_hint_applied = 0; return launch_cfg_amode<4, 1, 32, 160, true, AMODE, 2>(a_in, stream); }
@@ -1230,9 +1271,9 @@
         CFGPP_HIP_CHECK(hipFuncSetAttribute(reinterpret_cast<const void*>(kern), hipFuncAttributeMaxDynamicSharedMemorySize, smem));
         attr_smem = smem;
     }
-    const int ntm = cdiv(a.M, 128), ntn = a.N / 160;
+    const int ntn = a.N / 160;
     a.n_main = ntm * ntn; a.ksplit = 1; a.ws = nullptr; a.staged_epi = 1;
-    const double w_bytes = 2.0 * a.N * a.K, a_bytes = 2.0 * a.M * (a.C0 + a.C1) * (a.amode == 2 ? 4.0 : a.amode == 3 ? 0.25 : 1.0);
+    const double w_bytes = 2.0 * a.N * a.K, a_bytes = a_bytes_of(a);
     a.n_major = (g_n_major == 1 || (g_n_major < 0 && w_bytes > 1.5 * a_bytes && ntn >= 8)) ? 1 : 0;
     if (g_n_major < 0 && a.walk_hint) a.n_major = a.walk_hint == 2 ? 1 : 0;
     a.walk_div = a.n_major ? ntm : ntn;
@@ -1250,6 +1291,7 @@
         case 1: return launch_mf16_amode<1, NST>(a, stream);
         case 2: return launch_mf16_amode<2, NST>(a, stream);
         case 3: return launch_mf16_amode<3, NST>(a, stream);
+        case 4: return launch_mf16_amode<4, NST>(a, stream);
         default: cfgpp_set_error("igemm: bad amode %d", a.amode); return -2;
     }
 }
@@ -1267,7 +1309,7 @@
     const int smem = big4_smem(cfg, a);
     const int ntm = cdiv(a.M, BM), ntn = cdiv(a.N, BN);
     a.n_main = ntm * ntn; a.ksplit = 1; a.ws = nullptr; a.staged_epi = 1;
-    const double w_bytes = 2.0 * a.N * a.K, a_bytes = 2.0 * a.M * (a.C0 + a.C1) * (a.amode == 2 ? 4.0 : a.amode == 3 ? 0.25 : 1.0);
+    const double w_bytes = 2.0 * a.N * a.K, a_bytes = a_bytes_of(a);
     a.n_major = (g_n_major == 1 || (g_n_major < 0 && w_bytes > 1.5 * a_bytes && ntn >= 8)) ? 1 : 0;
     if (g_n_major < 0 && a.walk_hint) a.n_major = a.walk_hint == 2 ? 1 : 0;
     a.walk_div = a.n_major ? ntm : ntn;
@@ -1326,8 +1368,10 @@
                  return launch_tile32<4, 2, 64, 160, 4, 2>(a, stream);
         case 18: return mf16_supports(a) ? launch_mf16<3>(a, stream) : launch_cfg<4, 1, 32, 160, true>(a, stream);
         case 19: return mf16_supports(a) ? launch_mf16<4>(a, stream) : launch_cfg<4, 1, 32, 160, true>(a, stream);
-        case 24: case 25: case 26: return big4_ok(cfg, a) ? launch_big4(cfg, a, stream) : launch_cfg<2, 2, 64, 64, true>(a, stream);
-        case 28: return big4p_ok(a) ? launch_big4p(a, stream) : launch_cfg<2, 2, 64, 64, true>(a, stream);
+        case 24: case 25: case 26: if (a.amode == 4) g_last_hint_applied = 0;
+                 return big4_ok(cfg, a) ? launch_big4(cfg, a, stream) : launch_cfg<2, 2, 64, 64, true>(a, stream);
+        case 28: if (a.amode == 4) g_last_hint_applied = 0;
+                 return big4p_ok(a) ? launch_big4p(a, stream) : launch_cfg<2, 2, 64, 64, true>(a, stream);
         default: cfgpp_set_error("igemm: bad config %d", cfg); return -2;
     }
 }
@@ -1352,7 +1396,7 @@
 unsigned igemm_tune_mask() { return g_tune_mask; }
 extern "C" unsigned cfgpp_igemm_tuner_state(void) {
     return g_tune_mask ^ ((unsigned)g_big_tiles << 1) ^ ((unsigned)g_tail_split << 3) ^ ((unsigned)(g_n_major + 1) << 6) ^ ((unsigned)g_walk_blocked << 9) ^
-           ((unsigned)g_staged_epi << 10) ^ ((unsigned)g_force_cfg << 12) ^ ((unsigned)g_staging << 20);
+           ((unsigned)g_staged_epi << 10) ^ ((unsigned)(g_upsample_phase ^ 1) << 11) ^ ((unsigned)g_force_cfg << 12) ^ ((unsigned)g_staging << 20);
 }
 
 extern "C" void cfgpp_igemm_timeline(void* buf, long cap_blocks, int target) {
@@ -1361,20 +1405,26 @@
 extern "C" void cfgpp_igemm_timeline_info(int* out12) { for (int i = 0; i < 12; ++i) out12[i] = g_tl_info[i]; }
 
 int igemm_last_hint_applied() { return g_last_hint_applied; }
+int igemm_upsample_phase_enabled() { return g_upsample_phase; }
 
 int igemm_launch(const IGemmArgs& a_in, hipStream_t stream) {
     IGemmArgs a = a_in;
+    g_last_amode = a.amode;
     g_last_hint_applied = (a_in.cfg_hint & 63) == 0 ? 1 : 0;
     a.allow_split = 1;
     a.tl = nullptr;
     if (g_tl) { if (g_tl_count == g_tl_target) a.tl = g_tl; ++g_tl_count; }
     const int Cin = a.C0 + a.C1;
     CFGPP_REQUIRE(a.C0 > 0 && a.C0 % 64 == 0 && a.C1 % 64 == 0, "igemm: C0=%d C1=%d must be multiples of 64", a.C0, a.C1);
-    CFGPP_REQUIRE(a.taps == 1 || a.taps == 9, "igemm: taps=%d", a.taps);
+    CFGPP_REQUIRE(a.amode >= 0 && a.amode <= 4, "igemm: bad amode %d", a.amode);
+    CFGPP_REQUIRE(a.amode == 4 ? a.taps == 4 : (a.taps == 1 || a.taps == 9), "igemm: taps=%d (amode %d)", a.taps, a.amode);
     CFGPP_REQUIRE(a.K == a.taps * Cin, "igemm: K=%d != taps*Cin=%d", a.K, a.taps * Cin);
     CFGPP_REQUIRE(a.N % 4 == 0 && a.M > 0 && a.N > 0, "igemm: M=%d N=%d (N must be a multiple of 4)", a.M, a.N);
     CFGPP_REQUIRE(a.amode == 0 || (a.H > 0 && a.W > 0 && a.rows_per_batch == a.H * a.W), "igemm: spatial args");
     CFGPP_REQUIRE(a.amode != 3 || (a.H < 2048 && a.W < 2048 && (a.M / a.rows_per_batch) < 512), "igemm: upsample range");
+    CFGPP_REQUIRE(a.amode != 4 || (a.C1 == 0 && a.H % 2 == 0 && a.W % 2 == 0 && a.M % a.rows_per_batch == 0 && a.epi == EPI_STORE && a.omode == 1 &&
+                                   a.resid == nullptr && a.temb == nullptr && a.N % 8 == 0 && (long)(a.M / a.rows_per_batch) * (a.H + 2) * (a.W + 2) < (1L << 31)),
+                  "igemm: 2x2 phase form (amode 4) needs one source, even H x W, M a multiple of H * W, a plain store (N %% 8 == 0) into a padded output, no residual / time embedding");
     CFGPP_REQUIRE(a.epi != EPI_GEGLU || a.N % 64 == 0, "igemm: GEGLU needs N %% 64 == 0");
     CFGPP_REQUIRE(a.epi != EPI_HEADS || (a.head_dim % 4 == 0 && a.part_width % 4 == 0), "igemm: heads args");
     CFGPP_REQUIRE(a.rows_per_batch <= 0 || a.M / a.rows_per_batch < (1 << 20), "igemm: %d rows in batches of %d (batch index must stay below 2^20)", a.M, a.rows_per_batch);
@@ -1418,11 +1468,11 @@
         const int KT = a.K >> 6;
         const long t128 = (long)cdiv(a.M, 128) * cdiv(a.N, 128);
         const long t_rule = cfg == 14 ? (long)cdiv(a.M, 256) * cdiv(a.N, 128) : t128;
-        const bool rule_splits = (cfg == 1 || cfg == 12 || cfg == 14) && g_tail_split && a.epi == EPI_STORE && KT >= 32 && t_rule * 2 <= (cfg == 1 ? 512 : 256);
+        const bool rule_splits = a.amode != 4 && (cfg == 1 || cfg == 12 || cfg == 14) && g_tail_split && a.epi == EPI_STORE && KT >= 32 && t_rule * 2 <= (cfg == 1 ? 512 : 256);
         const int h = a.cfg_hint & 63;
         const bool valid = (h == 1 || h == 4 || h == 6 || h == 12 || h == 14 || (h == 10 && a.epi == EPI_GEGLU) ||
                             ((h == 5 || h == 7 || h == 8 || h == 9 || h == 11) && a.epi != EPI_GEGLU) ||
-                            h == 13 || h == 15 || h == 16 || h == 17 || (h == 20 && a.epi != EPI_GEGLU) || (h == 27 && a.epi == EPI_STORE) || ((h >= 24 && h <= 26) && big4_ok(h, a)) || (h == 28 && big4p_ok(a))) && (g_big_tiles || h == 1);
+                            h == 13 || h == 15 || h == 16 || h == 17 || (h == 20 && a.epi != EPI_GEGLU) || (h == 27 && a.epi == EPI_STORE) || ((h >= 24 && h <= 26) && a.amode != 4 && big4_ok(h, a)) || (h == 28 && big4p_ok(a))) && (g_big_tiles || h == 1);
         if (!rule_splits && valid) { cfg = h; a.allow_split = 0; g_last_hint_applied = 1; }
     }
     a.walk_hint = (g_force_cfg == 0 && g_staging != 0) ? (a.cfg_hint >> 6) & 3 : 0;
diff --git a/cfgpp_amd/csrc/lora_kernels.hip b/cfgpp_amd/csrc/lora_kernels.hip
--- a/cfgpp_amd/csrc/lora_kernels.hip
+++ b/cfgpp_amd/csrc/lora_kernels.hip
@@ -78,6 +78,39 @@
     }
 }
 
+__global__ __launch_bounds__(256) void fold_upsample_kernel(const half_t* __restrict__ w9, half_t* __restrict__ w4, long O, long CB) {
+    const long idx = (long)blockIdx.x * 256 + threadIdx.x;
+    if (idx >= 4 * O * CB * 32) return;
+    const int c8 = (int)(idx & 7), tap = (int)((idx >> 3) & 3);
+    const long r = idx >> 5, cb = r % CB, po = r / CB, o = po % O;
+    const int phase = (int)(po / O);
+    const int py = phase >> 1, px = phase & 1, a = tap >> 1, b = tap & 1;
+    const int t0 = a == 0 ? 0 : 1 + py, t1 = a == 0 ? py : 2;
+    const int s0 = b == 0 ? 0 : 1 + px, s1 = b == 0 ? px : 2;
+    const half_t* src = w9 + ((o * CB + cb) * 9) * 64 + c8 * 8;
+    float acc[8];
+#pragma unroll
+    for (int k = 0; k < 8; ++k) acc[k] = 0.f;
+    for (int t = t0; t <= t1; ++t)
+        for (int s = s0; s <= s1; ++s) {
+            const half8_t v = *reinterpret_cast<const half8_t*>(src + (t * 3 + s) * 64);
+#pragma unroll
+            for (int k = 0; k < 8; ++k) acc[k] += (float)v[k];
+        }
+    half8_t out;
+#pragma unroll
+    for (int k = 0; k < 8; ++k) out[k] = (half_t)acc[k];
+    *reinterpret_cast<half8_t*>(w4 + idx * 8) = out;
+}
+
+}
+
+int igemm_fold_upsample_launch(const half_t* w9, half_t* w4, long O, long I, hipStream_t s) {
+    CFGPP_REQUIRE(w9 && w4 && O > 0 && I > 0 && I % 64 == 0 && O * I < (1L << 34), "fold_upsample: bad args (O=%ld, I=%ld: a multiple of 64)", O, I);
+    const long n = 4 * O * (I / 64) * 32;
+    hipLaunchKernelGGL(fold_upsample_kernel, dim3((unsigned)cdiv(n, 256L)), dim3(256), 0, s, w9, w4, O, I / 64);
+    CFGPP_HIP_CHECK(hipGetLastError());
+    return 0;
 }
 
 int lora_merge_launch(const half_t* base, half_t* dst, const float* up, const float* down, int rank, int kind, long O, long I,
diff --git a/cfgpp_amd/csrc/unet.hip b/cfgpp_amd/csrc/unet.hip
--- a/cfgpp_amd/csrc/unet.hip
+++ b/cfgpp_amd/csrc/unet.hip
@@ -1159,7 +1159,10 @@
     hipStream_t s = (hipStream_t)stream;
     const size_t bytes = (size_t)w->O * w->K() * sizeof(half_t);
     if (rank == 0) {
-        if (w->base) CFGPP_HIP_CHECK(hipMemcpyAsync(w->rows(), w->base, bytes, hipMemcpyDeviceToDevice, s));
+        if (w->base) {
+            CFGPP_HIP_CHECK(hipMemcpyAsync(w->rows(), w->base, bytes, hipMemcpyDeviceToDevice, s));
+            return u->refold(w->rows(), s);
+        }
         return 0;
     }
     if (!w->base) {
@@ -1170,8 +1173,8 @@
     }
     const int kind = w->kind == SLOT_MEMBER ? SLOT_PLAIN : w->kind;
     int e = lora_merge_launch(w->base, w->rows(), up, down, rank, kind, w->O, w->I, w->taps, s);
-    if (e) { const std::string m = cfgpp_last_error(); cfgpp_set_error("lora: %s: %s", key, m.c_str()); }
-    return e;
+    if (e) { const std::string m = cfgpp_last_error(); cfgpp_set_error("lora: %s: %s", key, m.c_str()); return e; }
+    return u->refold(w->rows(), s);
 }
 
 int cfgpp_unet_read_weight(cfgpp_unet* u, const char* key, void* host_fp16_out) {
@@ -1215,6 +1218,21 @@
     return igemm_launch(a, (hipStream_t)stream);
 }
 
+int cfgpp_op_fold_upsample(const void* w9, void* w4, int O, int I, void* stream) {
+    return igemm_fold_upsample_launch((const half_t*)w9, (half_t*)w4, O, I, (hipStream_t)stream);
+}
+
+int cfgpp_op_upsample_conv3x3(const void* src, int C, int Hs, int Ws, const void* w9, const void* w4, int rows, int N,
+                              const float* bias, void* out, void* stream) {
+    IGemmArgs a = base_args();
+    const bool ph = w4 != nullptr && upsample_phase_form(Hs, Ws, N);
+    a.a0 = (const half_t*)src; a.C0 = C; a.taps = ph ? 4 : 9; a.amode = ph ? 4 : 3; a.H = 2 * Hs; a.W = 2 * Ws;
+    a.w = (const half_t*)(ph ? w4 : w9); a.M = rows * a.H * a.W; a.N = N; a.K = a.taps * C; a.bias = bias;
+    a.rows_per_batch = a.H * a.W; a.out = (half_t*)out; a.omode = 1; a.old = N; a.epi = EPI_STORE;
+    a.gstat = g_op_gstat; a.stat_flag = &g_op_gstat_flag; g_op_gstat_flag = 0;
+    return igemm_launch(a, (hipStream_t)stream);
+}
+
 int cfgpp_op_igemm_heads(const void* a_, int K, const void* w, int M, int N, const float* bias, int rows_per_batch,
                          void* hq, void* hk, void* hvt, int part0, int part_width, int head_dim, int heads,
                          int q_tok_pad, int tok_pad, void* stream) {
```

New measurement: 8.870 images/sec, median of 6. +3.2%, better.
